# shionhonda/IaGo

Measured on AMD Instinct MI355X. Metric: self-play games/sec, higher is better.
Workload: dtype f16 MFMA operands (float32 split in 2 / 3 pieces), f32 accumulate; u64 bitboards; f32 / f64 tree statistics

## Files before the change

### iago_amd/csrc/conv_policy_body.hpp

```cpp
#pragma once
#include "abi_common.hpp"
#include "search_request.hpp"

#include <hip/hip_fp16.h>

#include <cstdlib>

#include <atomic>

namespace iago_policy {


typedef _Float16 half8 __attribute__((ext_vector_type(8)));
typedef float float16v __attribute__((ext_vector_type(16)));
typedef float float4v __attribute__((ext_vector_type(4)));
#define IAGO_POLICY_MFMA16(acc, a, b) asm volatile("v_mfma_f32_16x16x32_f16 %0, %1, %2, %0" : "+a"(acc) : "v"(a), "v"(b))
typedef unsigned int u32x4 __attribute__((ext_vector_type(4)));
typedef float f2 __attribute__((ext_vector_type(2)));
typedef _Float16 h2 __attribute__((ext_vector_type(2)));

constexpr int RS = 800;
constexpr int ZB = 1280;
constexpr int BS = 64 * RS + ZB;
constexpr int HEAD_FLOATS = 64;
constexpr int W1_LDS = (64 * 18 + 64) * 4;
constexpr int LDS_BYTES = BS + 1024 + HEAD_FLOATS * 4 + W1_LDS;
constexpr float S1 = 1.0f / 2048.0f, S2 = 1.0f / (2048.0f * 2048.0f);

struct PolicyParams {
    const uint64_t *own, *opp;
    const int64_t *index;
    const int32_t *n_dev;
    int64_t n;
    const float *w1, *b1;
    const uint4 *w_hi[7], *w_mid[7], *w_lo[7];
    const float *bias[7];
    const float *w9, *b10;
    float *probs;
    uint32_t *overflow;
    int layer_lo, layer_hi;
    uint4 *scratch;
    int64_t row_lo, row_hi;
};

__device__ __forceinline__ void split3(const f2 v, h2 &hi, h2 &mid, h2 &lo)
{
    hi = __builtin_convertvector(v, h2);
    const f2 r1 = (v - __builtin_convertvector(hi, f2)) * 2048.0f;
    mid = __builtin_convertvector(r1, h2);
    const f2 r2 = (r1 - __builtin_convertvector(mid, f2)) * 2048.0f;
    lo = __builtin_convertvector(r2, h2);
}

extern __shared__ __align__(16) char policy_lds[];

template <bool SRCH = false>
__device__ __forceinline__ void policy_item(const PolicyParams &P, const int64_t row_id, const uint32_t *pos = nullptr,
                                            float *res = nullptr, const float *w1_staged = nullptr,
                                            const float *head_w = nullptr)
{
    char *const T = policy_lds;
    int tid_ = threadIdx.x;
    if constexpr (SRCH)
        asm volatile("" : "+v"(tid_));
    const int tid = tid_, wv = __builtin_amdgcn_readfirstlane(tid >> 6), lane = tid & 63;
    const int64_t b = P.index ? P.index[row_id] : row_id;

    if (tid < ZB / 16)
        *(uint4 *)(T + 64 * RS + tid * 16) = make_uint4(0, 0, 0, 0);
    bool saturated = false;
    if (P.layer_lo > 0) {
        const uint4 *src = P.scratch + (row_id - P.row_lo) * (64 * RS / 16);
        for (int e = tid; e < 64 * RS / 16; e += 256)
            *(uint4 *)(T + e * 16) = src[e];
    } else {
        const int cell = tid & 63, y = cell >> 3, x = cell & 7;
        const uint64_t bits0 = SRCH ? iago_request::opp(pos) : P.opp[b];
        const uint64_t bits1 = SRCH ? iago_request::own(pos) : P.own[b];
        float in[18];
#pragma unroll
        for (int c = 0; c < 2; c++)
#pragma unroll
            for (int ky = 0; ky < 3; ky++)
#pragma unroll
                for (int kx = 0; kx < 3; kx++) {
                    const int yy = y + ky - 1, xx = x + kx - 1;
                    const bool ok = yy >= 0 && yy < 8 && xx >= 0 && xx < 8;
                    const int a = (yy * 8 + xx) & 63;
                    in[c * 9 + ky * 3 + kx] = (ok && (((c ? bits1 : bits0) >> a) & 1ull)) ? 1.0f : 0.0f;
                }
        const float *w1s = w1_staged;
        if constexpr (!SRCH) {
            float *const st = (float *)(T + BS + 1024 + HEAD_FLOATS * 4);
            for (int e = tid; e < 64 * 18 / 4; e += 256)
                ((float4 *)st)[e] = ((const float4 *)P.w1)[e];
            if (tid < 16)
                ((float4 *)(st + 64 * 18))[tid] = ((const float4 *)P.b1)[tid];
            __syncthreads();
            w1s = st;
        }
#pragma unroll 1
        for (int g2 = 0; g2 < 2; g2++) {
            const int grp = __builtin_amdgcn_readfirstlane(g2 * 4 + wv);
            const int co0 = grp * 8;
            _Float16 p0[8], p1[8], p2[8];
#pragma unroll
            for (int k = 0; k < 8; k += 2) {
                const float *wa = w1s + (co0 + k) * 18, *wb = wa + 18;
                f2 acc = (f2){w1s[64 * 18 + co0 + k], w1s[64 * 18 + co0 + k + 1]};
#pragma unroll
                for (int j = 0; j < 18; j++)
                    acc = __builtin_elementwise_fma((f2){wa[j], wb[j]}, (f2){in[j], in[j]}, acc);
                saturated |= !(acc.x <= 65000.0f) || !(acc.y <= 65000.0f);
                f2 v;
                v.x = fminf(fmaxf(acc.x, 0.0f), 65000.0f);
                v.y = fminf(fmaxf(acc.y, 0.0f), 65000.0f);
                h2 a0, a1, a2;
                split3(v, a0, a1, a2);
                p0[k] = a0.x, p0[k + 1] = a0.y;
                p1[k] = a1.x, p1[k + 1] = a1.y;
                p2[k] = a2.x, p2[k + 1] = a2.y;
            }
            char *dst = T + cell * RS + (grp >> 1) * 32 + (grp & 1) * 16;
            *(uint4 *)dst = *(const uint4 *)p0;
            *(uint4 *)(dst + 256) = *(const uint4 *)p1;
            *(uint4 *)(dst + 512) = *(const uint4 *)p2;
        }
    }
    __syncthreads();

    const int c16 = lane & 15, kq = lane >> 4;
    uint32_t addr[4][9];
#pragma unroll
    for (int q = 0; q < 4; q++)
#pragma unroll
        for (int tap = 0; tap < 9; tap++) {
            const int cell = 16 * q + c16;
            const int yy = (cell >> 3) + tap / 3 - 1, xx = (cell & 7) + tap % 3 - 1;
            const bool ok = yy >= 0 && yy < 8 && xx >= 0 && xx < 8;
            const int lin = (cell + (tap / 3 - 1) * 8 + (tap % 3 - 1)) & 7;
            addr[q][tap] = (uint32_t)((ok ? (yy * 8 + xx) * RS : 64 * RS + 32 * lin) + kq * 16);
        }
    uint32_t wrow[4];
#pragma unroll
    for (int q = 0; q < 4; q++)
        wrow[q] = (uint32_t)((16 * q + c16) * RS);

    for (int L = P.layer_lo; L < P.layer_hi; L++) {
        const int n_pairs = L == 0 ? 2 : 4;
        const char *const wh = (const char *)P.w_hi[L], *const wm = (const char *)P.w_mid[L], *const wl = (const char *)P.w_lo[L];
        const uint32_t a_lane = (uint32_t)(((32 * wv + c16) * 2 + (kq & 1) + (kq >> 1) * (9 * 256)) * 16);
        auto a_load = [&](const char *base, uint32_t step_bytes, int m) -> u32x4 {
            return *(const u32x4 *)(base + step_bytes + a_lane + (uint32_t)m * 512u);
        };
        float4v acc0[2][4], acc0b[2][4], acc1[2][4], acc2[2][4];
#pragma unroll
        for (int m = 0; m < 2; m++)
#pragma unroll
            for (int n = 0; n < 4; n++)
#pragma unroll
                for (int v = 0; v < 4; v++) {
                    acc0[m][n][v] = 0.0f;
                    acc0b[m][n][v] = 0.0f;
                    acc1[m][n][v] = 0.0f;
                    acc2[m][n][v] = 0.0f;
                }
        u32x4 a_hi[3][2], a_mid[3][2], a_lo[3][2];
#pragma unroll
        for (int i = 0; i < 2; i++)
#pragma unroll
            for (int m = 0; m < 2; m++) {
                a_hi[i][m] = a_load(wh, (uint32_t)i * 4096u, m);
                a_mid[i][m] = a_load(wm, (uint32_t)i * 4096u, m);
                a_lo[i][m] = a_load(wl, (uint32_t)i * 4096u, m);
            }
        half8 bh[3], bm[3], bl[3];
        auto b_addr = [&](int tile) -> const char * {
            const int over = tile >= 36 ? 64 : 0, tt = tile % 36;
            return T + addr[tt & 3][tt >> 2] + over;
        };
        {
            const char *p0 = b_addr(0), *p1 = b_addr(1);
            bh[0] = *(const half8 *)p0, bm[0] = *(const half8 *)(p0 + 256), bl[0] = *(const half8 *)(p0 + 512);
            bh[1] = *(const half8 *)p1, bm[1] = *(const half8 *)(p1 + 256), bl[1] = *(const half8 *)(p1 + 512);
        }
        for (int cp = 0; cp < n_pairs; cp++) {
#pragma unroll
            for (int tap = 0; tap < 9; tap++) {
                int cp2 = cp, tp2 = tap + 2;
                if (tp2 >= 9) {
                    tp2 -= 9;
                    cp2 += 1;
                }
                if (cp2 >= n_pairs) {
                    cp2 = n_pairs - 1;
                    tp2 = 8;
                }
                const uint32_t w2 = (uint32_t)(18 * cp2 + tp2) * 4096u;
                half8 ah[2], am[2], al[2];
#pragma unroll
                for (int m = 0; m < 2; m++) {
                    ah[m] = __builtin_bit_cast(half8, a_hi[tap % 3][m]);
                    am[m] = __builtin_bit_cast(half8, a_mid[tap % 3][m]);
                    al[m] = __builtin_bit_cast(half8, a_lo[tap % 3][m]);
                }
#pragma unroll
                for (int q = 0; q < 4; q++) {
                    const int tile = tap * 4 + q, cur = tile % 3, nxt = (tile + 2) % 3;
                    const char *p = b_addr(tile + 2);
                    __builtin_amdgcn_sched_barrier(0);
                    IAGO_POLICY_MFMA16(acc2[0][q], ah[0], bl[cur]);
                    bh[nxt] = *(const half8 *)p;
                    __builtin_amdgcn_sched_barrier(0);
                    IAGO_POLICY_MFMA16(acc2[1][q], ah[1], bl[cur]);
                    bm[nxt] = *(const half8 *)(p + 256);
                    __builtin_amdgcn_sched_barrier(0);
                    IAGO_POLICY_MFMA16(acc1[0][q], ah[0], bm[cur]);
                    bl[nxt] = *(const half8 *)(p + 512);
                    __builtin_amdgcn_sched_barrier(0);
                    IAGO_POLICY_MFMA16(acc1[1][q], ah[1], bm[cur]);
                    if (q == 0)
                        a_hi[(tap + 2) % 3][0] = a_load(wh, w2, 0);
                    else if (q == 1)
                        a_mid[(tap + 2) % 3][0] = a_load(wm, w2, 0);
                    else if (q == 2)
                        a_lo[(tap + 2) % 3][0] = a_load(wl, w2, 0);
                    __builtin_amdgcn_sched_barrier(0);
                    if (tap & 1)
                        IAGO_POLICY_MFMA16(acc0b[0][q], ah[0], bh[cur]);
                    else
                        IAGO_POLICY_MFMA16(acc0[0][q], ah[0], bh[cur]);
                    if (q == 0)
                        a_hi[(tap + 2) % 3][1] = a_load(wh, w2, 1);
                    else if (q == 1)
                        a_mid[(tap + 2) % 3][1] = a_load(wm, w2, 1);
                    else if (q == 2)
                        a_lo[(tap + 2) % 3][1] = a_load(wl, w2, 1);
                    __builtin_amdgcn_sched_barrier(0);
                    if (tap & 1)
                        IAGO_POLICY_MFMA16(acc0b[1][q], ah[1], bh[cur]);
                    else
                        IAGO_POLICY_MFMA16(acc0[1][q], ah[1], bh[cur]);
                    IAGO_POLICY_MFMA16(acc2[0][q], al[0], bh[cur]);
                    IAGO_POLICY_MFMA16(acc2[1][q], al[1], bh[cur]);
                    IAGO_POLICY_MFMA16(acc1[0][q], am[0], bh[cur]);
                    IAGO_POLICY_MFMA16(acc1[1][q], am[1], bh[cur]);
                    IAGO_POLICY_MFMA16(acc2[0][q], am[0], bm[cur]);
                    IAGO_POLICY_MFMA16(acc2[1][q], am[1], bm[cur]);
                    __builtin_amdgcn_sched_barrier(0);
                }
            }
#pragma unroll
            for (int q = 0; q < 4; q++)
#pragma unroll
                for (int tap = 0; tap < 9; tap++)
                    addr[q][tap] += 64u;
        }
#pragma unroll
        for (int q = 0; q < 4; q++)
#pragma unroll
            for (int tap = 0; tap < 9; tap++)
                addr[q][tap] -= 64u * (uint32_t)n_pairs;

        f2 bia[2][2];
#pragma unroll
        for (int m = 0; m < 2; m++) {
            const float4 bq = *(const float4 *)(P.bias[L] + 32 * wv + 16 * m + 4 * kq);
            bia[m][0] = (f2){bq.x, bq.y};
            bia[m][1] = (f2){bq.z, bq.w};
        }
        asm volatile("s_nop 15\n\ts_nop 7" ::: "memory");
        __syncthreads();
        float vmax = 0.0f;
        f2 vsum = (f2){0.0f, 0.0f};
#pragma unroll
        for (int q = 0; q < 4; q++) {
            char *row = T + wrow[q] + (32 * wv + 4 * kq) * 2;
#pragma unroll
            for (int m = 0; m < 2; m++) {
                h2 p0[2], p1[2], p2[2];
#pragma unroll
                for (int t2 = 0; t2 < 2; t2++) {
                    const f2 m0 = (f2){acc0[m][q][2 * t2], acc0[m][q][2 * t2 + 1]} + (f2){acc0b[m][q][2 * t2], acc0b[m][q][2 * t2 + 1]};
                    const f2 m1 = (f2){acc1[m][q][2 * t2], acc1[m][q][2 * t2 + 1]};
                    const f2 m2 = (f2){acc2[m][q][2 * t2], acc2[m][q][2 * t2 + 1]};
                    f2 v = (m2 * S2 + m1 * S1) + m0 + bia[m][t2];
                    vmax = fmaxf(fmaxf(vmax, v.x), v.y);
                    vsum += v;
                    v.x = __builtin_amdgcn_fmed3f(v.x, 0.0f, 65000.0f);
                    v.y = __builtin_amdgcn_fmed3f(v.y, 0.0f, 65000.0f);
                    split3(v, p0[t2], p1[t2], p2[t2]);
                }
                *(uint2 *)(row + 32 * m) = (uint2){__builtin_bit_cast(uint32_t, p0[0]), __builtin_bit_cast(uint32_t, p0[1])};
                *(uint2 *)(row + 32 * m + 256) =
                    (uint2){__builtin_bit_cast(uint32_t, p1[0]), __builtin_bit_cast(uint32_t, p1[1])};
                *(uint2 *)(row + 32 * m + 512) =
                    (uint2){__builtin_bit_cast(uint32_t, p2[0]), __builtin_bit_cast(uint32_t, p2[1])};
            }
        }
        saturated |= !(vmax <= 65000.0f) || !(vsum.x + vsum.y == vsum.x + vsum.y);
        __syncthreads();
    }
    if (P.overflow && saturated)
        *P.overflow = 1u;
    if (P.layer_hi < 7) {
        uint4 *dst = P.scratch + (row_id - P.row_lo) * (64 * RS / 16);
        for (int e = tid; e < 64 * RS / 16; e += 256)
            dst[e] = *(const uint4 *)(T + e * 16);
        return;
    }

    if (wv == 0) {
        const char *row = T + lane * RS;
        float acc = 0.0f;
#pragma unroll 4
        for (int c8 = 0; c8 < 16; c8++) {
            const half8 xh = *(const half8 *)(row + c8 * 16), xm = *(const half8 *)(row + 256 + c8 * 16),
                        xl = *(const half8 *)(row + 512 + c8 * 16);
            const float *w9 = SRCH ? head_w : P.w9;
            const float4 wa = *(const float4 *)(w9 + c8 * 8), wb = *(const float4 *)(w9 + c8 * 8 + 4);
            const float w[8] = {wa.x, wa.y, wa.z, wa.w, wb.x, wb.y, wb.z, wb.w};
#pragma unroll
            for (int e = 0; e < 8; e++) {
                const float xv = ((float)xl[e] * S2 + (float)xm[e] * S1) + (float)xh[e];
                acc = fmaf(w[e], xv, acc);
            }
        }
        const float logit = acc + (SRCH ? head_w[128 + lane] : P.b10[lane]);
        float mx = logit;
#pragma unroll
        for (int o = 32; o > 0; o >>= 1)
            mx = fmaxf(mx, __shfl_xor(mx, o));
        const float e = expf(logit - mx);
        float sum = e;
#pragma unroll
        for (int o = 32; o > 0; o >>= 1)
            sum += __shfl_xor(sum, o);
        if constexpr (SRCH)
            res[lane] = e / sum;
        else
            P.probs[row_id * 64 + lane] = e / sum;
    }
}

inline int policy_params_of(const iago_policy_split3_args *a, PolicyParams &P)
{
    if (!a || a->n < 0)
        return iago_fail(IAGO_ERR_INVALID, "iago_policy_forward_split3: null args or n < 0");
    if (!a->own || !a->opp || !a->w1 || !a->b1 || !a->w9 || !a->b10 || !a->probs)
        return iago_fail(IAGO_ERR_INVALID, "iago_policy_forward_split3: null pointer");
    for (int L = 0; L < 7; L++) {
        if (!a->w_hi[L] || !a->w_mid[L] || !a->w_lo[L] || !a->bias[L] || ((uintptr_t)a->w_hi[L] & 15u) ||
            ((uintptr_t)a->w_mid[L] & 15u) || ((uintptr_t)a->w_lo[L] & 15u) || ((uintptr_t)a->bias[L] & 15u))
            return iago_fail(IAGO_ERR_INVALID, "iago_policy_forward_split3: weights and biases of blocks 2..8 must be "
                                               "non-null and 16-byte aligned");
        P.w_hi[L] = (const uint4 *)a->w_hi[L];
        P.w_mid[L] = (const uint4 *)a->w_mid[L];
        P.w_lo[L] = (const uint4 *)a->w_lo[L];
        P.bias[L] = a->bias[L];
    }
    if (((uintptr_t)a->w9 & 15u) || ((uintptr_t)a->w1 & 15u) || ((uintptr_t)a->b1 & 15u))
        return iago_fail(IAGO_ERR_INVALID, "iago_policy_forward_split3: w1, b1, w9 must be 16-byte aligned");
    P.own = a->own;
    P.opp = a->opp;
    P.index = a->index;
    P.n_dev = a->n_dev;
    P.n = a->n;
    P.w1 = a->w1;
    P.b1 = a->b1;
    P.w9 = a->w9;
    P.b10 = a->b10;
    P.probs = a->probs;
    P.overflow = a->overflow;
    P.layer_lo = 0;
    P.layer_hi = 7;
    P.scratch = nullptr;
    P.row_lo = 0;
    P.row_hi = a->n;
    return IAGO_OK;
}

}
```

### iago_amd/csrc/conv_policy_kernel.hip

```cpp
#include "conv_policy_body.hpp"

#include <cstdlib>

namespace {
using namespace iago_policy;

__global__ __launch_bounds__(256) __attribute__((amdgpu_waves_per_eu(1, 1))) void policy_resident_kernel(PolicyParams P)
{
    int64_t n_rows = P.row_hi;
    if (P.n_dev)
        n_rows = min(n_rows, (int64_t)*P.n_dev);
    for (int64_t row = P.row_lo + blockIdx.x; row < n_rows; row += gridDim.x) {
        policy_item(P, row);
        __syncthreads();
    }
}

}

int iago_policy_forward_split3(const iago_policy_split3_args *a, void *stream)
{
    if (a && a->n == 0)
        return IAGO_OK;
    PolicyParams P;
    if (const int rc = policy_params_of(a, P))
        return rc;
    static std::atomic<uint64_t> configured{0};
    if (iago_reserve_lds((const void *)policy_resident_kernel, LDS_BYTES, configured,
                         "iago_policy_forward_split3: cannot reserve 52 KB of LDS"))
        return IAGO_ERR_HIP;
    static const int64_t cap = []() {
        const char *e = getenv("IAGO_POLICY_GRID");
        const long v = e ? atol(e) : 256;
        return (int64_t)(v < 1 ? 1 : v > 1024 ? 1024 : v);
    }();

    const int parts = a->parts < 1 ? 1 : (a->parts > 7 ? 7 : a->parts);
    if (parts > 1 && (!a->scratch || ((uintptr_t)a->scratch & 15u)))
        return iago_fail(IAGO_ERR_INVALID, "iago_policy_forward_split3: parts > 1 needs a 16-byte aligned scratch "
                                           "buffer of n x 51,200 bytes");
    P.scratch = (uint4 *)a->scratch;
    const int64_t chunk = (parts > 1 && a->scratch_rows > 0 && a->scratch_rows < a->n) ? a->scratch_rows : a->n;
    for (int64_t lo = 0; lo < a->n; lo += chunk) {
        P.row_lo = lo;
        P.row_hi = lo + chunk < a->n ? lo + chunk : a->n;
        const int64_t rows = P.row_hi - P.row_lo;
        const unsigned grid = (unsigned)(rows < cap ? rows : cap);
        for (int p = 0; p < parts; p++) {
            P.layer_lo = 7 * p / parts;
            P.layer_hi = 7 * (p + 1) / parts;
            hipLaunchKernelGGL(policy_resident_kernel, dim3(grid), dim3(256), LDS_BYTES, (hipStream_t)stream, P);
        }
    }
    return iago_check_launch("iago_policy_forward_split3");
}
```

### iago_amd/csrc/conv_trunk_body.hpp

```cpp
#pragma once
#include "abi_common.hpp"
#include "rollout_row_body.hpp"
#include "search_request.hpp"

#include <hip/hip_fp16.h>

#include <atomic>
#include <type_traits>

namespace iago_trunk {


typedef _Float16 half8 __attribute__((ext_vector_type(8)));
typedef float float16v __attribute__((ext_vector_type(16)));
typedef float float4v __attribute__((ext_vector_type(4)));
typedef unsigned int u32x4 __attribute__((ext_vector_type(4)));
typedef float f2 __attribute__((ext_vector_type(2)));
typedef _Float16 h2 __attribute__((ext_vector_type(2)));

constexpr int RS = 544;
constexpr int ZB = 1024;
constexpr int BS = 64 * RS + ZB;
constexpr int lds_alloc(int tb) { return tb * BS + 1024; }
constexpr int MAX_LAYERS = 8;

#define IAGO_MFMA16(acc, a, b) asm volatile("v_mfma_f32_16x16x32_f16 %0, %1, %2, %0" : "+a"(acc) : "v"(a), "v"(b))

struct TrunkRParams {
    const uint4 *x_hi, *x_lo;
    uint4 *y_hi, *y_lo;
    const uint4 *w_hi[MAX_LAYERS], *w_lo[MAX_LAYERS];
    const float *bias[MAX_LAYERS];
    int64_t n;
    int32_t cin0, n_layers;
    uint32_t *overflow;
    const float *planes;
    const uint64_t *own, *opp;
    const float *w1, *b1;
    const uint4 *w9_hi, *w9_lo;
    const float *b9, *w10, *w11;
    float *out;
    const int64_t *index;
    const int32_t *n_dev;
    int32_t count_lo, count_hi;
    int32_t layer_lo, layer_hi;
    char *scratch;
};
constexpr int IMG = 64 * RS;

struct Piece {
    const int64_t *index;
    const int32_t *n_dev;
    char *scratch;
    int layer_lo, layer_hi;
    const uint32_t *pos;
    float *res;
    const float *w1s;
    const char *head_w;
};
constexpr int HEAD_W_W9LO = 8192, HEAD_W_W10 = 16384, HEAD_W_W11 = 16384 + 32768, HEAD_W_B9 = HEAD_W_W11 + 512,
              HEAD_W_LDS = HEAD_W_B9 + 16;
__device__ __forceinline__ Piece whole_walk(const TrunkRParams &P)
{
    return Piece{P.index, P.n_dev, P.scratch, P.layer_lo, P.layer_hi, nullptr, nullptr, nullptr, nullptr};
}

constexpr int head_lds(int tb) { return (9 * 64 * tb + 64 * tb + 128 * tb) * 4; }
constexpr int W1_LDS = (64 * 18 + 64) * 4;
constexpr int lds_alloc_fused(int tb) { return lds_alloc(tb) + head_lds(tb) + W1_LDS; }

__device__ __forceinline__ int cell_of_lane(int r)
{
    return r < 4 ? r : r < 12 ? 16 + (r - 4) : r < 16 ? 4 + (r - 12) : r < 20 ? 24 + (r - 16) : r < 28 ? 8 + (r - 20)
                                                                                              : 28 + (r - 28);
}

extern __shared__ __align__(16) char trunk_lds[];

constexpr bool tile_off_board(int tb, int tap, int n)
{
    return tb >= 2 && ((tap < 3 && (n & 7) == 0) || (tap >= 6 && (n & 7) == 7));
}
constexpr int kept_before(int tb, int tap, int n)
{
    int k = 0;
    for (int t = 0; t < 9; t++)
        for (int m = 0; m < 4 * tb; m++) {
            if (t == tap && m == n)
                return k;
            k += !tile_off_board(tb, t, m);
        }
    return k;
}
constexpr int kept_tile(int tb, int k)
{
    for (int t = 0; t < 9; t++)
        for (int m = 0; m < 4 * tb; m++)
            if (!tile_off_board(tb, t, m) && k-- == 0)
                return t * 4 * tb + m;
    return -1;
}
template <int I0, int I1, class F>
__device__ __forceinline__ void static_for(F &&f)
{
    if constexpr (I0 < I1) {
        f(std::integral_constant<int, I0>{});
        static_for<I0 + 1, I1>(f);
    }
}

template <bool FUSED, int TB, bool SRCH = false>
__device__ __forceinline__ void trunk_item(const TrunkRParams &P, const Piece &W, const int64_t b0, const int64_t n_rows)
{
    constexpr int NN = 4 * TB;
    char *const T = trunk_lds;
    int tid_ = threadIdx.x;
    if constexpr (SRCH)
        asm volatile("" : "+v"(tid_));
    const int tid = tid_, wv = __builtin_amdgcn_readfirstlane(tid >> 6), lane = tid & 63, r = lane & 31, h = lane >> 5;

    if (tid < TB * (ZB / 16))
        *(uint4 *)(T + (tid / (ZB / 16)) * BS + 64 * RS + (tid % (ZB / 16)) * 16) = make_uint4(0, 0, 0, 0);
    bool saturated = false;
    constexpr bool PIECES = FUSED && TB <= 2;
    if (PIECES && W.layer_lo > 0) {
        constexpr int PER = (TB * (IMG / 16) + 255) / 256;
        uint4 img[PER];
#pragma unroll
        for (int i = 0; i < PER; i++) {
            const int e = min(tid + i * 256, TB * (IMG / 16) - 1);
            const int board = e / (IMG / 16), off = e - board * (IMG / 16);
            const int64_t row = min(b0 + board, n_rows - 1);
            img[i] = ((const uint4 *)(W.scratch + row * IMG))[off];
        }
#pragma unroll
        for (int i = 0; i < PER; i++) {
            const int e = tid + i * 256;
            const int board = e / (IMG / 16), off = e - board * (IMG / 16);
            if (e < TB * (IMG / 16))
                *(uint4 *)(T + board * BS + off * 16) = img[i];
        }
    } else if constexpr (FUSED) {
        const int cell = tid & 63, y = cell >> 3, x = cell & 7;
        float in[TB][18];
#pragma unroll
        for (int board = 0; board < TB; board++) {
            const int64_t row = min(b0 + board, n_rows - 1);
            const int64_t b = W.index ? W.index[row] : row;
            const float *pl = P.planes + b * 128;
            uint64_t bits0, bits1;
            if constexpr (SRCH) {
                const uint32_t *w = W.pos + iago_request::WORDS * board;
                bits1 = iago_request::own(w);
                bits0 = iago_request::opp(w);
            } else {
                bits0 = P.planes ? 0ull : P.opp[b];
                bits1 = P.planes ? 0ull : P.own[b];
            }
#pragma unroll
            for (int c = 0; c < 2; c++)
#pragma unroll
                for (int ky = 0; ky < 3; ky++)
#pragma unroll
                    for (int kx = 0; kx < 3; kx++) {
                        const int yy = y + ky - 1, xx = x + kx - 1;
                        const bool ok = yy >= 0 && yy < 8 && xx >= 0 && xx < 8;
                        const int a = (yy * 8 + xx) & 63;
                        float v;
                        if (P.planes)
                            v = ok ? pl[c * 64 + a] : 0.0f;
                        else
                            v = (ok && (((c ? bits1 : bits0) >> a) & 1ull)) ? 1.0f : 0.0f;
                        in[board][c * 9 + ky * 3 + kx] = v;
                    }
        }
        const float *w1s = W.w1s;
        if constexpr (!SRCH) {
            float *const st = (float *)(T + lds_alloc(TB) + head_lds(TB));
            for (int e = tid; e < 64 * 18 / 4; e += 256)
                ((float4 *)st)[e] = ((const float4 *)P.w1)[e];
            if (tid < 16)
                ((float4 *)(st + 64 * 18))[tid] = ((const float4 *)P.b1)[tid];
            __syncthreads();
            w1s = st;
        }
#pragma unroll 1
        for (int g2 = 0; g2 < 2; g2++) {
            const int grp = __builtin_amdgcn_readfirstlane(g2 * 4 + wv);
            const int co0 = grp * 8;
            _Float16 h8[TB][8], l8[TB][8];
#pragma unroll
            for (int k = 0; k < 8; k++) {
                const float *wk = w1s + (co0 + k) * 18;
                const float bk = w1s[64 * 18 + co0 + k];
                float wreg[18];
#pragma unroll
                for (int j = 0; j < 18; j++)
                    wreg[j] = wk[j];
                float accs[TB];
                if constexpr (TB % 2 == 0) {
#pragma unroll
                    for (int bp = 0; bp < TB; bp += 2) {
                        f2 acc = (f2){bk, bk};
#pragma unroll
                        for (int j = 0; j < 18; j++)
                            acc = __builtin_elementwise_fma((f2){wreg[j], wreg[j]}, (f2){in[bp][j], in[bp + 1][j]}, acc);
                        accs[bp] = acc.x;
                        accs[bp + 1] = acc.y;
                    }
                } else {
#pragma unroll
                    for (int board = 0; board < TB; board++) {
                        float acc = bk;
#pragma unroll
                        for (int j = 0; j < 18; j++)
                            acc = fmaf(wreg[j], in[board][j], acc);
                        accs[board] = acc;
                    }
                }
#pragma unroll
                for (int board = 0; board < TB; board++) {
                    const float acc = accs[board];
                    saturated |= !(acc <= 65000.0f);
                    const float v = fminf(fmaxf(acc, 0.0f), 65000.0f);
                    const _Float16 vh = (_Float16)v;
                    h8[board][k] = vh;
                    l8[board][k] = (_Float16)((v - (float)vh) * 2048.0f);
                }
            }
#pragma unroll
            for (int board = 0; board < TB; board++) {
                char *dst = T + board * BS + cell * RS + (grp >> 1) * 32 + (grp & 1) * 16;
                *(uint4 *)dst = *(const uint4 *)h8[board];
                *(uint4 *)(dst + 256) = *(const uint4 *)l8[board];
            }
        }
    } else {
        const int chunks0 = P.cin0 >> 4;
        const int pieces = TB * chunks0 * 128;
        for (int e = tid; e < pieces; e += 256) {
            const int board = e / (chunks0 * 128), rem = e - board * chunks0 * 128;
            const int chunk = rem >> 7, cell = (rem >> 1) & 63, hp = rem & 1;
            const int64_t b = min(b0 + board, P.n - 1);
            const int64_t src = (b * chunks0 + chunk) * 128 + (rem & 127);
            char *dst = T + board * BS + cell * RS + chunk * 32 + hp * 16;
            *(uint4 *)dst = P.x_hi[src];
            *(uint4 *)(dst + 256) = P.x_lo[src];
        }
    }
    __syncthreads();

    constexpr bool ROWS = TB >= 2;
    static_assert(TB == 1 || TB == 2 || TB == 4, "boards per workgroup");
    const int c16 = lane & 15, kq = lane >> 4;
    constexpr int NADDR = ROWS ? 9 : 36;
    uint32_t addr[NADDR];
    uint32_t sx[2] = {0u, 0u};
    uint32_t wrow[ROWS ? 1 : 4];
    if constexpr (ROWS) {
        const int x = c16 & 7, odd = c16 >> 3;
#pragma unroll
        for (int tap = 0; tap < 9; tap++) {
            const int row = tap < 3 ? 1 : 0;
            const int yy = row + tap / 3 - 1, xx = x + tap % 3 - 1;
            const bool ok = xx >= 0 && xx < 8;
            addr[tap] = (uint32_t)(odd * BS + (ok ? (yy * 8 + xx) * RS : 64 * RS + 32 * (xx & 7)) + kq * 16);
        }
        sx[0] = x > 0 ? 8u * RS : 0u;
        sx[1] = x < 7 ? 8u * RS : 0u;
        wrow[0] = (uint32_t)(odd * BS + x * RS);
    } else {
#pragma unroll
        for (int q = 0; q < 4; q++)
#pragma unroll
            for (int tap = 0; tap < 9; tap++) {
                const int cell = 16 * q + c16;
                const int yy = (cell >> 3) + tap / 3 - 1, xx = (cell & 7) + tap % 3 - 1;
                const bool ok = yy >= 0 && yy < 8 && xx >= 0 && xx < 8;
                const int lin = (cell + (tap / 3 - 1) * 8 + (tap % 3 - 1)) & 7;
                addr[9 * q + tap] = (uint32_t)((ok ? (yy * 8 + xx) * RS : 64 * RS + 32 * lin) + kq * 16);
            }
#pragma unroll
        for (int q = 0; q < 4; q++)
            wrow[q] = (uint32_t)((16 * q + c16) * RS);
    }
    auto b_off = [&](int tap, int n) -> uint32_t {
        if constexpr (ROWS) {
            const int dx = tap % 3 - 1, r = (n & 7) - (tap < 3 ? 1 : 0);
            return addr[tap] + (uint32_t)r * (dx == 0 ? 8u * RS : sx[dx > 0]) + (uint32_t)(n >> 3) * (2u * BS);
        } else {
            return addr[9 * n + tap];
        }
    };

    const int L_lo = PIECES ? W.layer_lo : 0, L_hi = PIECES ? W.layer_hi : P.n_layers;
    for (int L = L_lo; L < L_hi; L++) {
        const int n_pairs = L == 0 ? (P.cin0 >> 5) : 4;
        const char *const wh = (const char *)P.w_hi[L], *const wl = (const char *)P.w_lo[L];
        const uint32_t a_lane = (uint32_t)(((32 * wv + c16) * 2 + (kq & 1) + (kq >> 1) * (9 * 256)) * 16);
        auto a_load = [&](const char *base, uint32_t step_bytes, int m) -> u32x4 {
            return *(const u32x4 *)(base + step_bytes + a_lane + (uint32_t)m * 512u);
        };
        float4v acc_main[2][NN], acc_cross[2][NN];
#pragma unroll
        for (int m = 0; m < 2; m++)
#pragma unroll
            for (int n = 0; n < NN; n++)
#pragma unroll
                for (int v = 0; v < 4; v++) {
                    acc_main[m][n][v] = 0.0f;
                    acc_cross[m][n][v] = 0.0f;
                }

        u32x4 a_hi[3][2], a_lo[3][2];
#pragma unroll
        for (int i = 0; i < 2; i++)
#pragma unroll
            for (int m = 0; m < 2; m++) {
                a_hi[i][m] = a_load(wh, (uint32_t)i * 4096u, m);
                a_lo[i][m] = a_load(wl, (uint32_t)i * 4096u, m);
            }
        constexpr int KEPT = kept_before(TB, 9, 0), NR = KEPT % 4 == 0 ? 4 : 6;
        static_assert(KEPT % NR == 0, "the B ring must line up at every chunk pair");
        half8 bh[NR], bl[NR];
        static_for<0, 3>([&](auto kc) __attribute__((always_inline)) {
            constexpr int tile = kept_tile(TB, decltype(kc)::value);
            const char *p0 = T + b_off(tile / NN, tile % NN);
            bh[decltype(kc)::value] = *(const half8 *)p0;
            bl[decltype(kc)::value] = *(const half8 *)(p0 + 256);
        });
        for (int cp = 0; cp < n_pairs; cp++) {
            static_for<0, KEPT>([&](auto kc) __attribute__((always_inline)) {
                constexpr int k = decltype(kc)::value, tile = kept_tile(TB, k), tap = tile / NN, n = tile % NN;
                constexpr int j = k - kept_before(TB, tap, 0);
                static_assert(kept_before(TB, tap + 1, 0) - kept_before(TB, tap, 0) >= 4, "four A loads per k-step");
                constexpr int kn = k + 3, tile_n = kept_tile(TB, kn % KEPT), cur = k % NR, nxt = kn % NR;
                constexpr uint32_t over = kn >= KEPT ? 64u : 0u;
                int cp2 = cp, tp2 = tap + 2;
                if (tp2 >= 9) {
                    tp2 -= 9;
                    cp2 += 1;
                }
                if (cp2 >= n_pairs) {
                    cp2 = n_pairs - 1;
                    tp2 = 8;
                }
                const uint32_t w2 = (uint32_t)(18 * cp2 + tp2) * 4096u;
                const half8 ah0 = __builtin_bit_cast(half8, a_hi[tap % 3][0]), ah1 = __builtin_bit_cast(half8, a_hi[tap % 3][1]);
                const half8 al0 = __builtin_bit_cast(half8, a_lo[tap % 3][0]), al1 = __builtin_bit_cast(half8, a_lo[tap % 3][1]);
                const char *p = T + b_off(tile_n / NN, tile_n % NN) + over;
                __builtin_amdgcn_sched_barrier(0);
                IAGO_MFMA16(acc_cross[0][n], ah0, bl[cur]);
                bh[nxt] = *(const half8 *)p;
                __builtin_amdgcn_sched_barrier(0);
                IAGO_MFMA16(acc_cross[1][n], ah1, bl[cur]);
                bl[nxt] = *(const half8 *)(p + 256);
                __builtin_amdgcn_sched_barrier(0);
                IAGO_MFMA16(acc_main[0][n], ah0, bh[cur]);
                if constexpr (j == 0)
                    a_hi[(tap + 2) % 3][0] = a_load(wh, w2, 0);
                else if constexpr (j == 1)
                    a_hi[(tap + 2) % 3][1] = a_load(wh, w2, 1);
                else if constexpr (j == 2)
                    a_lo[(tap + 2) % 3][0] = a_load(wl, w2, 0);
                else if constexpr (j == 3)
                    a_lo[(tap + 2) % 3][1] = a_load(wl, w2, 1);
                __builtin_amdgcn_sched_barrier(0);
                IAGO_MFMA16(acc_main[1][n], ah1, bh[cur]);
                IAGO_MFMA16(acc_cross[0][n], al0, bh[cur]);
                IAGO_MFMA16(acc_cross[1][n], al1, bh[cur]);
                __builtin_amdgcn_sched_barrier(0);
            });
#pragma unroll
            for (int i = 0; i < NADDR; i++)
                addr[i] += 64u;
        }
#pragma unroll
        for (int i = 0; i < NADDR; i++)
            addr[i] -= 64u * (uint32_t)n_pairs;

        f2 bia[2][2];
#pragma unroll
        for (int m = 0; m < 2; m++) {
            const float4 bq = *(const float4 *)(P.bias[L] + 32 * wv + 16 * m + 4 * kq);
            bia[m][0] = (f2){bq.x, bq.y};
            bia[m][1] = (f2){bq.z, bq.w};
        }
        asm volatile("s_nop 15\n\ts_nop 7" ::: "memory");
        __syncthreads();
        float vmax = 0.0f;
        f2 vsum = (f2){0.0f, 0.0f};
#pragma unroll
        for (int n = 0; n < NN; n++) {
            char *row = T + (ROWS ? wrow[0] + (n & 7) * (8 * RS) + (n >> 3) * (2 * BS) : wrow[ROWS ? 0 : n]) + (32 * wv + 4 * kq) * 2;
#pragma unroll
            for (int m = 0; m < 2; m++) {
                h2 hi[2], lo[2];
#pragma unroll
                for (int t2 = 0; t2 < 2; t2++) {
                    const f2 mm = (f2){acc_main[m][n][2 * t2], acc_main[m][n][2 * t2 + 1]};
                    const f2 c = (f2){acc_cross[m][n][2 * t2], acc_cross[m][n][2 * t2 + 1]};
                    f2 v = c * (1.0f / 2048.0f) + mm + bia[m][t2];
                    vmax = fmaxf(fmaxf(vmax, v.x), v.y);
                    vsum += v;
                    v.x = __builtin_amdgcn_fmed3f(v.x, 0.0f, 65000.0f);
                    v.y = __builtin_amdgcn_fmed3f(v.y, 0.0f, 65000.0f);
                    hi[t2] = __builtin_convertvector(v, h2);
                    lo[t2] = __builtin_convertvector((v - __builtin_convertvector(hi[t2], f2)) * 2048.0f, h2);
                }
                *(uint2 *)(row + 32 * m) = (uint2){__builtin_bit_cast(uint32_t, hi[0]), __builtin_bit_cast(uint32_t, hi[1])};
                *(uint2 *)(row + 32 * m + 256) =
                    (uint2){__builtin_bit_cast(uint32_t, lo[0]), __builtin_bit_cast(uint32_t, lo[1])};
            }
        }
        saturated |= !(vmax <= 65000.0f) || !(vsum.x + vsum.y == vsum.x + vsum.y);
        __syncthreads();
    }
    if (P.overflow && saturated)
        *P.overflow = 1u;

    if (PIECES && W.layer_hi < P.n_layers) {
        for (int e = tid; e < TB * (IMG / 16); e += 256) {
            const int board = e / (IMG / 16), off = e - board * (IMG / 16);
            if (b0 + board < n_rows)
                ((uint4 *)(W.scratch + (b0 + board) * IMG))[off] = *(const uint4 *)(T + board * BS + off * 16);
        }
        return;
    }
    if constexpr (FUSED) {
        constexpr int NC = 64 * TB;
        float *const Dm = (float *)(T + lds_alloc(TB));
        float *const h9s = Dm + 9 * NC;
        float *const hid = h9s + NC;
        float4 w10row[16];
        if constexpr (!SRCH) {
#pragma unroll
            for (int c = 0; c < 16; c++)
                w10row[c] = ((const float4 *)(P.w10 + (tid & 127) * 64))[c];
        }
        const float w11j = SRCH ? ((const float *)(W.head_w + HEAD_W_W11))[tid & 127] : P.w11[tid & 127];
        const float b9 = SRCH ? *(const float *)(W.head_w + HEAD_W_B9) : P.b9[0];
        const int lane_cell = cell_of_lane(r);
        if (wv < TB) {
            const u32x4 *w9h = (const u32x4 *)P.w9_hi + r * 2 + h;
            const u32x4 *w9l = (const u32x4 *)P.w9_lo + r * 2 + h;
            float16v hm[2], hc[2];
#pragma unroll
            for (int jt = 0; jt < 2; jt++)
#pragma unroll
                for (int v = 0; v < 16; v++) {
                    hm[jt][v] = 0.0f;
                    hc[jt][v] = 0.0f;
                }
            u32x4 w9a[SRCH ? 1 : 8], w9b[SRCH ? 1 : 8];
            if constexpr (!SRCH) {
#pragma unroll
                for (int c = 0; c < 8; c++) {
                    w9a[c] = w9h[c * 64];
                    w9b[c] = w9l[c * 64];
                }
            }
#pragma unroll
            for (int c = 0; c < 8; c++) {
                const half8 ah = SRCH ? *(const half8 *)(W.head_w + (c * 64 + r * 2 + h) * 16)
                                      : __builtin_bit_cast(half8, w9a[SRCH ? 0 : c]);
                const half8 al = SRCH ? *(const half8 *)(W.head_w + HEAD_W_W9LO + (c * 64 + r * 2 + h) * 16)
                                      : __builtin_bit_cast(half8, w9b[SRCH ? 0 : c]);
#pragma unroll
                for (int jt = 0; jt < 2; jt++) {
                    const int jj = 2 * wv + jt;
                    const char *p = T + (jj >> 1) * BS + (32 * (jj & 1) + lane_cell) * RS + h * 16 + c * 32;
                    const half8 bh9 = *(const half8 *)p, bl9 = *(const half8 *)(p + 256);
                    hm[jt] = __builtin_amdgcn_mfma_f32_32x32x16_f16(ah, bh9, hm[jt], 0, 0, 0);
                    hc[jt] = __builtin_amdgcn_mfma_f32_32x32x16_f16(ah, bl9, hc[jt], 0, 0, 0);
                    hc[jt] = __builtin_amdgcn_mfma_f32_32x32x16_f16(al, bh9, hc[jt], 0, 0, 0);
                }
            }
#pragma unroll
            for (int jt = 0; jt < 2; jt++) {
                const int jj = 2 * wv + jt;
                const int base = (jj >> 1) * 64 + 32 * (jj & 1) + lane_cell;
#pragma unroll
                for (int t = 0; t < 4; t++)
                    Dm[(4 * h + t) * NC + base] = hm[jt][t] + hc[jt][t] * (1.0f / 2048.0f);
                if (h == 0)
                    Dm[8 * NC + base] = hm[jt][4] + hc[jt][4] * (1.0f / 2048.0f);
            }
        }
        __syncthreads();
        if constexpr (SRCH) {
#pragma unroll
            for (int c = 0; c < 16; c++)
                w10row[c] = ((const float4 *)(W.head_w + HEAD_W_W10))[c * 128 + (tid & 127)];
        }
        if (tid < NC) {
            const int cell = tid & 63, y = cell >> 3, x = cell & 7;
            float s9 = 0.0f;
#pragma unroll
            for (int tap = 0; tap < 9; tap++) {
                const int yy = y + tap / 3 - 1, xx = x + tap % 3 - 1;
                if (yy >= 0 && yy < 8 && xx >= 0 && xx < 8)
                    s9 += Dm[tap * NC + (tid & ~63) + yy * 8 + xx];
            }
            h9s[tid] = fmaxf(s9 + b9, 0.0f);
        }
        __syncthreads();
        if ((tid >> 7) * 2 < TB) {
            const int j = tid & 127, pb = (tid >> 7) * 2;
            float s0 = 0.0f, s1 = 0.0f;
#pragma unroll
            for (int c = 0; c < 16; c++) {
                const float4 wq = w10row[c];
                const float4 x0 = *(const float4 *)(h9s + pb * 64 + 4 * c);
                const float4 x1 = *(const float4 *)(h9s + (pb + 1 < TB ? pb + 1 : pb) * 64 + 4 * c);
                s0 = fmaf(wq.x, x0.x, s0);
                s0 = fmaf(wq.y, x0.y, s0);
                s0 = fmaf(wq.z, x0.z, s0);
                s0 = fmaf(wq.w, x0.w, s0);
                s1 = fmaf(wq.x, x1.x, s1);
                s1 = fmaf(wq.y, x1.y, s1);
                s1 = fmaf(wq.z, x1.z, s1);
                s1 = fmaf(wq.w, x1.w, s1);
            }
            hid[pb * 128 + j] = s0 * w11j;
            if (pb + 1 < TB)
                hid[(pb + 1) * 128 + j] = s1 * w11j;
        }
        __syncthreads();
        if (tid < TB && b0 + tid < n_rows) {
            float4 hv[32];
#pragma unroll
            for (int j4 = 0; j4 < 32; j4++)
                hv[j4] = *(const float4 *)(hid + tid * 128 + 4 * j4);
            float v = 0.0f;
#pragma unroll
            for (int j4 = 0; j4 < 32; j4++) {
#pragma clang fp reassociate(off)
                v += hv[j4].x;
                v += hv[j4].y;
                v += hv[j4].z;
                v += hv[j4].w;
            }
            const int64_t row = b0 + tid;
            if constexpr (SRCH)
                W.res[tid] = v;
            else
                P.out[W.index ? W.index[row] : row] = v;
        }
        return;
    }
    for (int e = tid; e < TB * 1024; e += 256) {
        const int board = e >> 10, cb = (e >> 7) & 7, cell = (e >> 1) & 63, hp = e & 1;
        const int64_t b = b0 + board;
        if (b < P.n) {
            const char *src = T + board * BS + cell * RS + cb * 32 + hp * 16;
            P.y_hi[b * 1024 + (e & 1023)] = *(const uint4 *)src;
            P.y_lo[b * 1024 + (e & 1023)] = *(const uint4 *)(src + 256);
        }
    }
}

template <bool FUSED, int TB>
__device__ __forceinline__ void trunk_walk(const TrunkRParams &P, const Piece &W, const int64_t bid, const int64_t nb)
{
    int64_t n_rows = P.n;
    if constexpr (FUSED) {
        if (W.n_dev)
            n_rows = min(P.n, (int64_t)*W.n_dev);
        if (n_rows <= P.count_lo || n_rows > P.count_hi)
            return;
    }
    for (int64_t b0 = bid * TB; b0 < n_rows; b0 += nb * TB) {
        trunk_item<FUSED, TB>(P, W, b0, n_rows);
        __syncthreads();
    }
}

inline int value_params_of(const iago_value_split_args *a, TrunkRParams &P)
{
    if (!a || a->n < 0)
        return iago_fail(IAGO_ERR_INVALID, "iago_value_forward_split: null args or n < 0");
    if ((!a->planes && (!a->own || !a->opp)) || !a->w1 || !a->b1 || !a->w9_hi || !a->w9_lo || !a->b9 || !a->w10 ||
        !a->w11 || !a->out)
        return iago_fail(IAGO_ERR_INVALID, "iago_value_forward_split: null pointer");
    for (int L = 0; L < 7; L++) {
        if (!a->w_hi[L] || !a->w_lo[L] || !a->bias[L] || ((uintptr_t)a->w_hi[L] & 15u) || ((uintptr_t)a->w_lo[L] & 15u) ||
            ((uintptr_t)a->bias[L] & 15u))
            return iago_fail(IAGO_ERR_INVALID, "iago_value_forward_split: weights and biases of blocks 2..8 must be "
                                               "non-null and 16-byte aligned");
        P.w_hi[L] = (const uint4 *)a->w_hi[L];
        P.w_lo[L] = (const uint4 *)a->w_lo[L];
        P.bias[L] = a->bias[L];
    }
    P.w_hi[7] = P.w_hi[6];
    P.w_lo[7] = P.w_lo[6];
    P.bias[7] = P.bias[6];
    if (((uintptr_t)a->w9_hi & 15u) || ((uintptr_t)a->w9_lo & 15u) || ((uintptr_t)a->w10 & 15u) || ((uintptr_t)a->w1 & 15u) ||
        ((uintptr_t)a->b1 & 15u))
        return iago_fail(IAGO_ERR_INVALID, "iago_value_forward_split: w1, b1, w9_hi, w9_lo, w10 must be 16-byte aligned");
    P.x_hi = P.x_lo = nullptr;
    P.y_hi = P.y_lo = nullptr;
    P.n = a->n;
    P.cin0 = 64;
    P.n_layers = 7;
    P.overflow = a->overflow;
    P.planes = a->planes;
    P.own = a->own;
    P.opp = a->opp;
    P.w1 = a->w1;
    P.b1 = a->b1;
    P.w9_hi = (const uint4 *)a->w9_hi;
    P.w9_lo = (const uint4 *)a->w9_lo;
    P.b9 = a->b9;
    P.w10 = a->w10;
    P.w11 = a->w11;
    P.out = a->out;
    if (a->index && a->planes)
        return iago_fail(IAGO_ERR_INVALID, "iago_value_forward_split: a gather list needs the boards, not planes");
    P.index = a->index;
    P.n_dev = a->n_dev;
    P.layer_lo = 0;
    P.layer_hi = 7;
    P.scratch = nullptr;
    return IAGO_OK;
}

}
```

### iago_amd/csrc/search_kernel.hip

```cpp
#include "mcts_dev.hpp"
#include "conv_trunk_body.hpp"
#include "conv_policy_body.hpp"
#include "sample_dev.hpp"
#include "search_request.hpp"
#include "../../include/iago_hip_serving.h"

#include <algorithm>
#include <cstdlib>
#include <mutex>
#include <string>
#include <vector>

namespace {
using namespace iago;
using namespace iago_mcts;

typedef unsigned long long u64;
#define RLX_AGENT __ATOMIC_RELAXED, __HIP_MEMORY_SCOPE_AGENT

constexpr uint32_t QCAP = IAGO_SEARCH_QUEUE_ENTRIES;
constexpr int CTL_FINISHED = 2, CTL_ABORT = 3;
__host__ __device__ constexpr int ctl_head(uint32_t q) { return 8 + 2 * (int)q; }
__host__ __device__ constexpr int ctl_tail(uint32_t q) { return 9 + 2 * (int)q; }
enum { ST_READY = 0, ST_WAIT_PRIOR, ST_PRIOR_READY, ST_ROLL, ST_ROLL_FRESH, ST_WAIT_VALUE, ST_HAVE_VALUE, ST_DONE, ST_TURN, ST_MOVE,
       ST_WAIT_DRAW, ST_DRAW,
       ST_IDLE };
constexpr int CTL_NO_CHILDREN = 4;
constexpr uint32_t MATCH_KEY = 0x4D415443u;
constexpr int CTL_BAD_DRAW = 13;
constexpr int CTL_PROGRESS = 5, CTL_PLAYING = 6;
constexpr int CTL_NET_WGS = 7;
constexpr int CTL_IDLE = 14;
constexpr int CTL_NEXT_GAME = 12;
namespace rq = iago_request;
using rq::KIND_POLICY;
using rq::KIND_VALUE;
using rq::NOBODY;
constexpr int GAMES_PER_WG = IAGO_SEARCH_GAMES_PER_WORKGROUP;

constexpr int SEARCH_IMG_V = iago_trunk::lds_alloc(2) + iago_trunk::head_lds(2);
constexpr int SEARCH_IMG_P = iago_policy::BS + 1024 + iago_policy::HEAD_FLOATS * 4;
constexpr int SEARCH_IMG_TOP = SEARCH_IMG_V > SEARCH_IMG_P ? SEARCH_IMG_V : SEARCH_IMG_P;

struct SearchParams {
    Tree T;
    const uint64_t *root_own, *root_opp;
    const uint8_t *active;
    float c_puct, lmbda;
    int32_t n_thr, n_sims, n_game_wgs, games_per_wg;
    int32_t *cur_node;
    uint64_t *cur_own, *cur_opp;
    int32_t *path;
    int32_t path_stride;
    int32_t *done;
    uint8_t *roll;
    int8_t *z;
    float *leaf_value;
    int8_t *z_log;
    int32_t *z_log_n;
    int32_t z_log_rows;
    u64 *q_slots;
    uint32_t *ctl;
    u64 *rep_v, *rep_p;
    int64_t *totals;
    int32_t *stats;
    uint64_t *wg_own, *wg_opp;
    long long clock_limit;
    int32_t max_turns;
    uint64_t *game_own, *game_opp;
    int32_t *n_turns;
    uint64_t *rec_own, *rec_opp;
    uint8_t *rec_valid;
    int8_t *rec_move;
    int32_t *rec_pi;
    int32_t games_total, stream;
    u64 *vtable;
    uint32_t vtable_mask;
    int64_t *trace;
    int32_t trace_rows;
    int32_t policy_xcds;
    int32_t pair_backlog;
    int32_t pace_margin, pace_backlog;
    int32_t ahead_idle;
    int32_t roll_defer;
    int32_t path_lds_cap;
    int32_t wave;
    float vloss;
    int64_t n_slots;
    int64_t *wave_timing;
    int32_t park_empties;
    uint8_t *parked;
    int32_t *park_stones;
    uint8_t *park_pass;
    int32_t explore_turns;
    int32_t cap_fast, cap_full_256;
    int32_t chain_skip;
    uint16_t *noise_counts;
    int32_t noise_eps, noise_lg;
    int32_t forced_k_256;
    int32_t negamax;
    float prior_off;
    double visit_off;
    const int32_t *gumbel_g, *gumbel_ln;
    const int16_t *gumbel_sched;
    int32_t gumbel_m, gumbel_c_visit, gumbel_c_scale;
};

constexpr int ROOT_PLAIN = 0, ROOT_NOISE = 1, ROOT_GUMBEL = 2;

__device__ __forceinline__ u64 ld(const u64 *p) { return __hip_atomic_load(p, RLX_AGENT); }
__device__ __forceinline__ void st(u64 *p, u64 x) { __hip_atomic_store(p, x, RLX_AGENT); }

__device__ __forceinline__ u64 *ring_entry(const SearchParams &S, uint32_t q, uint32_t t)
{
    return S.q_slots + ((u64)q * QCAP + t % QCAP) * (u64)rq::SLOT_STRIDE;
}

__device__ __forceinline__ void send_request(const SearchParams &S, uint32_t kind, int64_t g, uint32_t reply_tag,
                                             uint64_t own, uint64_t opp)
{
    const uint32_t t = __hip_atomic_fetch_add(&S.ctl[ctl_tail(kind)], 1u, RLX_AGENT);
    u64 *e = S.q_slots + ((u64)kind * QCAP + t % QCAP) * (u64)rq::SLOT_STRIDE;
    st(e + rq::W_TAG, rq::entry_word(t, reply_tag));
    st(e + rq::W_OWN_LO, rq::entry_word(t, (uint32_t)own));
    st(e + rq::W_OWN_HI, rq::entry_word(t, (uint32_t)(own >> 32)));
    st(e + rq::W_OPP_LO, rq::entry_word(t, (uint32_t)opp));
    st(e + rq::W_OPP_HI, rq::entry_word(t, (uint32_t)(opp >> 32)));
    st(e + rq::W_WHO, rq::entry_word(t, rq::who_word(kind, (uint32_t)g)));
    atomicAdd((unsigned long long *)&S.totals[(uint32_t)g == NOBODY ? 11 : kind], 1ull);
}

__device__ __forceinline__ bool search_over(const SearchParams &S, const long long t0)
{
    bool out = false;
    if (threadIdx.x == 0)
        out = __hip_atomic_load(&S.ctl[CTL_FINISHED], RLX_AGENT) >= (uint32_t)S.n_game_wgs ||
              __hip_atomic_load(&S.ctl[CTL_ABORT], RLX_AGENT) != 0u || wall_clock64() - t0 > S.clock_limit;
    return __builtin_amdgcn_ballot_w64(out) != 0ull;
}

__device__ __forceinline__ int ring_backlog(const SearchParams &S, uint32_t q)
{
    int d = 0;
    if (threadIdx.x == 0)
        d = (int32_t)(__hip_atomic_load(&S.ctl[ctl_tail(q)], RLX_AGENT) - __hip_atomic_load(&S.ctl[ctl_head(q)], RLX_AGENT));
    return __builtin_amdgcn_readfirstlane(d);
}
__device__ __forceinline__ uint32_t ring_take(const SearchParams &S, uint32_t q)
{
    uint32_t t = 0;
    if (threadIdx.x == 0)
        t = __hip_atomic_fetch_add(&S.ctl[ctl_head(q)], 1u, RLX_AGENT);
    return __builtin_amdgcn_readfirstlane(t);
}
__device__ __forceinline__ int ring_fetch(const SearchParams &S, uint32_t q, uint32_t t, uint32_t max_spins, uint32_t *dst,
                                          const long long t0)
{
    const int tid = threadIdx.x;
    const u64 *e = ring_entry(S, q, t);
    u64 x = 0;
    int status = 0;
    for (uint32_t spins = 0;; spins++) {
        x = (tid < rq::WORDS) ? ld(e + tid) : 0ull;
        const bool ok = tid >= rq::WORDS || rq::entry_is(x, t);
        if (__builtin_amdgcn_ballot_w64(ok) == ~0ull)
            break;
        if (max_spins && spins + 1u >= max_spins) {
            status = 1;
            break;
        }
        if ((spins & 15u) == 15u && search_over(S, t0)) {
            status = 2;
            break;
        }
        __builtin_amdgcn_s_sleep(8);
    }
    if (status == 0 && tid < rq::WORDS)
        dst[tid] = (uint32_t)x;
    return status;
}

__device__ __forceinline__ void reply_value(const SearchParams &S, const uint32_t *r, uint32_t bits)
{
    if (rq::game(r) != NOBODY)
        st(&S.rep_v[(int64_t)rq::game(r)], rq::reply_word(rq::tag(r), bits));
}
__device__ __forceinline__ void reply_prior(const SearchParams &S, const uint32_t *r, int i, uint32_t bits)
{
    st(&S.rep_p[(int64_t)rq::game(r) * 64 + i], rq::reply_word(rq::tag(r), bits));
}

__device__ __forceinline__ uint32_t vtable_slot(const SearchParams &S, uint64_t own, uint64_t opp)
{
    uint64_t h = own * 0x9E3779B97F4A7C15ull ^ (opp + 0xD1B54A32D192ED03ull) * 0xBF58476D1CE4E5B9ull;
    h ^= h >> 29;
    h *= 0x94D049BB133111EBull;
    h ^= h >> 32;
    return (uint32_t)h & S.vtable_mask;
}

__device__ __forceinline__ bool vtable_get(const SearchParams &S, uint64_t own, uint64_t opp, uint32_t &bits, uint32_t &writer)
{
    const u64 *e = S.vtable + (u64)vtable_slot(S, own, opp) * 4u;
    const u64 s1 = ld(e), o = ld(e + 1), p = ld(e + 2), v = ld(e + 3);
    __builtin_amdgcn_fence(__ATOMIC_ACQUIRE, "wavefront");
    const u64 s2 = ld(e);
    bits = (uint32_t)v;
    writer = (uint32_t)(s1 >> 32);
    return s1 != 0ull && (s1 & 1ull) == 0ull && s1 == s2 && o == own && p == opp && (v >> 32) == (s1 & 0xFFFFFFFFull);
}

__device__ __forceinline__ u64 *vtable_put_begin(const SearchParams &S, uint64_t own, uint64_t opp, uint32_t bits, uint32_t writer,
                                                 u64 &publish)
{
    u64 *e = S.vtable + (u64)vtable_slot(S, own, opp) * 4u;
    const u64 s = __hip_atomic_fetch_or(e, 1ull, RLX_AGENT);
    if (s & 1ull)
        return nullptr;
    uint32_t seq = (uint32_t)s + 2u;
    seq = seq ? seq : 2u;
    st(e + 1, own);
    st(e + 2, opp);
    st(e + 3, ((u64)seq << 32) | bits);
    publish = ((u64)writer << 32) | seq;
    return e;
}
__device__ __forceinline__ void vtable_put_end(u64 *e, u64 publish)
{
    asm volatile("s_waitcnt vmcnt(0)" ::: "memory");
    st(e, publish);
}

template <int CTRL>
__device__ __forceinline__ void most_visited_step(int &n, int &a)
{
    const int on = (int)dpp_u32<CTRL>((uint32_t)n), oa = (int)dpp_u32<CTRL>((uint32_t)a);
    const bool take = on > n || (on == n && oa < a);
    n = take ? on : n;
    a = take ? oa : a;
}

__device__ __forceinline__ bool group8_all(bool x)
{
    return group8_add(x ? 0u : 1u) == 0u;
}

__device__ __forceinline__ int policy_draw(const u64 *rep, uint64_t lg, double u)
{
    double s = 0.0;
#pragma unroll 1
    for (int j = 0; j < 64; j++)
        s += ((lg >> j) & 1ull) ? (double)__uint_as_float(rq::reply_bits(ld(rep + j))) : 0.0;
    double last = 0.0;
#pragma unroll 1
    for (int j = 0; j < 64; j++)
        last += (((lg >> j) & 1ull) ? (double)__uint_as_float(rq::reply_bits(ld(rep + j))) : 0.0) / s;
    if (!(s > 0.0) || !(s <= 1.7976931348623157e308) || !(last > 0.0))
        return 64;
    double acc = 0.0;
    int n = 0;
#pragma unroll 1
    for (int j = 0; j < 64; j++) {
        acc += (((lg >> j) & 1ull) ? (double)__uint_as_float(rq::reply_bits(ld(rep + j))) : 0.0) / s;
        n += acc / last <= u ? 1 : 0;
    }
    return n;
}

__device__ __forceinline__ int path_entry(int path_at, const int32_t *gpath, int d)
{
    return path_at >= 0 ? ((const int32_t *)iago_trunk::trunk_lds)[path_at + d] : gpath[d];
}

template <bool WAVE>
__device__ __forceinline__ void backup_game(const SearchParams &S, int64_t g, uint32_t r, int leaf, bool fresh, float vg,
                                            int path_n, const int8_t zl, const int negamax, const int path_at,
                                            const int64_t gt)
{
    const int64_t base = gt * (int64_t)S.T.capacity;
    const float lmbda = S.lmbda;
    if (fresh && lmbda < 1.0f && r == 0u)
        S.T.nodes[base + leaf].v = vg;
    const int8_t zg = lmbda > 0.0f ? zl : (int8_t)0;
    const float lv = leaf_mix(lmbda, vg, zg);
    if (r == 0u) {
        S.leaf_value[g] = lv;
        if (S.z_log && lmbda > 0.0f)
            log_z(S.z_log, S.z_log_n, S.z_log_rows, gt, S.T.n_games, zg);
    }
    const int len = path_n < S.path_stride ? path_n : S.path_stride;
    const int32_t *const gpath = S.path + g * (int64_t)S.path_stride;
    const float lvd = backup_value(negamax, lv, path_n, (int)r);
    for (int d = (int)r; d < len; d += 8) {
        const int node = path_entry(path_at, gpath, d);
        visit(S.T, base + node, lvd);
        if constexpr (WAVE)
            S.T.nodes[base + node].reserved1 -= 1;
    }
}

__device__ __forceinline__ bool wg_handoff_or(bool x)
{
    __builtin_amdgcn_fence(__ATOMIC_RELEASE, "workgroup");
    const bool any = __syncthreads_or(x) != 0;
    __builtin_amdgcn_fence(__ATOMIC_ACQUIRE, "workgroup");
    return any;
}


struct Slot {
    int tid, gl;
    int wg;
    uint32_t r;
    Lane8 L;
    bool mine, exists;
    int64_t g, gt, base;
    int64_t n_slots;
    int W, s_in, tl;
    int path_at;
    int32_t *gpath;
    bool whole, need_v, need_z;
    int search_end;
};

struct Game {
    int state;
    uint32_t epoch;
    int n_done, turn, stones;
    bool pass_flg, g_over;
    uint64_t g_own, g_opp;
};

struct Cursor {
    int node, fc, k, nv, nvv;
    uint32_t vbits;
    uint64_t own, opp;
    int path_n, leaf;
    bool may_expand, leaf_fresh;
    float v_reply;
};

struct GameLds {
    uint64_t h_own[GAMES_PER_WG], h_opp[GAMES_PER_WG];
    int32_t h_stream[GAMES_PER_WG];
    int32_t h_game[GAMES_PER_WG];
    int32_t h_budget[GAMES_PER_WG];
    uint8_t h_fast[GAMES_PER_WG];
    uint32_t wg_count[7];
    int32_t ch_from[GAMES_PER_WG], ch_len[GAMES_PER_WG], ch_run[GAMES_PER_WG];
    int32_t roll_list[GAMES_PER_WG];
    uint32_t roll_wave[BLOCK / 64], roll_wave_old[BLOCK / 64];
    int32_t pace[4];
    uint32_t claimed;
    int32_t negamax;
    int8_t h_z[GAMES_PER_WG];
};
template <bool WAVE> struct GameShared : GameLds {};
template <> struct GameShared<true> : GameLds {
    int32_t wv_next[GAMES_PER_WG], wv_size[GAMES_PER_WG], wv_block[GAMES_PER_WG];
    long long wv_time[4];
};

template <bool WAVE>
__device__ __forceinline__ Slot make_slot(const SearchParams &S, const int wg)
{
    Slot I;
    I.wg = wg;
    I.tid = threadIdx.x;
    I.gl = I.tid >> 3;
    I.L = make_lane8(threadIdx.x);
    I.r = I.L.l8;
    I.mine = I.tid < 8 * S.games_per_wg;
    I.g = (int64_t)wg * S.games_per_wg + I.gl;
    I.W = WAVE ? S.wave : 1;
    I.n_slots = WAVE ? S.n_slots : S.T.n_games;
    I.exists = I.mine && I.g < I.n_slots;
    I.gt = WAVE ? I.g / I.W : I.g;
    I.s_in = WAVE ? (int)(I.g % I.W) : 0;
    I.tl = WAVE ? I.gl / I.W : 0;
    I.base = I.exists ? I.gt * (int64_t)S.T.capacity : 0;
    I.need_v = S.lmbda < 1.0f;
    I.need_z = S.lmbda > 0.0f;
    const bool path_lds = (size_t)S.games_per_wg * (size_t)S.path_stride * 4u <= (size_t)S.path_lds_cap;
    I.path_at = path_lds ? I.gl * S.path_stride : -1;
    I.gpath = S.path + (I.exists ? I.g : 0) * (int64_t)S.path_stride;
    I.whole = S.max_turns > 0;
    I.search_end = I.whole ? ST_MOVE : ST_DONE;
    return I;
}

__device__ __forceinline__ void start_game(Game &G, uint64_t own, uint64_t opp)
{
    G.g_own = own;
    G.g_opp = opp;
    G.turn = 0;
    G.stones = 4;
    G.pass_flg = false;
    G.g_over = false;
    G.n_done = 0;
}

template <bool WAVE>
__device__ __forceinline__ void cursor_to(Cursor &C, int node, uint32_t fc, uint32_t nv, uint32_t an, uint32_t vv, uint32_t vbits)
{
    C.node = node;
    C.fc = (int)fc;
    C.k = (int)((an >> 8) & 0xFFu);
    C.nv = (int)nv;
    if (WAVE)
        C.nvv = (int)vv;
    C.vbits = vbits;
}

__device__ __forceinline__ void finish_playout(const SearchParams &S, const Slot &I, const GameLds &sh, Game &G,
                                               const Cursor &C, bool fresh, float v)
{
    backup_game<false>(S, I.g, I.r, C.leaf, fresh, v, C.path_n, sh.h_z[I.gl], sh.negamax, I.path_at, I.g);
    G.n_done++;
    if (S.trace && I.r == 0u)
        atomicAdd((unsigned long long *)&S.totals[9], 1ull);
    if (I.r == 0u)
        S.done[I.g] = G.turn * S.n_sims + G.n_done;
    G.state = G.n_done >= sh.h_budget[I.gl] ? I.search_end : ST_READY;
}

__device__ __forceinline__ void take_replies(const SearchParams &S, const iago_row::HwParams &R, const Slot &I,
                                             const GameLds &sh, Game &G, Cursor &C)
{
    if (G.state == ST_WAIT_PRIOR || G.state == ST_WAIT_DRAW) {
        bool ok = true;
#pragma unroll
        for (int i = 0; i < 8; i++)
            ok = ok && rq::reply_tag(ld(&S.rep_p[I.g * 64 + (int)I.r * 8 + i])) == G.epoch;
        if (group8_all(ok)) {
            if (G.state == ST_WAIT_DRAW) {
                const uint64_t lg = group8_legal(to_lane(G.g_own, I.L), to_lane(G.g_opp, I.L), I.L);
                const double u = sample_uniform(R.key0, R.key1 ^ MATCH_KEY, R.id_base + (uint32_t)sh.h_game[I.gl],
                                                (uint32_t)G.turn, 0u);
                C.leaf = policy_draw(S.rep_p + I.g * 64, lg, u);
                if (C.leaf == 64) {
                    if (I.r == 0u)
                        __hip_atomic_store(&S.ctl[CTL_BAD_DRAW], 1u, RLX_AGENT);
                    C.leaf = (int)__builtin_ctzll(lg);
                }
            }
            G.state = G.state == ST_WAIT_PRIOR ? ST_PRIOR_READY : ST_DRAW;
        }
    } else if (G.state == ST_WAIT_VALUE) {
        const u64 x = ld(&S.rep_v[I.g]);
        if (rq::reply_tag(x) == G.epoch) {
            C.v_reply = __uint_as_float(rq::reply_bits(x));
            G.state = ST_HAVE_VALUE;
        }
    }
}

__device__ __forceinline__ int most_visited(const Tree &T, const Slot &I, uint64_t lg, int rfc, bool at_move, int (&row_n)[8])
{
    int best_n = -1, best_a = 0x7fffffff;
#pragma unroll
    for (int i = 0; i < 8; i++) {
        const int a = (int)(8u * I.r) + i;
        int n = 0;
        if (at_move && rfc >= 0 && ((lg >> a) & 1ull)) {
            n = T.nodes[I.base + rfc + __popcll(lg & ((1ull << a) - 1ull))].n_visits;
            if (n > best_n) {
                best_n = n;
                best_a = a;
            }
        }
        row_n[i] = n;
    }
    most_visited_step<DPP_XOR1>(best_n, best_a);
    most_visited_step<DPP_XOR2>(best_n, best_a);
    most_visited_step<DPP_HALF_MIRROR>(best_n, best_a);
    return best_n >= 0 ? best_a : -2;
}

__device__ __forceinline__ void record_turn(const SearchParams &S, const Slot &I, const GameLds &sh, const Game &G, int valid,
                                            int mv, const int (&row_n)[8])
{
    const int64_t row = (int64_t)G.turn * S.games_total + sh.h_game[I.gl];
    if (I.r == 0u) {
        S.rec_own[row] = G.g_own;
        S.rec_opp[row] = G.g_opp;
        S.rec_valid[row] = (uint8_t)valid;
        S.rec_move[row] = (int8_t)(valid ? mv : -1);
    }
#pragma unroll
    for (int i = 0; i < 8; i++)
        S.rec_pi[row * 64 + (int)(8u * I.r) + i] = row_n[i];
}

__device__ __forceinline__ void advance_root(const Tree &T, const Slot &I, uint64_t lg, int rfc, int mv)
{
    int child = -1;
    if (rfc >= 0) {
        if (mv >= 0 && ((lg >> mv) & 1ull))
            child = rfc + __popcll(lg & ((1ull << mv) - 1ull));
        else if (mv == -1 && (int)T.nodes[I.base + rfc].action == -1)
            child = rfc;
    }
    if (child >= 0) {
        T.root[I.g] = child;
        T.nodes[I.base + child].parent = -1;
    } else {
        fresh_root(T, I.g, I.base);
    }
}

__device__ __forceinline__ void play_move(const SearchParams &S, const Slot &I, const GameLds &sh, Game &G, bool played, int mv,
                                          const long long t0)
{
    place_stone(G.g_own, G.g_opp, mv, I.L);
    const bool was_over = G.g_over;
    G.stones += played ? 1 : 0;
    const bool passing = !played && !was_over;
    if (passing && G.pass_flg)
        G.stones = 64;
    if (!was_over)
        G.pass_flg = passing;
    if (G.turn % 2 == 1)
        G.g_over = was_over || G.stones >= 64;
    G.turn++;
    if (G.turn >= S.max_turns || (G.turn % 2 == 0 && G.g_over)) {
        if (I.r == 0u) {
            const int64_t id = sh.h_game[I.gl];
            S.n_turns[id] = G.turn;
            S.game_own[id] = G.g_own;
            S.game_opp[id] = G.g_opp;
        }
        G.state = ST_DONE;
        if (S.trace && I.r == 0u && I.g < S.trace_rows) {
            int64_t *row = S.trace + 4 * ((int64_t)S.trace_rows - 1 - I.g);
            row[0] = wall_clock64() - t0;
            row[1] = G.epoch;
            row[2] = G.turn;
        }
    } else {
        G.state = ST_TURN;
    }
}

template <bool PARK>
__device__ __forceinline__ void turn_boundary(const SearchParams &S, const iago_row::HwParams &R, const Slot &I, GameLds &sh,
                                              Game &G, const Cursor &C, bool &busy, const long long t0)
{
    const Tree &T = S.T;
    for (int rep = 0; rep < 6; rep++) {
        const bool at_move = G.state == ST_MOVE, at_turn = G.state == ST_TURN, at_draw = G.state == ST_DRAW;
        if (__builtin_amdgcn_ballot_w64(at_move || at_turn || at_draw) == 0ull)
            break;
        busy = busy || at_move || at_turn || at_draw;
        if (at_move || at_turn || at_draw)
            sh.ch_from[I.gl] = -1;
        const bool explores = S.explore_turns > 0 && at_move && G.turn < S.explore_turns;
        const bool caps = S.cap_fast > 0 && at_turn;
        uint32_t w = 0u;
        if (__builtin_amdgcn_ballot_w64(explores || caps) != 0ull)
            w = turn_word(R.key0, R.key1 ^ (caps ? CAP_KEY : EXPLORE_KEY), R.id_base + (uint32_t)sh.h_game[I.gl], (uint32_t)G.turn);
        if (caps) {
            const bool fast = cap_fast_turn(w, (uint32_t)S.cap_full_256);
            sh.h_budget[I.gl] = fast ? S.cap_fast : S.n_sims;
            sh.h_fast[I.gl] = fast ? 1 : 0;
        }
        const uint64_t lg = group8_legal(to_lane(G.g_own, I.L), to_lane(G.g_opp, I.L), I.L);
        const bool can_move = lg != 0ull && !G.g_over;
        const int code = (at_turn && can_move && !S.stream) ? (int)S.active[I.g] : 0;
        const bool match = code == 2 || code == 3;
        const bool forced = match && G.stones > 62 && __popcll(lg) == 1;
        const bool policy_turn = match && !forced && (G.turn & 1) == (code == 2 ? 1 : 0);
        if (policy_turn) {
            G.epoch++;
            if (I.r == 0u)
                send_request(S, KIND_POLICY, I.g, G.epoch, G.g_own, G.g_opp);
            G.state = ST_WAIT_DRAW;
        }
        bool park = false;
        if constexpr (PARK)
            park = at_turn && can_move && 64 - __popcll(G.g_own | G.g_opp) <= S.park_empties;
        if (park) {
            if (I.r == 0u) {
                const int64_t id = sh.h_game[I.gl];
                S.n_turns[id] = G.turn;
                S.game_own[id] = G.g_own;
                S.game_opp[id] = G.g_opp;
                S.park_stones[id] = G.stones;
                S.park_pass[id] = G.pass_flg ? 1 : 0;
                S.parked[id] = 1;
            }
            G.state = ST_DONE;
        }
        if (at_turn && can_move && !forced && !policy_turn && !park) {
            G.n_done = 0;
            if (I.r == 0u)
                S.done[I.g] = G.turn * S.n_sims;
            G.state = ST_READY;
        }
        const bool drawn = at_draw || forced;
        const bool moving = at_move || drawn || (at_turn && !can_move);
        const int root = moving ? T.root[I.g] : 0;
        const int rfc = moving ? T.nodes[I.base + root].first_child : -1;
        int row_n[8];
        int best = most_visited(T, I, lg, rfc, at_move, row_n);
        if (__builtin_amdgcn_ballot_w64(explores) != 0ull) {
            const int drawn_a = explore_draw8(row_n, I.r, w);
            best = (explores && drawn_a < 64) ? drawn_a : best;
        }
        if (moving) {
            int mv = -1;
            if (at_move) {
                mv = best;
                if (mv == -2 && I.r == 0u)
                    __hip_atomic_store(&S.ctl[CTL_NO_CHILDREN], 1u, RLX_AGENT);
            }
            if (at_draw)
                mv = C.leaf;
            if (forced)
                mv = (int)__builtin_ctzll(lg);
            if (S.rec_move)
                record_turn(S, I, sh, G, at_move ? ((S.cap_fast > 0 && sh.h_fast[I.gl]) ? 4 : 1) : (drawn ? 2 : 0), mv, row_n);
            if (!G.g_over && !forced && I.r == 0u)
                advance_root(T, I, lg, rfc, mv);
            play_move(S, I, sh, G, at_move || drawn, mv, t0);
        }
    }
}

__device__ __forceinline__ void ask_priors(const SearchParams &S, const Slot &I, GameLds &sh, Game &G, const Cursor &C)
{
    G.epoch++;
    if (I.r == 0u)
        send_request(S, KIND_POLICY, I.g, G.epoch, C.own, C.opp);
    G.state = ST_WAIT_PRIOR;
    if (sh.pace[3] > 0 && I.need_v) {
        uint64_t rest = group8_legal(to_lane(C.own, I.L), to_lane(C.opp, I.L), I.L);
        while (rest) {
            const int a2 = (int)__builtin_ctzll(rest);
            rest &= rest - 1ull;
            uint64_t c_own = C.own, c_opp = C.opp;
            place_stone(c_own, c_opp, a2, I.L);
            uint32_t known = 0u, by = 0u;
            if (I.r == 0u && !vtable_get(S, c_own, c_opp, known, by) && atomicSub(&sh.pace[3], 1) > 0)
                send_request(S, KIND_VALUE, (int64_t)NOBODY, (uint32_t)I.g, c_own, c_opp);
        }
    }
}

template <bool WAVE>
__device__ __forceinline__ void reach_leaf(const SearchParams &S, const Slot &I, GameShared<WAVE> &sh, Game &G, Cursor &C,
                                           bool descending)
{
    if (descending && C.fc >= 0 && I.r == 0u)
        S.T.overflow[I.gt] = 1;
    C.leaf = C.node;
    if constexpr (!WAVE) {
        if (S.chain_skip && I.r == 0u) {
            const int run = sh.ch_run[I.gl];
            sh.ch_from[I.gl] = (!descending && C.path_n <= S.path_stride && run < C.path_n - 1) ? run : -1;
            sh.ch_len[I.gl] = C.path_n;
        }
    }
    const float c = __uint_as_float(C.vbits);
    C.leaf_fresh = I.need_v && c != c;
    bool ask = C.leaf_fresh;
    if (S.vtable) {
        uint32_t hit = 0u, bits = 0u, by = 0u;
        if (C.leaf_fresh && I.r == 0u && vtable_get(S, C.own, C.opp, bits, by)) {
            hit = 1u;
            atomicAdd((unsigned long long *)&S.totals[8], 1ull);
            if (by == (uint32_t)I.g)
                atomicAdd((unsigned long long *)&S.totals[12], 1ull);
        }
        hit = group8_add(hit);
        bits = group8_add(I.r == 0u ? bits : 0u);
        if (hit) {
            C.vbits = bits;
            ask = false;
        }
    }
    if (ask)
        G.epoch++;
    if (I.r == 0u) {
        S.cur_node[I.g] = C.node;
        S.cur_own[I.g] = C.own;
        S.cur_opp[I.g] = C.opp;
        sh.h_own[I.gl] = C.own;
        sh.h_opp[I.gl] = C.opp;
        sh.h_stream[I.gl] = G.turn * S.n_sims + G.n_done + I.s_in;
        if (ask)
            send_request(S, KIND_VALUE, I.g, G.epoch, C.own, C.opp);
    }
    G.state = ask ? ST_ROLL_FRESH : ST_ROLL;
    if constexpr (WAVE) {
        __threadfence_block();
        const int len = C.path_n < S.path_stride ? C.path_n : S.path_stride;
        for (int d = (int)I.r; d < len; d += 8)
            S.T.nodes[I.base + path_entry(I.path_at, I.gpath, d)].reserved1 += 1;
        if (I.r == 0u)
            sh.wv_next[I.tl] = I.s_in + 1;
    }
}

template <int NOISE>
__device__ __forceinline__ void expand(const SearchParams &S, const Slot &I, Cursor &C, bool &descending, bool have_priors,
                                       bool &need_prior)
{
    const Tree &T = S.T;
    const bool grow = descending && C.may_expand && C.fc < 0 && C.nv >= S.n_thr;
    if (__builtin_amdgcn_ballot_w64(grow) == 0ull)
        return;
    const uint64_t lg = group8_legal(to_lane(C.own, I.L), to_lane(C.opp, I.L), I.L);
    if (grow) {
        const int kn = lg ? __popcll(lg) : 1;
        if (lg != 0ull && kn > 1 && !have_priors) {
            need_prior = true;
            descending = false;
        } else {
            C.may_expand = false;
            const uint32_t fc1 = alloc_children(T, I.gt, kn, I.r == 0u);
            if (fc1 != 0u) {
                const int nf = (int)fc1 - 1;
                make_children(T, I.base, nf, C.node, lg, I.r, S.prior_off,
                              [&](int a) { return __uint_as_float(rq::reply_bits(ld(&S.rep_p[I.g * 64 + a]))); });
                if constexpr (NOISE == ROOT_NOISE) {
                    if (C.path_n == 1 && kn > 1) {
                        uint32_t c[8];
#pragma unroll
                        for (int i = 0; i < 8; i++)
                            c[i] = S.noise_counts[I.g * 64 + (int)(8u * I.r) + i];
                        noise_remix_children(T, I.base, nf, lg, I.r, c, (uint32_t)S.noise_eps, (uint32_t)S.noise_lg);
                    }
                }
                if (I.r == 0u)
                    link_children(T, I.base + C.node, nf, kn);
                C.fc = nf;
                C.k = kn;
            }
        }
    }
    __threadfence_block();
}

__device__ __forceinline__ void gumbel_child(const SearchParams &S, const Slot &I, uint4 s, uint4 l, int j, int want, int max_n,
                                             double &best_v, int &best_i, uint32_t (&pl)[4])
{
    const int n = (int)s.x;
    if (n != want)
        return;
    const int a = (int)(int8_t)(l.z & 0xFFu);
    const double v = gumbel_score(S.gumbel_g[I.gt * 64 + (a & 63)], gumbel_logit_q16(__uint_as_float(s.z), S.gumbel_ln),
                                  gumbel_q16(__uint_as_float(s.y), n), max_n, S.gumbel_c_visit, S.gumbel_c_scale);
    if (v > best_v) {
        best_v = v;
        best_i = j;
        pl[0] = l.x, pl[1] = (uint32_t)n, pl[2] = l.z & 0xFFFFu, pl[3] = s.w;
    }
}

template <bool WAVE, int NOISE>
__device__ __forceinline__ int select_child(const SearchParams &S, const Slot &I, Cursor &C, bool descending)
{
    const int kk = descending ? C.k : 0;
    const double sq = sqrt((double)(WAVE ? C.nv + C.nvv : C.nv));
    const double force_k = (NOISE == ROOT_NOISE && C.path_n == 1 && kk >= 2) ? (double)S.forced_k_256 : 0.0, force_n = (double)C.nv;
    double best_v = -INFINITY;
    int best_i = 0x7fffffff;
    uint32_t pl[4] = {0u, 0u, 0u, 0u};
    [[maybe_unused]] bool groot = false;
    [[maybe_unused]] int want = 0, max_n = 0;
    if constexpr (NOISE == ROOT_GUMBEL) {
        groot = C.path_n == 1 && kk >= 2;
        const int kg = groot ? kk : 0;
        uint32_t t = 0u, mx = 0u;
        for (int j = (int)I.r; j < kg; j += 8) {
            const uint32_t n = (uint32_t)S.T.nodes[I.base + C.fc + j].n_visits;
            t += n;
            mx = max(mx, n);
        }
        t = group8_add(t);
        mx = max(mx, dpp_u32<DPP_XOR1>(mx));
        mx = max(mx, dpp_u32<DPP_XOR2>(mx));
        mx = max(mx, dpp_u32<DPP_HALF_MIRROR>(mx));
        max_n = (int)mx;
        const int row = kk < S.gumbel_m ? kk : S.gumbel_m, col = (int)t < S.n_sims - 1 ? (int)t : S.n_sims - 1;
        want = groot ? (int)S.gumbel_sched[(int64_t)row * S.n_sims + col] : 0;
        uint32_t hit = 0u;
        for (int j = (int)I.r; j < kg; j += 8)
            hit |= S.T.nodes[I.base + C.fc + j].n_visits == want ? 1u : 0u;
        want = group8_add(hit) != 0u ? want : max_n;
    }
    for (int j0 = (int)I.r; j0 < kk; j0 += 16) {
        const int j1 = j0 + 8;
        const bool two = j1 < kk;
        const int64_t c0 = I.base + C.fc + j0, c1 = two ? I.base + C.fc + j1 : c0;
        uint4 s0, l0, s1, l1;
        node_record(S.T, c0, s0, l0);
        node_record(S.T, c1, s1, l1);
        if constexpr (NOISE == ROOT_GUMBEL) {
            if (groot) {
                gumbel_child(S, I, s0, l0, j0, want, max_n, best_v, best_i, pl);
                if (two)
                    gumbel_child(S, I, s1, l1, j1, want, max_n, best_v, best_i, pl);
                continue;
            }
        }
        score_child<WAVE, NOISE == ROOT_NOISE>(S.c_puct, (double)S.vloss, S.visit_off, s0, l0, j0, sq, best_v, best_i, pl, force_k,
                                               force_n);
        if (two)
            score_child<WAVE, NOISE == ROOT_NOISE>(S.c_puct, (double)S.vloss, S.visit_off, s1, l1, j1, sq, best_v, best_i, pl,
                                                   force_k, force_n);
    }
    argmax_step_payload<DPP_XOR1>(best_v, best_i, pl);
    argmax_step_payload<DPP_XOR2>(best_v, best_i, pl);
    argmax_step_payload<DPP_HALF_MIRROR>(best_v, best_i, pl);
    uint64_t own = C.own, opp = C.opp;
    const int action = descending ? (int)(int8_t)(pl[2] & 0xFFu) : -1;
    place_stone(own, opp, action, I.L);
    if (descending) {
        C.own = own;
        C.opp = opp;
        cursor_to<WAVE>(C, C.fc + best_i, pl[0], pl[1], pl[2], pl[2] >> 16, pl[3]);
    }
    return action;
}

template <bool WAVE, int NOISE>
__device__ __forceinline__ bool descend(const SearchParams &S, const Slot &I, GameShared<WAVE> &sh, Game &G, Cursor &C,
                                        int pace_limit, int &st_levels, int &st_children)
{
    bool my_turn = true;
    if constexpr (WAVE)
        my_turn = I.s_in == sh.wv_next[I.tl];
    const bool fresh_start = G.state == ST_READY && (WAVE ? my_turn : G.turn * S.n_sims + G.n_done <= pace_limit);
    bool descending = fresh_start || (G.state == ST_PRIOR_READY && my_turn);
    bool have_priors = G.state == ST_PRIOR_READY;
    bool skip_record = G.state == ST_PRIOR_READY;
    bool need_prior = false;
    if (fresh_start) {
        const int root = S.T.root[I.gt];
        C.own = I.whole ? G.g_own : S.root_own[I.gt];
        C.opp = I.whole ? G.g_opp : S.root_opp[I.gt];
        uint4 s0, l0;
        node_record(S.T, I.base + root, s0, l0);
        cursor_to<WAVE>(C, root, l0.x, s0.x, l0.z, l0.w, s0.w);
        C.path_n = 0;
        C.may_expand = true;
    }
    int jump_at = -1, jumped = 0;
    if constexpr (!WAVE) {
        if (S.chain_skip) {
            jump_at = descending ? sh.ch_from[I.gl] : -1;
            if (fresh_start && I.r == 0u)
                sh.ch_run[I.gl] = 0;
        }
    }
    const bool went = descending;
    for (int depth = 0; depth < MAX_DEPTH; depth++) {
        if constexpr (!WAVE) {
            if (descending && depth + jumped >= MAX_DEPTH) {
                descending = false;
                jumped = -1;
            }
            if (descending && !skip_record && C.path_n == jump_at) {
                const int len = sh.ch_len[I.gl], n_skip = len - 1 - jump_at;
                const int last = path_entry(I.path_at, I.gpath, len - 1);
                if (path_entry(I.path_at, I.gpath, jump_at) == C.node && depth + n_skip < MAX_DEPTH) {
                    uint4 s0, l0;
                    node_record(S.T, I.base + last, s0, l0);
                    if (n_skip & 1) {
                        const uint64_t t = C.own;
                        C.own = C.opp;
                        C.opp = t;
                    }
                    cursor_to<WAVE>(C, last, l0.x, s0.x, l0.z, l0.w, s0.w);
                    C.path_n = len;
                    skip_record = true;
                    jumped = n_skip;
                    st_levels += n_skip;
                    st_children += n_skip;
                    if (I.r == 0u)
                        atomicAdd(&sh.wg_count[6], (uint32_t)n_skip);
                }
                jump_at = -1;
            }
        }
        if (descending && !skip_record) {
            if (I.r == 0u) {
                if (C.path_n < S.path_stride) {
                    if (I.path_at >= 0)
                        ((int32_t *)iago_trunk::trunk_lds)[I.path_at + C.path_n] = C.node;
                    else
                        I.gpath[C.path_n] = C.node;
                }
                else
                    S.T.overflow[I.gt] = 1;
            }
            C.path_n++;
        }
        skip_record = false;
        expand<NOISE>(S, I, C, descending, have_priors, need_prior);
        have_priors = false;
        descending = descending && C.fc >= 0;
        if (__builtin_amdgcn_ballot_w64(descending) == 0ull)
            break;
        st_levels += descending ? 1 : 0;
        st_children += descending ? C.k : 0;
        if (__builtin_amdgcn_ballot_w64(descending && C.k != 1) == 0ull) {
            uint4 s0, l0;
            node_record(S.T, descending ? I.base + C.fc : I.base, s0, l0);
            const bool pass_child = (int)(int8_t)(l0.z & 0xFFu) < 0;
            if (__builtin_amdgcn_ballot_w64(descending && !pass_child) == 0ull) {
                if (descending) {
                    const uint64_t t = C.own;
                    C.own = C.opp;
                    C.opp = t;
                    cursor_to<WAVE>(C, C.fc, l0.x, s0.x, l0.z, l0.w, s0.w);
                }
                continue;
            }
        }
        const bool one = C.k == 1;
        const int action = select_child<WAVE, NOISE>(S, I, C, descending);
        if constexpr (!WAVE) {
            if (S.chain_skip && descending && I.r == 0u && !(one && action < 0))
                sh.ch_run[I.gl] = C.path_n;
        }
    }
    if constexpr (!WAVE)
        descending = descending || jumped < 0;
    if (went) {
        if (need_prior)
            ask_priors(S, I, sh, G, C);
        else
            reach_leaf<WAVE>(S, I, sh, G, C, descending);
    }
    if (I.exists && I.r == 0u)
        S.roll[I.g] = (I.need_z && (G.state == ST_ROLL || G.state == ST_ROLL_FRESH)) ? 1 : 0;
    return went;
}

struct CtlWords {
    uint32_t abort, idle, t0, h0, t1, h1, play, prog, next;
};
__device__ __forceinline__ CtlWords read_ctl(const SearchParams &S, int tid)
{
    CtlWords c = {0u, 0u, 0u, 0u, 0u, 0u, 0u, 0u, 0u};
    if (tid == 0) {
        if (S.stream)
            c.next = __hip_atomic_load(&S.ctl[CTL_NEXT_GAME], RLX_AGENT);
        c.abort = __hip_atomic_load(&S.ctl[CTL_ABORT], RLX_AGENT);
        c.idle = __hip_atomic_load(&S.ctl[CTL_IDLE], RLX_AGENT);
        c.t0 = __hip_atomic_load(&S.ctl[ctl_tail(0)], RLX_AGENT);
        c.h0 = __hip_atomic_load(&S.ctl[ctl_head(0)], RLX_AGENT);
        c.t1 = __hip_atomic_load(&S.ctl[ctl_tail(1)], RLX_AGENT);
        c.h1 = __hip_atomic_load(&S.ctl[ctl_head(1)], RLX_AGENT);
        c.play = __hip_atomic_load(&S.ctl[CTL_PLAYING], RLX_AGENT);
        c.prog = __hip_atomic_load(&S.ctl[CTL_PROGRESS], RLX_AGENT);
    }
    return c;
}

__device__ __forceinline__ bool rollout_passes(const SearchParams &S, const iago_row::HwParams &R, const Slot &I, GameLds &sh,
                                               bool rolls, bool &deferred, bool &table_ready)
{
    const uint64_t bal = __builtin_amdgcn_ballot_w64(rolls && I.r == 0u);
    const uint64_t balo = __builtin_amdgcn_ballot_w64(rolls && deferred && I.r == 0u);
    if ((I.tid & 63) == 0) {
        sh.roll_wave[I.tid >> 6] = (uint32_t)(((bal & 0x0101010101010101ull) * 0x0102040810204080ull) >> 56);
        sh.roll_wave_old[I.tid >> 6] = (uint32_t)(((balo & 0x0101010101010101ull) * 0x0102040810204080ull) >> 56);
    }
    if (I.tid < GAMES_PER_WG)
        sh.roll_list[I.tid] = -1;
    __syncthreads();
    uint32_t gm = 0u, go = 0u;
#pragma unroll
    for (int w = 0; w < BLOCK / 64; w++) {
        gm |= sh.roll_wave[w] << (8 * w);
        go |= sh.roll_wave_old[w] << (8 * w);
    }
    const int n_roll = __popc(gm), rem = n_roll & 15;
    const int n_now = (n_roll < 16 || rem > S.roll_defer) ? n_roll : n_roll - rem;
    const uint32_t below = (1u << I.gl) - 1u;
    const int rank = deferred ? __popc(go & below) : __popc(go) + __popc(gm & ~go & below);
    const bool now = rolls && rank < n_now;
    if (now && I.r == 0u)
        sh.roll_list[rank] = (int32_t)I.g;
    deferred = rolls && !now;
    __syncthreads();
    if (I.tid == 0)
        sh.wg_count[2 + (n_roll == 0 ? 0 : n_roll <= 16 ? 1 : n_roll <= 20 ? 2 : 3)]++;
    const iago_row::RowHandoff hand = {sh.h_own, sh.h_opp, sh.h_stream, sh.h_game, sh.h_z,
                                       (int32_t)((int64_t)I.wg * S.games_per_wg)};
#pragma unroll 1
    for (int at = 0; at < n_now; at += 16) {
        iago_row::rollout_row_body<false, true, true>(R, 0u, sh.roll_list + at, table_ready, &hand);
        table_ready = true;
        __syncthreads();
    }
    return !rolls || now;
}

__device__ __forceinline__ void wave_backups(const SearchParams &S, const Slot &I, GameShared<true> &sh, Game &G,
                                             const Cursor &C, const long long c_roll, bool &busy)
{
    const long long c_back = wall_clock64();
    if (I.tid == 0)
        sh.wv_time[1] += c_back - c_roll;
    if (I.mine && I.r == 0u && G.state != ST_HAVE_VALUE && G.state != ST_DONE && I.s_in < sh.wv_size[I.tl])
        sh.wv_block[I.tl] = 1;
    __syncthreads();
    const bool ready = I.mine && G.state != ST_DONE && sh.wv_block[I.tl] == 0;
    if (wg_handoff_or(ready)) {
        for (int j = 0; j < I.W; j++) {
            if (ready && I.s_in == j && G.state == ST_HAVE_VALUE) {
                backup_game<true>(S, I.g, I.r, C.leaf, C.leaf_fresh, C.v_reply, C.path_n, sh.h_z[I.gl], sh.negamax, I.path_at, I.gt);
                if (S.trace && I.r == 0u)
                    atomicAdd((unsigned long long *)&S.totals[9], 1ull);
            }
            wg_handoff_or(false);
        }
        if (ready) {
            G.n_done += sh.wv_size[I.tl];
            const int m = S.n_sims - G.n_done < I.W ? S.n_sims - G.n_done : I.W;
            G.state = G.n_done >= S.n_sims ? ST_DONE : (I.s_in < m ? ST_READY : ST_IDLE);
            if (I.r == 0u)
                S.done[I.g] = G.n_done;
            busy = true;
        }
        __syncthreads();
        if (ready && I.s_in == 0 && I.r == 0u) {
            const int m = S.n_sims - G.n_done < I.W ? S.n_sims - G.n_done : I.W;
            sh.wv_size[I.tl] = m;
            sh.wv_next[I.tl] = 0;
        }
    }
    if (I.mine && I.r == 0u && I.s_in == 0)
        sh.wv_block[I.tl] = 0;
    if (I.tid == 0)
        sh.wv_time[2] += wall_clock64() - c_back;
}

__device__ __forceinline__ bool iteration_end(const SearchParams &S, const Slot &I, GameLds &sh, const Game &G,
                                              const CtlWords &c, const long long t0, int &contrib, bool &in_play)
{
    const Tree &T = S.T;
    if (S.trace && I.wg == 0 && I.tid == 0 && (int64_t)sh.wg_count[0] < S.trace_rows - T.n_games) {
        const int64_t iters = (int64_t)sh.wg_count[0];
        S.trace[4 * iters + 0] = wall_clock64() - t0;
        S.trace[4 * iters + 1] = __hip_atomic_load(&S.ctl[ctl_tail(0)], RLX_AGENT) + __hip_atomic_load(&S.ctl[ctl_tail(1)], RLX_AGENT);
        S.trace[4 * iters + 2] = __hip_atomic_load(&S.ctl[ctl_head(0)], RLX_AGENT) + __hip_atomic_load(&S.ctl[ctl_head(1)], RLX_AGENT);
        S.trace[4 * iters + 3] = (int64_t)__hip_atomic_load(&S.ctl[CTL_FINISHED], RLX_AGENT) |
                                 (__hip_atomic_load(&S.totals[9], RLX_AGENT) << 8);
    }
    if (I.tid == 0)
        sh.wg_count[0]++;
    const int prog = G.state == ST_DONE ? 0 : G.turn * S.n_sims + G.n_done;
    if (I.mine && I.r == 0u) {
        if (prog != contrib)
            atomicAdd(&sh.pace[0], prog - contrib);
        if (in_play && G.state == ST_DONE)
            atomicAdd(&sh.pace[1], -1);
    }
    contrib = prog;
    in_play = in_play && G.state != ST_DONE;
    const bool over = wall_clock64() - t0 > S.clock_limit;
    if (over && I.tid == 0)
        __hip_atomic_store(&S.ctl[CTL_ABORT], 1u, RLX_AGENT);
    const int stop = __syncthreads_or(over || (I.tid == 0 && c.abort != 0u));
    if (I.tid == 0) {
        if (sh.pace[0])
            __hip_atomic_fetch_add(&S.ctl[CTL_PROGRESS], (uint32_t)sh.pace[0], RLX_AGENT);
        if (sh.pace[1])
            __hip_atomic_fetch_add(&S.ctl[CTL_PLAYING], (uint32_t)sh.pace[1], RLX_AGENT);
        sh.pace[0] = 0;
        sh.pace[1] = 0;
        int limit = 0x7fffffff;
        sh.pace[3] = 0;
        const int32_t wait0 = (int32_t)(c.t0 - c.h0), wait1 = (int32_t)(c.t1 - c.h1);
        if (S.ahead_idle >= 0 && S.vtable && I.n_slots <= (int64_t)(QCAP / 2u) && c.idle >= (uint32_t)S.ahead_idle &&
            wait0 <= 0 && wait1 <= 0)
            sh.pace[3] = (int32_t)((QCAP - (uint32_t)I.n_slots) / 2u) / S.n_game_wgs;
        if (S.pace_margin >= 0 && (!S.stream || (int64_t)c.next + T.n_games >= (int64_t)S.games_total)) {
            if (wait0 + wait1 > S.pace_backlog && c.play != 0u && c.play <= (uint32_t)T.n_games)
                limit = (int)(c.prog / c.play) + S.pace_margin;
        }
        sh.pace[2] = limit;
    }
    return stop != 0;
}

__device__ __forceinline__ bool stream_claim(const SearchParams &S, const Slot &I, GameLds &sh, Game &G, bool &in_play)
{
    const Tree &T = S.T;
    const int n_here = (int)min((int64_t)S.games_per_wg, I.n_slots - (int64_t)I.wg * S.games_per_wg);
    if (I.tid == 0)
        sh.claimed = __hip_atomic_fetch_add(&S.ctl[CTL_NEXT_GAME], (uint32_t)n_here, RLX_AGENT);
    __syncthreads();
    const int64_t next = T.n_games + (int64_t)sh.claimed + I.gl;
    if (I.exists && next < S.games_total) {
        start_game(G, S.game_own[next], S.game_opp[next]);
        if (I.r == 0u) {
            S.done[I.g] = 0;
            fresh_root(T, I.g, I.base);
            atomicAdd(&sh.pace[1], 1);
        }
        sh.h_game[I.gl] = (int32_t)next;
        sh.ch_from[I.gl] = -1;
        G.state = ST_TURN;
        in_play = true;
    }
    return __syncthreads_and(!I.mine || G.state == ST_DONE) != 0;
}

template <bool WAVE>
__device__ __forceinline__ void epilogue(const SearchParams &S, const Slot &I, GameShared<WAVE> &sh, const Game &G,
                                         int st_levels, int st_children, const long long t0)
{
    if (I.exists && I.r == 0u && S.stats) {
        if (WAVE) {
            atomicAdd(&S.stats[2 * I.gt], st_levels);
            atomicAdd(&S.stats[2 * I.gt + 1], st_children);
        } else {
            S.stats[2 * I.g] += st_levels;
            S.stats[2 * I.g + 1] += st_children;
        }
    }
    if constexpr (WAVE) {
        if (I.tid < 4 && S.wave_timing)
            atomicAdd((unsigned long long *)&S.wave_timing[I.tid], (unsigned long long)sh.wv_time[I.tid]);
    }
    if (I.exists && I.r == 0u && G.state != ST_DONE && __hip_atomic_load(&S.ctl[CTL_ABORT], RLX_AGENT) != 0u) {
        S.cur_node[I.g] = (int32_t)G.epoch;
        S.leaf_value[I.g] = (float)G.state;
    }
    if (I.tid == 0) {
        atomicAdd((unsigned long long *)&S.totals[2], (unsigned long long)sh.wg_count[0]);
        atomicAdd((unsigned long long *)&S.totals[6], (unsigned long long)sh.wg_count[1]);
        atomicAdd((unsigned long long *)&S.totals[10], (unsigned long long)sh.wg_count[2]);
        atomicAdd((unsigned long long *)&S.totals[13], (unsigned long long)sh.wg_count[3]);
        atomicAdd((unsigned long long *)&S.totals[14], (unsigned long long)sh.wg_count[4]);
        atomicAdd((unsigned long long *)&S.totals[15], (unsigned long long)sh.wg_count[5]);
        if (S.chain_skip)
            atomicAdd((unsigned long long *)&S.totals[16], (unsigned long long)sh.wg_count[6]);
        atomicAdd((unsigned long long *)&S.totals[7], (unsigned long long)(wall_clock64() - t0));
        __hip_atomic_fetch_add(&S.ctl[CTL_FINISHED], 1u, RLX_AGENT);
    }
}

template <bool WAVE, bool PARK = false, int NOISE = ROOT_PLAIN>
__device__ __forceinline__ void game_workgroup(const SearchParams &S, const iago_row::HwParams &R, const long long t0, const int wg)
{
    __shared__ GameShared<WAVE> sh;
    const Slot I = make_slot<WAVE>(S, wg);
    const bool first = I.exists && I.gt < S.games_total && (S.stream || S.active[I.gt] != 0);
    Game G;
    G.state = (first && S.n_sims > 0) ? (I.whole ? ST_TURN : ST_READY) : ST_DONE;
    G.epoch = 0u;
    if constexpr (WAVE) {
        const int m = S.n_sims < I.W ? S.n_sims : I.W;
        if (G.state == ST_READY && I.s_in >= m)
            G.state = ST_IDLE;
        if (I.tid < GAMES_PER_WG) {
            sh.wv_next[I.tid] = 0;
            sh.wv_size[I.tid] = m;
            sh.wv_block[I.tid] = 0;
        }
        if (I.tid < 4)
            sh.wv_time[I.tid] = 0;
    }
    if (I.exists && I.r == 0u) {
        S.done[I.g] = 0;
        S.roll[I.g] = 0;
    }
    if (I.mine) {
        sh.h_game[I.gl] = (int32_t)I.gt;
        sh.h_budget[I.gl] = S.n_sims;
        sh.h_fast[I.gl] = 0;
        sh.ch_from[I.gl] = -1;
    }
    const bool whole_game = I.whole && I.exists && I.g < S.games_total;
    start_game(G, whole_game ? S.game_own[I.g] : 0ull, whole_game ? S.game_opp[I.g] : 0ull);
    if (whole_game && G.state == ST_DONE && I.r == 0u)
        S.n_turns[I.g] = 0;
    Cursor C = {};
    C.fc = -1;
    int st_levels = 0, st_children = 0;
    if (I.tid < 7)
        sh.wg_count[I.tid] = 0u;
    if (I.tid == 7)
        sh.negamax = S.negamax;
    bool deferred = false;
    bool table_ready = false;
    int contrib = 0;
    bool in_play = G.state != ST_DONE;
    if (I.tid < 4)
        sh.pace[I.tid] = I.tid == 2 ? 0x7fffffff : 0;
    __syncthreads();
    if (I.mine && in_play && I.r == 0u)
        atomicAdd(&sh.pace[1], 1);
    int pace_limit = 0x7fffffff;

    for (;;) {
        const long long c_it = WAVE ? wall_clock64() : 0;
        bool busy = false;
        if (I.mine) {
            take_replies(S, R, I, sh, G, C);
            if (!WAVE && G.state == ST_HAVE_VALUE) {
                finish_playout(S, I, sh, G, C, true, C.v_reply);
                busy = true;
            }
            if (!WAVE && I.whole)
                turn_boundary<PARK>(S, R, I, sh, G, C, busy, t0);
        }
        const long long c_desc = WAVE ? wall_clock64() : 0;
        for (int sub = 0; sub < (WAVE ? I.W : 1); sub++) {
            bool went = false;
            if (I.mine) {
                went = descend<WAVE, NOISE>(S, I, sh, G, C, pace_limit, st_levels, st_children);
                busy = busy || went;
            }
            if constexpr (WAVE) {
                if (!wg_handoff_or(went))
                    break;
            }
        }
        if constexpr (WAVE) {
            if (I.tid == 0)
                sh.wv_time[0] += wall_clock64() - c_desc;
        }
        const CtlWords c = read_ctl(S, I.tid);
        const bool rolls = I.mine && I.need_z && (G.state == ST_ROLL || G.state == ST_ROLL_FRESH);
        const long long c_roll = WAVE ? wall_clock64() : 0;
        const bool rolled = rollout_passes(S, R, I, sh, rolls, deferred, table_ready);
        if (I.mine && rolled) {
            if (G.state == ST_ROLL) {
                if constexpr (WAVE) {
                    C.v_reply = __uint_as_float(C.vbits);
                    G.state = ST_HAVE_VALUE;
                } else {
                    finish_playout(S, I, sh, G, C, C.leaf_fresh, __uint_as_float(C.vbits));
                }
            } else if (G.state == ST_ROLL_FRESH) {
                G.state = ST_WAIT_VALUE;
            }
        }
        if constexpr (WAVE)
            wave_backups(S, I, sh, G, C, c_roll, busy);
        const bool stop = iteration_end(S, I, sh, G, c, t0, contrib, in_play);
        bool all_done = __syncthreads_and(!I.mine || G.state == ST_DONE) != 0;
        pace_limit = sh.pace[2];
        if (all_done && !stop && S.stream)
            all_done = stream_claim(S, I, sh, G, in_play);
        if (all_done || stop)
            break;
        if (!__syncthreads_or(busy)) {
            if (I.tid == 0)
                sh.wg_count[1]++;
            __builtin_amdgcn_s_sleep(32);
            if constexpr (WAVE) {
                if (I.tid == 0)
                    sh.wv_time[3] += wall_clock64() - c_it;
            }
        }
    }
    epilogue<WAVE>(S, I, sh, G, st_levels, st_children, t0);
}


struct NetLds {
    uint32_t req[2][rq::WORDS];
    uint32_t status, count;
    float res_v[2], res_p[64];
};
struct NetWeights {
    float *w1_val, *w1_pol;
    char *head_v;
    float *head_p;
};
struct NetState {
    uint32_t carry;
    int n_carry;
    u64 *put_e;
    u64 put_word;
    long long t_wait, t_walk, n_pairs;
};

__device__ __forceinline__ NetWeights stage_net_weights(const iago_trunk::TrunkRParams &VP, const iago_policy::PolicyParams &PP)
{
    const int tid = threadIdx.x;
    float *const w1_val = (float *)(iago_trunk::trunk_lds + SEARCH_IMG_TOP), *const w1_pol = w1_val + (64 * 18 + 64);
    for (int e = tid; e < 64 * 18 / 4; e += 256) {
        ((float4 *)w1_val)[e] = ((const float4 *)VP.w1)[e];
        ((float4 *)w1_pol)[e] = ((const float4 *)PP.w1)[e];
    }
    if (tid < 16) {
        ((float4 *)(w1_val + 64 * 18))[tid] = ((const float4 *)VP.b1)[tid];
        ((float4 *)(w1_pol + 64 * 18))[tid] = ((const float4 *)PP.b1)[tid];
    }
    char *const head_v = (char *)(w1_pol + (64 * 18 + 64));
    float *const head_p = (float *)(head_v + iago_trunk::HEAD_W_LDS);
    for (int e = tid; e < 512; e += 256) {
        ((uint4 *)head_v)[e] = VP.w9_hi[e];
        ((uint4 *)(head_v + iago_trunk::HEAD_W_W9LO))[e] = VP.w9_lo[e];
    }
    for (int e = tid; e < 128 * 16; e += 256)
        ((float4 *)(head_v + iago_trunk::HEAD_W_W10))[(e & 15) * 128 + (e >> 4)] = ((const float4 *)VP.w10)[e];
    if (tid < 128)
        ((float *)(head_v + iago_trunk::HEAD_W_W11))[tid] = VP.w11[tid];
    if (tid == 0)
        *(float *)(head_v + iago_trunk::HEAD_W_B9) = VP.b9[0];
    if (tid < 128)
        head_p[tid] = PP.w9[tid];
    if (tid < 64)
        head_p[128 + tid] = PP.b10[tid];
    __syncthreads();
    return NetWeights{w1_val, w1_pol, head_v, head_p};
}

__device__ __forceinline__ void claim(const SearchParams &S, const uint32_t home, NetState &N, NetLds &L, const long long t0)
{
    const int tid = threadIdx.x;
    int status = 2, count = 0;
    bool polling = false;
    for (;;) {
        uint32_t q = home;
        bool have = N.n_carry > 0;
        uint32_t t1 = N.carry;
        if (have) {
            q = KIND_VALUE;
            N.n_carry = 0;
        } else if (ring_backlog(S, home) > 0) {
            t1 = ring_take(S, home);
            have = true;
        } else if (ring_backlog(S, home ^ 1u) > 0) {
            q = home ^ 1u;
            t1 = ring_take(S, q);
            have = true;
        }
        if (have) {
            status = ring_fetch(S, q, t1, 0u, L.req[0], t0);
            count = status == 0 ? 1 : 0;
            if (status == 0 && q == KIND_VALUE && ring_backlog(S, KIND_VALUE) >= S.pair_backlog) {
                const uint32_t t2 = ring_take(S, KIND_VALUE);
                if (ring_fetch(S, KIND_VALUE, t2, 8u, L.req[1], t0) == 0) {
                    count = 2;
                } else {
                    N.carry = t2;
                    N.n_carry = 1;
                }
            }
            break;
        }
        if (search_over(S, t0))
            break;
        if (!polling) {
            polling = true;
            if (tid == 0)
                __hip_atomic_fetch_add(&S.ctl[CTL_IDLE], 1u, RLX_AGENT);
        }
        __builtin_amdgcn_s_sleep(16);
    }
    if (polling && tid == 0)
        __hip_atomic_fetch_add(&S.ctl[CTL_IDLE], 0xFFFFFFFFu, RLX_AGENT);
    if (tid == 0) {
        L.status = (uint32_t)status;
        L.count = (uint32_t)count;
    }
}

__device__ __forceinline__ void answer_value(const SearchParams &S, const iago_trunk::TrunkRParams &VP, NetState &N, NetLds &L,
                                             const NetWeights &Wt, const int64_t row0, const int count)
{
    const int tid = threadIdx.x;
    iago_trunk::Piece W = iago_trunk::whole_walk(VP);
    W.pos = L.req[0];
    W.res = L.res_v;
    W.w1s = Wt.w1_val;
    W.head_w = Wt.head_v;
    if (count == 2)
        iago_trunk::trunk_item<true, 2, true>(VP, W, row0, row0 + count);
    else
        iago_trunk::trunk_item<true, 1, true>(VP, W, row0, row0 + count);
    __syncthreads();
    if (tid < count) {
        const uint32_t *r = L.req[tid];
        const uint32_t bits = __float_as_uint(L.res_v[tid]);
        reply_value(S, r, bits);
        if (S.vtable)
            N.put_e = vtable_put_begin(S, rq::own(r), rq::opp(r), bits, rq::game(r) != NOBODY ? rq::game(r) : rq::tag(r),
                                       N.put_word);
    }
}

__device__ __forceinline__ void answer_policy(const SearchParams &S, const iago_policy::PolicyParams &PP, NetLds &L,
                                              const NetWeights &Wt, const int64_t row0)
{
    const int tid = threadIdx.x;
    iago_policy::policy_item<true>(PP, row0, L.req[0], L.res_p, Wt.w1_pol, Wt.head_p);
    __syncthreads();
    if (tid < 64)
        reply_prior(S, L.req[0], tid, __float_as_uint(L.res_p[tid]));
}

__device__ __forceinline__ void leave(const SearchParams &S, const NetState &N)
{
    if (threadIdx.x == 0) {
        atomicAdd((unsigned long long *)&S.totals[3], (unsigned long long)N.n_pairs);
        atomicAdd((unsigned long long *)&S.totals[4], (unsigned long long)N.t_wait);
        atomicAdd((unsigned long long *)&S.totals[5], (unsigned long long)N.t_walk);
    }
}

__device__ __forceinline__ void net_workgroup(const SearchParams &S, const iago_trunk::TrunkRParams &VP,
                                              const iago_policy::PolicyParams &PP, const long long t0, const int wg)
{
    __shared__ __align__(16) NetLds L;
    const int tid = threadIdx.x;
    const int64_t row0 = 4 * (int64_t)wg;
    const uint32_t home = ((int)((uint32_t)wg & 7u) >= 8 - S.policy_xcds) ? KIND_POLICY : KIND_VALUE;
    NetState N = {0u, 0, nullptr, 0, 0, 0, 0};
    const NetWeights Wt = stage_net_weights(VP, PP);
    for (;;) {
        const long long c0 = wall_clock64();
        if (N.put_e) {
            vtable_put_end(N.put_e, N.put_word);
            N.put_e = nullptr;
        }
        if (tid < 64)
            claim(S, home, N, L, t0);
        __syncthreads();
        const long long c1 = wall_clock64();
        N.t_wait += c1 - c0;
        if (L.status != 0u) {
            leave(S, N);
            return;
        }
        const uint32_t kind = rq::kind(L.req[0]);
        const int count = (int)L.count;
        N.n_pairs += count - 1;
        if (kind == KIND_VALUE)
            answer_value(S, VP, N, L, Wt, row0, count);
        else
            answer_policy(S, PP, L, Wt, row0);
        __syncthreads();
        N.t_walk += wall_clock64() - c1;
    }
}

template <bool WAVE, bool PARK = false, int NOISE = ROOT_PLAIN>
__device__ __forceinline__ void search_body(const SearchParams &S, const iago_row::HwParams &R, const iago_trunk::TrunkRParams &VP,
                                            const iago_policy::PolicyParams &PP)
{
    const long long t0 = wall_clock64();
    const int wg = (int)blockIdx.x;
    if (wg == 0 && threadIdx.x == 0)
        __hip_atomic_store(&S.ctl[CTL_NET_WGS], (uint32_t)gridDim.x - (uint32_t)S.n_game_wgs, RLX_AGENT);
    if (wg < S.n_game_wgs)
        game_workgroup<WAVE, PARK, NOISE>(S, R, t0, wg);
    net_workgroup(S, VP, PP, t0, wg);
}

__global__ __launch_bounds__(256) __attribute__((amdgpu_waves_per_eu(1, 1))) void search_kernel(
    SearchParams S, iago_row::HwParams R, iago_trunk::TrunkRParams VP, iago_policy::PolicyParams PP)
{
    search_body<false>(S, R, VP, PP);
}

__global__ __launch_bounds__(256) __attribute__((amdgpu_waves_per_eu(1, 1))) void search_wave_kernel(
    SearchParams S, iago_row::HwParams R, iago_trunk::TrunkRParams VP, iago_policy::PolicyParams PP)
{
    search_body<true>(S, R, VP, PP);
}

__global__ __launch_bounds__(256) __attribute__((amdgpu_waves_per_eu(2, 2))) void search_game_kernel(SearchParams S,
                                                                                                   iago_row::HwParams R)
{
    game_workgroup<false>(S, R, wall_clock64(), (int)blockIdx.x);
}

__global__ __launch_bounds__(256) __attribute__((amdgpu_waves_per_eu(1, 1))) void search_park_kernel(
    SearchParams S, iago_row::HwParams R, iago_trunk::TrunkRParams VP, iago_policy::PolicyParams PP)
{
    search_body<false, true>(S, R, VP, PP);
}

__global__ __launch_bounds__(256) __attribute__((amdgpu_waves_per_eu(2, 2))) void search_game_park_kernel(SearchParams S,
                                                                                                        iago_row::HwParams R)
{
    game_workgroup<false, true>(S, R, wall_clock64(), (int)blockIdx.x);
}

__global__ __launch_bounds__(256) __attribute__((amdgpu_waves_per_eu(1, 1))) void search_noise_kernel(
    SearchParams S, iago_row::HwParams R, iago_trunk::TrunkRParams VP, iago_policy::PolicyParams PP)
{
    search_body<false, false, ROOT_NOISE>(S, R, VP, PP);
}

__global__ __launch_bounds__(256) __attribute__((amdgpu_waves_per_eu(2, 2))) void search_game_noise_kernel(SearchParams S,
                                                                                                         iago_row::HwParams R)
{
    game_workgroup<false, false, ROOT_NOISE>(S, R, wall_clock64(), (int)blockIdx.x);
}

__global__ __launch_bounds__(256) __attribute__((amdgpu_waves_per_eu(1, 1))) void search_gumbel_kernel(
    SearchParams S, iago_row::HwParams R, iago_trunk::TrunkRParams VP, iago_policy::PolicyParams PP)
{
    search_body<false, false, ROOT_GUMBEL>(S, R, VP, PP);
}

__global__ __launch_bounds__(256) __attribute__((amdgpu_waves_per_eu(2, 2))) void search_game_gumbel_kernel(SearchParams S,
                                                                                                          iago_row::HwParams R)
{
    game_workgroup<false, false, ROOT_GUMBEL>(S, R, wall_clock64(), (int)blockIdx.x);
}

__global__ __launch_bounds__(256) __attribute__((amdgpu_waves_per_eu(1, 1))) void search_net_kernel(
    SearchParams S, iago_trunk::TrunkRParams VP, iago_policy::PolicyParams PP)
{
    const long long t0 = wall_clock64();
    if (blockIdx.x == 0 && threadIdx.x == 0)
        __hip_atomic_store(&S.ctl[CTL_NET_WGS], (uint32_t)gridDim.x, RLX_AGENT);
    net_workgroup(S, VP, PP, t0, (int)blockIdx.x);
}

struct ArenaSet {
    SearchParams S;
    iago_row::HwParams R;
    iago_trunk::TrunkRParams VP;
    iago_policy::PolicyParams PP;
};
struct ArenaArgs {
    ArenaSet set[2];
};
static_assert(sizeof(ArenaArgs) <= 4096, "the arena's two parameter sets must fit the kernel argument segment");

__global__ __launch_bounds__(256) __attribute__((amdgpu_waves_per_eu(1, 1))) void search_arena_kernel(ArenaArgs P)
{
    const long long t0 = wall_clock64();
    const int b = (int)blockIdx.x;
    const int ga = P.set[0].S.n_game_wgs, games = ga + P.set[1].S.n_game_wgs;
    if (b == 0 && threadIdx.x == 0) {
        __hip_atomic_store(&P.set[0].S.ctl[CTL_NET_WGS], (uint32_t)gridDim.x - (uint32_t)games, RLX_AGENT);
        __hip_atomic_store(&P.set[1].S.ctl[CTL_NET_WGS], (uint32_t)gridDim.x - (uint32_t)games, RLX_AGENT);
    }
    const int home = b < games ? (b >= ga ? 1 : 0) : (b & 1);
    if (b < games) {
        const ArenaSet &X = P.set[home];
        game_workgroup<false>(X.S, X.R, t0, home ? b - ga : b);
    }
#pragma unroll 1
    for (int pass = 0; pass < 2; pass++) {
        const ArenaSet &X = P.set[home ^ pass];
        net_workgroup(X.S, X.VP, X.PP, t0, b);
    }
}

constexpr int search_lds() { return SEARCH_IMG_TOP + iago_trunk::W1_LDS + iago_policy::W1_LDS + iago_trunk::HEAD_W_LDS + 192 * 4; }

__global__ void search_scratch_warm_kernel(uint32_t *out, int n)
{
    volatile uint32_t a[64];
    for (int i = 0; i < 64; i++)
        a[i] = (uint32_t)(i * n) + threadIdx.x;
    uint32_t sum = 0;
    for (int i = 0; i < 64; i++)
        sum += a[(i * 7 + n) & 63];
    if (n == 0x7fffffff && out)
        out[0] = sum;
}

struct FormCache {
    const void *kernel;
    std::atomic<uint64_t> reserved{0};
    int static_lds = -1;
    struct {
        int lds = -1, per_cu = 0, cus = 0;
    } on[64];
};

using SearchKernel = void (*)(SearchParams, iago_row::HwParams, iago_trunk::TrunkRParams, iago_policy::PolicyParams);
using GameKernel = void (*)(SearchParams, iago_row::HwParams);
struct Variant {
    const char *who, *no_lds;
    SearchKernel single;
    GameKernel game;
    FormCache single_form{(const void *)single}, game_form{(const void *)game};
};
struct {
    Variant plain, wave, park, noise, gumbel;
} variants = {
    {"iago_mcts_search_persistent", nullptr, search_kernel, search_game_kernel},
    {"iago_mcts_search_wave", "iago_mcts_search_wave: cannot reserve the nets' LDS image", search_wave_kernel, nullptr},
    {"iago_mcts_search_park", "iago_mcts_search_park: cannot reserve the nets' LDS image", search_park_kernel, search_game_park_kernel},
    {"iago_mcts_search_noise", "iago_mcts_search_noise: cannot reserve the nets' LDS image", search_noise_kernel, search_game_noise_kernel},
    {"iago_mcts_search_gumbel", "iago_mcts_search_gumbel: cannot reserve the nets' LDS image", search_gumbel_kernel, search_game_gumbel_kernel}};
FormCache net_form{(const void *)search_net_kernel}, arena_form{(const void *)search_arena_kernel};
std::mutex form_cache_mutex;

int reserve_lds(FormCache &f, int bytes, const char *who) { return iago_reserve_lds(f.kernel, bytes, f.reserved, who); }

bool static_lds_of(FormCache &f, int &bytes)
{
    std::lock_guard<std::mutex> lock(form_cache_mutex);
    hipFuncAttributes fa;
    if (f.static_lds < 0 && hipFuncGetAttributes(&fa, f.kernel) == hipSuccess)
        f.static_lds = (int)fa.sharedSizeBytes;
    bytes = f.static_lds;
    return bytes >= 0;
}

bool residency_of(FormCache &f, int dev, int lds, int &per_cu, int *cus)
{
    std::lock_guard<std::mutex> lock(form_cache_mutex);
    auto &r = f.on[dev & 63];
    if (cus && r.cus < 1 && hipDeviceGetAttribute(&r.cus, hipDeviceAttributeMultiprocessorCount, dev) != hipSuccess) {
        r.cus = 0;
        return false;
    }
    if (r.lds != lds) {
        r.lds = -1;
        if (hipOccupancyMaxActiveBlocksPerMultiprocessor(&r.per_cu, f.kernel, 256, (size_t)lds) != hipSuccess)
            return false;
        r.lds = lds;
    }
    per_cu = r.per_cu;
    if (cus)
        *cus = r.cus;
    return true;
}

}

extern "C" int iago_mcts_search_capacity(int32_t *cus, int32_t *workgroups_per_cu)
{
    if (!cus || !workgroups_per_cu)
        return iago_fail(IAGO_ERR_INVALID, "iago_mcts_search_capacity: null pointer");
    if (reserve_lds(variants.plain.single_form, search_lds(), "iago_mcts_search_capacity: cannot reserve the nets' LDS image"))
        return IAGO_ERR_HIP;
    int dev = 0, n_cu = 0, per = 0;
    if (hipGetDevice(&dev) != hipSuccess)
        return iago_fail(IAGO_ERR_HIP, "iago_mcts_search_capacity: hipGetDevice failed");
    if (!residency_of(variants.plain.single_form, dev, search_lds(), per, &n_cu))
        return iago_fail(IAGO_ERR_HIP, "iago_mcts_search_capacity: the device does not answer");
    if (n_cu < 1 || per < 1 || per > 255)
        return iago_fail(IAGO_ERR_CAPACITY, "iago_mcts_search_capacity: the search kernel does not fit a CU of this device");
    *cus = n_cu;
    *workgroups_per_cu = per;
    return IAGO_OK;
}

struct iago_search_streams {
    int device;
    int32_t cus, game_cus;
    hipStream_t game, net;
    hipEvent_t ready, game_done, net_done;
};

namespace {
struct LaunchRequest {
    iago_search_streams *streams = nullptr;
    const iago_search_wave_args *wave = nullptr;
    const iago_search_park_args *park = nullptr;
    int explore_turns = 0;
    int cap_fast = 0, cap_full_256 = 256;
    const iago_root_noise *noise = nullptr;
    int forced_k_256 = 0;
    const iago_gumbel_root *gumbel = nullptr;
    Variant &variant() const
    {
        return wave ? variants.wave : gumbel ? variants.gumbel : noise ? variants.noise : park ? variants.park : variants.plain;
    }
};

constexpr int SEARCH_FLAGS = IAGO_SEARCH_CHAIN_SKIP | IAGO_SEARCH_NEGAMAX | IAGO_SEARCH_PUCT_AZ;
int games_per_wg_of(const iago_mcts_search_args *a)
{
    return a->games_per_workgroup > 0 ? (a->games_per_workgroup & ~SEARCH_FLAGS) : a->games_per_workgroup;
}

int check_args(const iago_mcts_search_args *a, const iago_search_wave_args *wv)
{
    if (!a || !a->tree || !a->value || !a->policy || !a->rollout)
        return iago_fail(IAGO_ERR_INVALID, "iago_mcts_search_persistent: null args");
    const iago_mcts_tree *tree = a->tree;
    if (tree->n_games < 1 || tree->capacity < 1 || !tree->nodes || ((uintptr_t)tree->nodes & 31u) || !tree->n_nodes ||
        !tree->root || !tree->overflow || !tree->has_v)
        return iago_fail(IAGO_ERR_INVALID, "iago_mcts_search_persistent: bad tree (the value cache `v` is required)");
    if (tree->n_games > 0x7FFFFFF0ll)
        return iago_fail(IAGO_ERR_INVALID, "iago_mcts_search_persistent: too many games");
    if (!a->active || !a->cur_node || !a->cur_own || !a->cur_opp || !a->path ||
        a->path_stride < 8 || !a->done || !a->roll || !a->leaf_value || !a->q_slots || !a->ctl || !a->rep_v || !a->rep_p ||
        !a->totals || !a->wg_own || !a->wg_opp || ((uintptr_t)a->q_slots & 63u) || ((uintptr_t)a->rep_p & 7u) ||
        ((uintptr_t)a->rep_v & 7u) || ((uintptr_t)a->ctl & 15u))
        return iago_fail(IAGO_ERR_INVALID, "iago_mcts_search_persistent: null or misaligned state array");
    if (a->n_thr < 1 || a->n_sims < 0 || !(a->lmbda >= 0.0f && a->lmbda <= 1.0f) || a->net_workgroups < 1)
        return iago_fail(IAGO_ERR_INVALID, "iago_mcts_search_persistent: n_thr >= 1, n_sims >= 0, 0 <= lmbda <= 1, "
                                           "net_workgroups >= 1 expected");
    if (a->max_turns < 0 || (a->max_turns > 0 && (!a->game_own || !a->game_opp || !a->n_turns)) ||
        (a->max_turns > 0 && a->rec_move && (!a->rec_own || !a->rec_opp || !a->rec_valid || !a->rec_pi)))
        return iago_fail(IAGO_ERR_INVALID, "iago_mcts_search_persistent: whole games (max_turns > 0) need game_own, game_opp, "
                                           "n_turns, and all of rec_own / rec_opp / rec_valid / rec_move / rec_pi or none");
    if (a->games_total < 0 || (a->games_total > 0 && (a->max_turns == 0 || a->n_sims < 1 || a->z_log || a->z_log_rows > 0 ||
                                                      a->trace || a->trace_rows > 0)))
        return iago_fail(IAGO_ERR_INVALID, "iago_mcts_search_persistent: games_total >= 0; a stream (games_total > 0) plays "
                                           "whole games (max_turns > 0, n_sims >= 1), without z_log or trace");
    if (a->max_turns == 0 && (!a->root_own || !a->root_opp))
        return iago_fail(IAGO_ERR_INVALID, "iago_mcts_search_persistent: root_own / root_opp expected");
    if (a->z_log_rows > 0 && (!a->z_log || !a->z_log_n))
        return iago_fail(IAGO_ERR_INVALID, "iago_mcts_search_persistent: z_log needs z_log_n");
    const iago_rollout_args *ro = a->rollout;
    const int64_t n_slots = tree->n_games * (wv ? wv->width : 1);
    if (wv && n_slots > (int64_t)QCAP)
        return iago_fail(IAGO_ERR_CAPACITY, "iago_mcts_search_wave: more slots (n_games x width) than a request ring holds");
    if (ro->n != n_slots || !ro->z || !ro->table || ((uintptr_t)ro->table & 15u) || ro->log_form || ro->trace ||
        ro->uniforms || ro->throughput_hint != 0)
        return iago_fail(IAGO_ERR_INVALID, "iago_mcts_search_persistent: product-form rollout of the n games without "
                                           "trace / uniforms expected");
    const int gpw = games_per_wg_of(a);
    if (!wv && gpw > 0 && gpw != 8 && gpw != 16 && gpw != 24 && gpw != 32)
        return iago_fail(IAGO_ERR_INVALID, "iago_mcts_search_persistent: games_per_workgroup is 0 (= 32), 8, 16 or 32");
    if (a->max_cus < 0)
        return iago_fail(IAGO_ERR_INVALID, "iago_mcts_search_persistent: max_cus < 0");
    if (a->vtable_slots > 0 && (!a->vtable || ((uintptr_t)a->vtable & 31u) || (a->vtable_slots & (a->vtable_slots - 1)) != 0))
        return iago_fail(IAGO_ERR_INVALID, "iago_mcts_search_persistent: vtable must be 32-byte aligned, vtable_slots a "
                                           "power of two");
    return IAGO_OK;
}

struct SearchGrid {
    int gpw;
    int chain_skip;
    int negamax;
    int puct_az;
    int64_t n_slots, n_game_wgs, net_wgs, grid;
    int path_lds_cap, game_lds;
};

void size_games(const iago_mcts_search_args *a, const iago_search_wave_args *wv, SearchGrid &G)
{
    G.gpw = wv || games_per_wg_of(a) <= 0 ? GAMES_PER_WG : games_per_wg_of(a);
    G.chain_skip = (!wv && a->games_per_workgroup > 0 && (a->games_per_workgroup & IAGO_SEARCH_CHAIN_SKIP)) ? 1 : 0;
    G.negamax = (a->games_per_workgroup > 0 && (a->games_per_workgroup & IAGO_SEARCH_NEGAMAX)) ? 1 : 0;
    G.puct_az = (a->games_per_workgroup > 0 && (a->games_per_workgroup & IAGO_SEARCH_PUCT_AZ)) ? 1 : 0;
    G.n_slots = a->tree->n_games * (wv ? wv->width : 1);
    G.n_game_wgs = (G.n_slots + G.gpw - 1) / G.gpw;
    G.path_lds_cap = SEARCH_IMG_TOP;
    G.game_lds = 0;
}

int cus_to_count_on(int max_cus, int cus) { return max_cus > 0 && max_cus < cus ? max_cus : cus; }

int check_net_rows(const iago_mcts_search_args *a, int64_t grid, const char *msg)
{
    if (a->value->n < 4 * grid || a->policy->n < 4 * grid || a->value->planes || a->value->index || a->value->n_dev ||
        a->policy->index || a->policy->n_dev || !a->value->own || a->value->own != a->wg_own ||
        a->value->opp != a->wg_opp || a->policy->own != a->wg_own || a->policy->opp != a->wg_opp)
        return iago_fail(IAGO_ERR_INVALID, msg);
    return IAGO_OK;
}

int size_grid(const iago_mcts_search_args *a, const LaunchRequest &q, SearchGrid &G)
{
    size_games(a, q.wave, G);
    int32_t cus = 0, per_cu = 0;
    if (const int rc = iago_mcts_search_capacity(&cus, &per_cu))
        return rc;
    int64_t resident = (int64_t)cus_to_count_on(a->max_cus, cus) * per_cu;
    if (const iago_search_streams *sp = q.streams) {
        int dev = 0;
        if (hipGetDevice(&dev) != hipSuccess || dev != sp->device || sp->cus != cus)
            return iago_fail(IAGO_ERR_INVALID, "iago_mcts_search_split: the streams belong to another device");
        if (a->max_cus != 0)
            return iago_fail(IAGO_ERR_INVALID, "iago_mcts_search_split: max_cus must be 0 (the split owns the device's CUs)");
        if (!q.variant().game)
            return iago_fail(IAGO_ERR_INVALID, "iago_mcts_search_split: this search has no game launch (the wave search is not split)");
        FormCache &game = q.variant().game_form;
        const size_t want = (size_t)G.gpw * (size_t)a->path_stride * 4u;
        int fixed = 0, per_game = 0;
        if (!static_lds_of(game, fixed))
            return iago_fail(IAGO_ERR_HIP, "iago_mcts_search_split: hipFuncGetAttributes failed");
        G.game_lds = (want + (size_t)fixed + 256u) * 2u <= (size_t)160 * 1024u ? (int)want : 0;
        G.path_lds_cap = G.game_lds;
        if (G.game_lds && reserve_lds(game, 96 * 1024, "iago_mcts_search_split: cannot reserve the game workgroups' LDS"))
            return IAGO_ERR_HIP;
        if (!residency_of(game, dev, G.game_lds, per_game, nullptr))
            return iago_fail(IAGO_ERR_HIP, "iago_mcts_search_split: the device does not answer");
        if (G.n_game_wgs > (int64_t)sp->game_cus * per_game)
            return iago_fail(IAGO_ERR_CAPACITY, "iago_mcts_search_split: the game workgroups do not fit the game launch's CUs "
                                                "(more game CUs, fewer games per launch, or the single launch)");
        const int64_t net_cus = cus - (sp->game_cus > cus / 8 ? sp->game_cus : cus / 8);
        resident = G.n_game_wgs + net_cus * per_cu;
    }
    if (G.n_game_wgs + 1 > resident)
        return iago_fail(IAGO_ERR_CAPACITY, "iago_mcts_search_persistent: the game workgroups and one net workgroup do not "
                                            "fit the device together (fewer games per launch, or the per-playout launches)");
    G.net_wgs = std::min<int64_t>(a->net_workgroups, resident - G.n_game_wgs);
    G.grid = G.n_game_wgs + G.net_wgs;
    return check_net_rows(a, G.grid, "iago_mcts_search_persistent: the nets read their rows from wg_own / wg_opp "
                                     "(four rows per workgroup of the grid: n >= 4 x (game + net workgroups)), no gather list, no "
                                     "device count");
}

SearchParams search_params(const iago_mcts_search_args *a, const SearchGrid &G, const LaunchRequest &q)
{
    const iago_search_wave_args *wv = q.wave;
    SearchParams S;
    S.T = *a->tree;
    S.root_own = a->root_own;
    S.root_opp = a->root_opp;
    S.active = a->active;
    S.c_puct = a->c_puct;
    S.lmbda = a->lmbda;
    S.n_thr = a->n_thr;
    S.n_sims = a->n_sims;
    S.n_game_wgs = (int32_t)G.n_game_wgs;
    S.games_per_wg = G.gpw;
    S.cur_node = a->cur_node;
    S.cur_own = a->cur_own;
    S.cur_opp = a->cur_opp;
    S.path = a->path;
    S.path_stride = a->path_stride;
    S.done = a->done;
    S.roll = a->roll;
    S.z = a->rollout->z;
    S.leaf_value = a->leaf_value;
    S.z_log = a->z_log_rows > 0 ? a->z_log : nullptr;
    S.z_log_n = a->z_log_n;
    S.z_log_rows = a->z_log_rows;
    S.q_slots = (u64 *)a->q_slots;
    S.ctl = a->ctl;
    S.rep_v = (u64 *)a->rep_v;
    S.rep_p = (u64 *)a->rep_p;
    S.totals = a->totals;
    S.stats = a->stats;
    S.wg_own = a->wg_own;
    S.wg_opp = a->wg_opp;
    S.clock_limit = (long long)(a->time_limit_ms > 0 ? a->time_limit_ms : 2000) * 100000ll;
    static const int pair_backlog = [] {
        const char *e = getenv("IAGO_PERSISTENT_PAIR");
        const int v = e ? atoi(e) : 1;
        return v < 1 ? 0x7fffffff : v;
    }();
    S.pair_backlog = pair_backlog;
    static const int policy_xcds = [] {
        const char *e = getenv("IAGO_PERSISTENT_POLICY_XCDS");
        const int v = e ? atoi(e) : 2;
        return v < 0 ? 0 : (v > 7 ? 7 : v);
    }();
    S.policy_xcds = policy_xcds;
    const char *pace_env = getenv("IAGO_PERSISTENT_PACE_BACKLOG");
    S.pace_backlog = pace_env ? atoi(pace_env) : 128;
    S.pace_margin = wv ? -1 : a->pace_margin == 0 ? 16 : (a->pace_margin < 0 ? -1 : a->pace_margin);
    const char *ahead_env = getenv("IAGO_PERSISTENT_AHEAD");
    S.ahead_idle = ahead_env ? atoi(ahead_env) : 4;
    const char *defer_env = getenv("IAGO_PERSISTENT_ROLL_DEFER");
    S.roll_defer = defer_env ? atoi(defer_env) : 10;
    if (S.roll_defer < 0 || S.roll_defer > 15)
        S.roll_defer = S.roll_defer < 0 ? 0 : 15;
    S.path_lds_cap = G.path_lds_cap;
    S.wave = wv ? wv->width : 1;
    S.vloss = wv ? wv->vloss : 0.0f;
    S.n_slots = G.n_slots;
    S.wave_timing = wv ? wv->timing : nullptr;
    S.max_turns = a->max_turns;
    S.game_own = a->game_own;
    S.game_opp = a->game_opp;
    S.n_turns = a->n_turns;
    S.rec_own = a->rec_own;
    S.rec_opp = a->rec_opp;
    S.rec_valid = a->rec_valid;
    S.rec_move = a->rec_move;
    S.rec_pi = a->rec_pi;
    S.stream = a->games_total > 0 ? 1 : 0;
    S.games_total = a->games_total > 0 ? a->games_total : (int32_t)a->tree->n_games;
    S.vtable = a->vtable_slots > 0 ? (u64 *)a->vtable : nullptr;
    S.vtable_mask = a->vtable_slots > 0 ? (uint32_t)(a->vtable_slots - 1) : 0u;
    S.trace = a->trace_rows > 0 ? a->trace : nullptr;
    S.trace_rows = a->trace_rows;
    S.park_empties = q.park ? q.park->park_empties : -1;
    S.parked = q.park ? q.park->parked : nullptr;
    S.park_stones = q.park ? q.park->stones : nullptr;
    S.park_pass = q.park ? q.park->pass_flg : nullptr;
    S.explore_turns = q.explore_turns;
    S.cap_fast = q.cap_fast;
    S.cap_full_256 = q.cap_full_256;
    S.chain_skip = G.chain_skip;
    S.negamax = G.negamax;
    S.prior_off = G.puct_az ? PRIOR_OFF_ALPHAZERO : PRIOR_OFF_REFERENCE;
    S.visit_off = G.puct_az ? VISIT_OFF_ALPHAZERO : VISIT_OFF_REFERENCE;
    S.noise_counts = q.noise ? q.noise->counts : nullptr;
    S.noise_eps = q.noise ? q.noise->eps_256 : 0;
    S.noise_lg = q.noise ? __builtin_ctz((unsigned)q.noise->draws) : 0;
    S.forced_k_256 = q.noise ? q.forced_k_256 : 0;
    S.gumbel_g = q.gumbel ? q.gumbel->g : nullptr;
    S.gumbel_ln = q.gumbel ? q.gumbel->ln_q16 : nullptr;
    S.gumbel_sched = q.gumbel ? q.gumbel->sched : nullptr;
    S.gumbel_m = q.gumbel ? q.gumbel->m : 0;
    S.gumbel_c_visit = q.gumbel ? q.gumbel->c_visit : 0;
    S.gumbel_c_scale = q.gumbel ? q.gumbel->c_scale_256 : 0;
    return S;
}

int net_params(const iago_mcts_search_args *a, iago_trunk::TrunkRParams &VP, iago_policy::PolicyParams &PP, iago_row::HwParams &R)
{
    if (const int rc = iago_trunk::value_params_of(a->value, VP))
        return rc;
    VP.count_lo = 0;
    VP.count_hi = 0x7fffffff;
    if (const int rc = iago_policy::policy_params_of(a->policy, PP))
        return rc;
    R = iago_row::hw_params_of(a->rollout);
    R.own = a->cur_own;
    R.opp = a->cur_opp;
    R.mask = a->roll;
    R.stream_ids = a->done;
    return IAGO_OK;
}

int zero_polled(const iago_mcts_search_args *a, int64_t n_slots, void *stream)
{
    if (hipMemsetAsync(a->ctl, 0, 64, (hipStream_t)stream) != hipSuccess ||
        hipMemsetAsync(a->q_slots, 0, (size_t)2 * QCAP * 64, (hipStream_t)stream) != hipSuccess ||
        hipMemsetAsync(a->rep_v, 0, (size_t)n_slots * 8, (hipStream_t)stream) != hipSuccess ||
        hipMemsetAsync(a->rep_p, 0, (size_t)n_slots * 512, (hipStream_t)stream) != hipSuccess)
        return iago_fail(IAGO_ERR_HIP, "iago_mcts_search_persistent: hipMemsetAsync failed");
    return IAGO_OK;
}

int launch_search(const iago_mcts_search_args *a, void *stream, const LaunchRequest &q, const SearchGrid &G, const SearchParams &S)
{
    iago_trunk::TrunkRParams VP;
    iago_policy::PolicyParams PP;
    iago_row::HwParams R;
    if (const int rc = net_params(a, VP, PP, R))
        return rc;
    constexpr int lds = search_lds();
    if (const int rc = zero_polled(a, G.n_slots, stream))
        return rc;
    const dim3 grid((unsigned)G.grid), block(256);
    iago_search_streams *const sp = q.streams;
    Variant &v = q.variant();
    if (!sp) {
        if (v.no_lds && reserve_lds(v.single_form, lds, v.no_lds))
            return IAGO_ERR_HIP;
        hipLaunchKernelGGL(v.single, grid, block, lds, (hipStream_t)stream, S, R, VP, PP);
        return iago_check_launch(v.who);
    }
    if (reserve_lds(net_form, lds, "iago_mcts_search_split: cannot reserve the nets' LDS image"))
        return IAGO_ERR_HIP;
    if (hipEventRecord(sp->ready, (hipStream_t)stream) != hipSuccess || hipStreamWaitEvent(sp->game, sp->ready, 0) != hipSuccess ||
        hipStreamWaitEvent(sp->net, sp->ready, 0) != hipSuccess)
        return iago_fail(IAGO_ERR_HIP, "iago_mcts_search_split: cannot order the launches after the stream");
    hipLaunchKernelGGL(v.game, dim3((unsigned)G.n_game_wgs), block, G.game_lds, sp->game, S, R);
    int rc = iago_check_launch("iago_mcts_search_split (game launch)");
    if (rc == IAGO_OK) {
        hipLaunchKernelGGL(search_net_kernel, dim3((unsigned)G.net_wgs), block, lds, sp->net, S, VP, PP);
        rc = iago_check_launch("iago_mcts_search_split (net launch)");
    }
    if (hipEventRecord(sp->game_done, sp->game) != hipSuccess || hipEventRecord(sp->net_done, sp->net) != hipSuccess ||
        hipStreamWaitEvent((hipStream_t)stream, sp->game_done, 0) != hipSuccess ||
        hipStreamWaitEvent((hipStream_t)stream, sp->net_done, 0) != hipSuccess)
        return iago_fail(IAGO_ERR_HIP, "iago_mcts_search_split: cannot order the stream after the launches");
    return rc;
}

int search_launch(const iago_mcts_search_args *a, void *stream, const LaunchRequest &q)
{
    SearchGrid G;
    if (const int rc = check_args(a, q.wave))
        return rc;
    if (const int rc = size_grid(a, q, G))
        return rc;
    const SearchParams S = search_params(a, G, q);
    if (q.park && hipMemsetAsync(q.park->parked, 0, (size_t)S.games_total, (hipStream_t)stream) != hipSuccess) {
        (void)hipGetLastError();
        return iago_fail(IAGO_ERR_HIP, "iago_mcts_search_park: clearing parked");
    }
    return launch_search(a, stream, q, G, S);
}

int has_match_codes(const uint8_t *active, int64_t n, hipStream_t stream)
{
    hipPointerAttribute_t at;
    const bool on_device = hipPointerGetAttributes(&at, active) == hipSuccess &&
                           (at.type == hipMemoryTypeDevice || at.type == hipMemoryTypeManaged);
    (void)hipGetLastError();
    std::vector<uint8_t> copy;
    if (on_device) {
        copy.resize((size_t)n);
        if (hipMemcpyAsync(copy.data(), active, (size_t)n, hipMemcpyDeviceToHost, stream) != hipSuccess ||
            hipStreamSynchronize(stream) != hipSuccess) {
            (void)hipGetLastError();
            return -1;
        }
        active = copy.data();
    }
    for (int64_t i = 0; i < n; i++)
        if (active[i] > 1)
            return 1;
    return 0;
}

int self_play_only(const iago_mcts_search_args *a, void *stream, const char *who, const char *why)
{
    if (a->max_turns == 0)
        return iago_fail(IAGO_ERR_INVALID, (std::string(who) + ": whole games only (max_turns > 0)").c_str());
    if (a->games_total == 0 && a->active && a->tree && a->tree->n_games >= 1) {
        const int m = has_match_codes(a->active, a->tree->n_games, (hipStream_t)stream);
        if (m < 0)
            return iago_fail(IAGO_ERR_HIP, (std::string(who) + ": cannot read `active`").c_str());
        if (m)
            return iago_fail(IAGO_ERR_INVALID,
                             (std::string(who) + ": match codes in `active` (self-play games only: " + why + ")").c_str());
    }
    return IAGO_OK;
}

int check_reserved(const int64_t (&reserved)[4], int32_t reserved0, const char *who)
{
    for (int i = 0; i < 4; i++)
        if (reserved[i] != 0 || reserved0 != 0)
            return iago_fail(IAGO_ERR_INVALID, (std::string(who) + ": reserved fields must be 0").c_str());
    return IAGO_OK;
}

int check_park(const iago_search_park_args *pk, const char *who)
{
    const std::string w(who);
    if (!pk->parked || !pk->stones || !pk->pass_flg)
        return iago_fail(IAGO_ERR_INVALID, (w + ": parked, stones and pass_flg expected").c_str());
    if (const int rc = check_reserved(pk->reserved, pk->reserved0, who))
        return rc;
    if (pk->park_empties < 0 || pk->park_empties > IAGO_ENDGAME_MAX_EMPTIES)
        return iago_fail(IAGO_ERR_INVALID, (w + ": park_empties must be in [0, 20]").c_str());
    return IAGO_OK;
}

int explore_launch(const iago_mcts_search_args *a, void *stream, const LaunchRequest &q, const char *who, const char *why)
{
    const std::string w(who);
    if (q.explore_turns < 0 || q.explore_turns > IAGO_MAX_TURNS)
        return iago_fail(IAGO_ERR_INVALID, (w + ": explore_turns must be in [0, 128]").c_str());
    if (q.park) {
        if (const int rc = check_park(q.park, (w + " (park)").c_str()))
            return rc;
        if (q.park->streams && q.park->streams != q.streams)
            return iago_fail(IAGO_ERR_INVALID, (w + " (park): park->streams must be NULL or `streams`").c_str());
    }
    if (const int rc = self_play_only(a, stream, who, why))
        return rc;
    return search_launch(a, stream, q);
}

bool arena_shared(const iago_mcts_search_args *a, const iago_mcts_search_args *b)
{
    const void *pa[] = {a->ctl, a->q_slots, a->rep_v, a->rep_p, a->tree, a->tree->nodes, a->tree->n_nodes, a->tree->root,
                        a->tree->overflow, a->cur_node, a->cur_own, a->cur_opp, a->path, a->done, a->roll, a->leaf_value,
                        a->rollout->z, a->wg_own, a->wg_opp};
    const void *pb[] = {b->ctl, b->q_slots, b->rep_v, b->rep_p, b->tree, b->tree->nodes, b->tree->n_nodes, b->tree->root,
                        b->tree->overflow, b->cur_node, b->cur_own, b->cur_opp, b->path, b->done, b->roll, b->leaf_value,
                        b->rollout->z, b->wg_own, b->wg_opp};
    for (size_t i = 0; i < sizeof(pa) / sizeof(pa[0]); i++)
        if (pa[i] == pb[i])
            return true;
    return a->vtable_slots > 0 && b->vtable_slots > 0 && a->vtable == b->vtable;
}
}

extern "C" int iago_mcts_search_persistent(const iago_mcts_search_args *a, void *stream)
{
    return search_launch(a, stream, LaunchRequest());
}

extern "C" int iago_mcts_search_split(const iago_mcts_search_args *a, iago_search_streams *streams, void *stream)
{
    if (!streams)
        return iago_fail(IAGO_ERR_INVALID, "iago_mcts_search_split: null streams");
    LaunchRequest q;
    q.streams = streams;
    return search_launch(a, stream, q);
}

extern "C" int iago_mcts_search_wave(const iago_mcts_search_args *a, const iago_search_wave_args *w, void *stream)
{
    if (!a || !w)
        return iago_fail(IAGO_ERR_INVALID, "iago_mcts_search_wave: null args");
    if (w->width != 1 && w->width != 8 && w->width != 16 && w->width != 32)
        return iago_fail(IAGO_ERR_INVALID, "iago_mcts_search_wave: width is 1, 8, 16 or 32");
    if (!(w->vloss >= 0.0f && w->vloss <= 3.4028235e38f))
        return iago_fail(IAGO_ERR_INVALID, "iago_mcts_search_wave: vloss >= 0 (finite) expected");
    if (a->max_turns != 0 || a->games_total != 0)
        return iago_fail(IAGO_ERR_INVALID, "iago_mcts_search_wave: one search per launch (max_turns 0, games_total 0): "
                                           "whole games take iago_mcts_search_persistent");
    LaunchRequest q;
    q.wave = w;
    return search_launch(a, stream, q);
}

extern "C" int iago_mcts_search_park(const iago_mcts_search_args *a, const iago_search_park_args *pk, void *stream)
{
    if (!a || !pk)
        return iago_fail(IAGO_ERR_INVALID, "iago_mcts_search_park: null args");
    if (const int rc = check_park(pk, "iago_mcts_search_park"))
        return rc;
    if (const int rc = self_play_only(a, stream, "iago_mcts_search_park",
                                      "a match's policy side needs the net workgroups to its last move"))
        return rc;
    LaunchRequest q;
    q.streams = pk->streams;
    q.park = pk;
    return search_launch(a, stream, q);
}

extern "C" int iago_mcts_search_explore(const iago_mcts_search_args *a, const iago_search_explore_args *ex, void *stream)
{
    if (!a || !ex)
        return iago_fail(IAGO_ERR_INVALID, "iago_mcts_search_explore: null args");
    if (const int rc = check_reserved(ex->reserved, ex->reserved0, "iago_mcts_search_explore"))
        return rc;
    LaunchRequest q;
    q.streams = ex->streams;
    q.park = ex->park;
    q.explore_turns = ex->explore_turns;
    return explore_launch(a, stream, q, "iago_mcts_search_explore", "a match's moves are not drawn from the visit counts");
}

extern "C" int iago_mcts_search_cap(const iago_mcts_search_args *a, const iago_search_cap_args *cap, void *stream)
{
    if (!a || !cap)
        return iago_fail(IAGO_ERR_INVALID, "iago_mcts_search_cap: null args");
    if (const int rc = check_reserved(cap->reserved, cap->reserved0, "iago_mcts_search_cap"))
        return rc;
    if (cap->n_fast < 1 || cap->n_fast > a->n_sims)
        return iago_fail(IAGO_ERR_INVALID, "iago_mcts_search_cap: n_fast must be in [1, n_sims]");
    if (cap->full_per_256 < 1 || cap->full_per_256 > 256)
        return iago_fail(IAGO_ERR_INVALID, "iago_mcts_search_cap: full_per_256 must be in [1, 256]");
    LaunchRequest q;
    q.streams = cap->streams;
    q.park = cap->park;
    q.explore_turns = cap->explore_turns;
    q.cap_fast = cap->n_fast;
    q.cap_full_256 = cap->full_per_256;
    return explore_launch(a, stream, q, "iago_mcts_search_cap", "a match's searches are not capped");
}

extern "C" int iago_mcts_search_noise(const iago_mcts_search_args *a, const iago_search_noise_args *nz, void *stream)
{
    if (!a || !nz)
        return iago_fail(IAGO_ERR_INVALID, "iago_mcts_search_noise: null args");
    if (const int rc = check_reserved(nz->reserved, 0, "iago_mcts_search_noise"))
        return rc;
    if (const int rc = check_root_noise(&nz->noise, "iago_mcts_search_noise"))
        return rc;
    if (a->max_turns != 0 || a->games_total != 0)
        return iago_fail(IAGO_ERR_INVALID, "iago_mcts_search_noise: one search per launch (max_turns 0, games_total 0): whole "
                                           "games with root noise run turn by turn");
    LaunchRequest q;
    q.streams = nz->streams;
    q.noise = &nz->noise;
    return search_launch(a, stream, q);
}

extern "C" int iago_mcts_search_forced(const iago_mcts_search_args *a, const iago_search_forced_args *fz, void *stream)
{
    if (!a || !fz)
        return iago_fail(IAGO_ERR_INVALID, "iago_mcts_search_forced: null args");
    if (const int rc = check_reserved(fz->reserved, fz->reserved0, "iago_mcts_search_forced"))
        return rc;
    if (const int rc = check_root_noise(&fz->noise, "iago_mcts_search_forced"))
        return rc;
    if (fz->k_256 < 1 || fz->k_256 > 4096)
        return iago_fail(IAGO_ERR_INVALID, "iago_mcts_search_forced: k_256 must be in [1, 4096]");
    if (a->max_turns != 0 || a->games_total != 0)
        return iago_fail(IAGO_ERR_INVALID, "iago_mcts_search_forced: one search per launch (max_turns 0, games_total 0): whole "
                                           "games with forced playouts run turn by turn");
    LaunchRequest q;
    q.streams = fz->streams;
    q.noise = &fz->noise;
    q.forced_k_256 = fz->k_256;
    return search_launch(a, stream, q);
}

extern "C" int iago_mcts_search_gumbel(const iago_mcts_search_args *a, const iago_search_gumbel_args *gz, void *stream)
{
    if (!a || !gz)
        return iago_fail(IAGO_ERR_INVALID, "iago_mcts_search_gumbel: null args");
    if (const int rc = check_reserved(gz->reserved, 0, "iago_mcts_search_gumbel"))
        return rc;
    if (const int rc = iago_check_gumbel_root(&gz->gumbel, "iago_mcts_search_gumbel"))
        return rc;
    if (!gz->gumbel.sched)
        return iago_fail(IAGO_ERR_INVALID, "iago_mcts_search_gumbel: null schedule");
    if (a->max_turns != 0 || a->games_total != 0)
        return iago_fail(IAGO_ERR_INVALID, "iago_mcts_search_gumbel: one search per launch (max_turns 0, games_total 0): whole "
                                           "games under the Gumbel rule run turn by turn");
    if (a->n_sims < 1 || a->n_sims > 32767)
        return iago_fail(IAGO_ERR_INVALID, "iago_mcts_search_gumbel: n_sims must be in [1, 32767] (the schedule's columns)");
    if (a->games_per_workgroup <= 0 || !(a->games_per_workgroup & IAGO_SEARCH_NEGAMAX))
        return iago_fail(IAGO_ERR_INVALID, "iago_mcts_search_gumbel: the negamax backup is required (IAGO_SEARCH_NEGAMAX: a root "
                                           "child's Q must be the root mover's value)");
    if (!(a->games_per_workgroup & IAGO_SEARCH_PUCT_AZ))
        return iago_fail(IAGO_ERR_INVALID, "iago_mcts_search_gumbel: the AlphaZero selection is required (IAGO_SEARCH_PUCT_AZ: a "
                                           "child's stored prior must be the policy's p)");
    LaunchRequest q;
    q.streams = gz->streams;
    q.gumbel = &gz->gumbel;
    return search_launch(a, stream, q);
}

extern "C" int iago_mcts_search_arena(const iago_mcts_search_args *a, const iago_mcts_search_args *b, void *stream)
{
    if (!a || !b)
        return iago_fail(IAGO_ERR_INVALID, "iago_mcts_search_arena: null args");
    const iago_mcts_search_args *const set[2] = {a, b};
    for (int i = 0; i < 2; i++) {
        if (set[i]->max_turns != 0 || set[i]->games_total != 0)
            return iago_fail(IAGO_ERR_INVALID, "iago_mcts_search_arena: one search per agent and launch (max_turns 0, "
                                               "games_total 0): a game's two trees live in different workgroups");
        if (const int rc = check_args(set[i], nullptr))
            return rc;
        const int m = has_match_codes(set[i]->active, set[i]->tree->n_games, (hipStream_t)stream);
        if (m < 0)
            return iago_fail(IAGO_ERR_HIP, "iago_mcts_search_arena: cannot read `active`");
        if (m)
            return iago_fail(IAGO_ERR_INVALID, "iago_mcts_search_arena: match codes in `active` (0 / 1 expected)");
    }
    if (arena_shared(a, b))
        return iago_fail(IAGO_ERR_INVALID, "iago_mcts_search_arena: the two argument sets share a tree, ctl, q_slots, reply "
                                           "or state arrays, or a position table (each agent needs its own)");
    const int want = a->net_workgroups > b->net_workgroups ? a->net_workgroups : b->net_workgroups;
    if (want < 2)
        return iago_fail(IAGO_ERR_INVALID, "iago_mcts_search_arena: net_workgroups >= 2 expected (a server per agent)");
    int32_t cus = 0, per_cu = 0;
    if (const int rc = iago_mcts_search_capacity(&cus, &per_cu))
        return rc;
    constexpr int lds = search_lds();
    if (reserve_lds(arena_form, lds, "iago_mcts_search_arena: cannot reserve the nets' LDS image"))
        return IAGO_ERR_HIP;
    int dev = 0, per = 0;
    if (hipGetDevice(&dev) != hipSuccess)
        return iago_fail(IAGO_ERR_HIP, "iago_mcts_search_arena: hipGetDevice failed");
    if (!residency_of(arena_form, dev, lds, per, nullptr))
        return iago_fail(IAGO_ERR_HIP, "iago_mcts_search_arena: the device does not answer");
    if (per < 1)
        return iago_fail(IAGO_ERR_CAPACITY, "iago_mcts_search_arena: the arena kernel does not fit a CU of this device");
    const int64_t resident = (int64_t)cus_to_count_on(b->max_cus, cus_to_count_on(a->max_cus, cus)) * per;
    SearchGrid G[2];
    int64_t games = 0;
    for (int i = 0; i < 2; i++) {
        size_games(set[i], nullptr, G[i]);
        games += G[i].n_game_wgs;
    }
    if (games + 2 > resident)
        return iago_fail(IAGO_ERR_CAPACITY, "iago_mcts_search_arena: both agents' game workgroups and two net workgroups do "
                                            "not fit the device together (fewer games per launch, or one search after the other)");
    const int64_t net_wgs = std::min<int64_t>(want, resident - games);
    const int64_t grid = games + net_wgs;
    ArenaArgs args;
    ArenaSet *const P = args.set;
    for (int i = 0; i < 2; i++) {
        G[i].net_wgs = net_wgs;
        G[i].grid = grid;
        if (const int rc = check_net_rows(set[i], grid,
                                          "iago_mcts_search_arena: each agent's nets read their rows from its wg_own / "
                                          "wg_opp (four rows per workgroup of the WHOLE grid: n >= 4 x (both agents' game "
                                          "workgroups + net workgroups)), no gather list, no device count"))
            return rc;
        P[i].S = search_params(set[i], G[i], LaunchRequest());
        if (const int rc = net_params(set[i], P[i].VP, P[i].PP, P[i].R))
            return rc;
    }
    const long long limit = P[0].S.clock_limit > P[1].S.clock_limit ? P[0].S.clock_limit : P[1].S.clock_limit;
    P[0].S.clock_limit = limit;
    P[1].S.clock_limit = limit;
    for (int i = 0; i < 2; i++)
        if (const int rc = zero_polled(set[i], G[i].n_slots, stream))
            return rc;
    hipLaunchKernelGGL(search_arena_kernel, dim3((unsigned)grid), dim3(256), lds, (hipStream_t)stream, args);
    return iago_check_launch("iago_mcts_search_arena");
}

extern "C" int iago_mcts_search_streams_create(int32_t game_cus, iago_search_streams **out)
{
    if (!out)
        return iago_fail(IAGO_ERR_INVALID, "iago_mcts_search_streams_create: null pointer");
    *out = nullptr;
    int dev = 0, cus = 0;
    if (hipGetDevice(&dev) != hipSuccess || hipDeviceGetAttribute(&cus, hipDeviceAttributeMultiprocessorCount, dev) != hipSuccess)
        return iago_fail(IAGO_ERR_HIP, "iago_mcts_search_streams_create: the device does not answer");
    if (game_cus < 8 || game_cus % 8 != 0 || cus % 8 != 0 || game_cus > cus / 2)
        return iago_fail(IAGO_ERR_INVALID, "iago_mcts_search_streams_create: game_cus is a multiple of 8, at most half the "
                                           "device's CUs");
    uint32_t gm[32] = {0}, nm[32] = {0};
    if (cus > 1024)
        return iago_fail(IAGO_ERR_CAPACITY, "iago_mcts_search_streams_create: more CUs than the mask holds");
    for (int i = 0; i < cus; i++)
        (i < game_cus ? gm : nm)[i / 32] |= 1u << (i % 32);
    iago_search_streams *sp = new iago_search_streams();
    sp->device = dev;
    sp->cus = cus;
    sp->game_cus = game_cus;
    const uint32_t words = (uint32_t)((cus + 31) / 32);
    bool ok = hipExtStreamCreateWithCUMask(&sp->game, words, gm) == hipSuccess;
    ok = ok && hipExtStreamCreateWithCUMask(&sp->net, words, nm) == hipSuccess;
    ok = ok && hipEventCreateWithFlags(&sp->ready, hipEventDisableTiming) == hipSuccess;
    ok = ok && hipEventCreateWithFlags(&sp->game_done, hipEventDisableTiming) == hipSuccess;
    ok = ok && hipEventCreateWithFlags(&sp->net_done, hipEventDisableTiming) == hipSuccess;
    if (ok) {
        hipLaunchKernelGGL(search_scratch_warm_kernel, dim3(1), dim3(64), 0, sp->game, (uint32_t *)nullptr, 1);
        hipLaunchKernelGGL(search_scratch_warm_kernel, dim3(1), dim3(64), 0, sp->net, (uint32_t *)nullptr, 1);
        ok = hipGetLastError() == hipSuccess && hipStreamSynchronize(sp->game) == hipSuccess &&
             hipStreamSynchronize(sp->net) == hipSuccess;
    }
    if (!ok) {
        (void)hipGetLastError();
        iago_mcts_search_streams_destroy(sp);
        return iago_fail(IAGO_ERR_HIP, "iago_mcts_search_streams_create: no CU-masked streams on this device (use the single "
                                       "launch, iago_mcts_search_persistent)");
    }
    *out = sp;
    return IAGO_OK;
}

extern "C" int iago_mcts_search_streams_destroy(iago_search_streams *sp)
{
    if (!sp)
        return IAGO_OK;
    if (sp->game)
        (void)hipStreamDestroy(sp->game);
    if (sp->net)
        (void)hipStreamDestroy(sp->net);
    if (sp->ready)
        (void)hipEventDestroy(sp->ready);
    if (sp->game_done)
        (void)hipEventDestroy(sp->game_done);
    if (sp->net_done)
        (void)hipEventDestroy(sp->net_done);
    delete sp;
    return IAGO_OK;
}
```

Before: 3043.

## Batch two policy boards per workgroup with a row-wise tile walk

Policy net workgroups can now take two queued policy requests at once (TB=2). They stage both boards in LDS and walk a new row-wise tiling that skips tiles lying off the board, so each MFMA A-fragment load is reused across twice as many B tiles. To make room in LDS, the value-head weights are overwritten when a pair is processed and restaged lazily before the next value request. The change adds policy pairing in the claim logic, a per-pair counter, and more LDS and register pressure, plus a restaging cost whenever the workgroup switches back to value work.

```diff
diff --git a/iago_amd/csrc/conv_policy_body.hpp b/iago_amd/csrc/conv_policy_body.hpp
--- a/iago_amd/csrc/conv_policy_body.hpp
+++ b/iago_amd/csrc/conv_policy_body.hpp
@@ -1,6 +1,7 @@
 #pragma once
 #include "abi_common.hpp"
 #include "search_request.hpp"
+#include "walk_tiles.hpp"
 
 #include <hip/hip_fp16.h>
 
@@ -24,7 +25,8 @@
 constexpr int BS = 64 * RS + ZB;
 constexpr int HEAD_FLOATS = 64;
 constexpr int W1_LDS = (64 * 18 + 64) * 4;
-constexpr int LDS_BYTES = BS + 1024 + HEAD_FLOATS * 4 + W1_LDS;
+constexpr int lds_bytes(int tb) { return tb * BS + 1024 + HEAD_FLOATS * 4 + W1_LDS; }
+constexpr int LDS_BYTES = lds_bytes(1);
 constexpr float S1 = 1.0f / 2048.0f, S2 = 1.0f / (2048.0f * 2048.0f);
 
 struct PolicyParams {
@@ -54,44 +56,60 @@
 
 extern __shared__ __align__(16) char policy_lds[];
 
-template <bool SRCH = false>
+template <bool SRCH = false, int TB = 1, bool OWN = SRCH>
 __device__ __forceinline__ void policy_item(const PolicyParams &P, const int64_t row_id, const uint32_t *pos = nullptr,
                                             float *res = nullptr, const float *w1_staged = nullptr,
                                             const float *head_w = nullptr)
 {
+    static_assert(TB == 1 || TB == 2, "boards per workgroup");
+    constexpr bool ROWS = TB == 2;
+    constexpr int NN = 4 * TB;
     char *const T = policy_lds;
     int tid_ = threadIdx.x;
-    if constexpr (SRCH)
+    if constexpr (OWN)
         asm volatile("" : "+v"(tid_));
     const int tid = tid_, wv = __builtin_amdgcn_readfirstlane(tid >> 6), lane = tid & 63;
     const int64_t b = P.index ? P.index[row_id] : row_id;
 
-    if (tid < ZB / 16)
-        *(uint4 *)(T + 64 * RS + tid * 16) = make_uint4(0, 0, 0, 0);
+    if constexpr (ROWS) {
+        if (tid < 2 * (ZB / 16))
+            *(uint4 *)(T + (tid >= ZB / 16 ? BS - ZB : 0) + 64 * RS + tid * 16) = make_uint4(0, 0, 0, 0);
+    } else {
+        if (tid < ZB / 16)
+            *(uint4 *)(T + 64 * RS + tid * 16) = make_uint4(0, 0, 0, 0);
+    }
     bool saturated = false;
     if (P.layer_lo > 0) {
-        const uint4 *src = P.scratch + (row_id - P.row_lo) * (64 * RS / 16);
-        for (int e = tid; e < 64 * RS / 16; e += 256)
-            *(uint4 *)(T + e * 16) = src[e];
+#pragma unroll
+        for (int board = 0; board < TB; board++) {
+            const uint4 *src = P.scratch + (row_id + board - P.row_lo) * (64 * RS / 16);
+            for (int e = tid; e < 64 * RS / 16; e += 256)
+                *(uint4 *)(T + board * BS + e * 16) = src[e];
+        }
     } else {
         const int cell = tid & 63, y = cell >> 3, x = cell & 7;
-        const uint64_t bits0 = SRCH ? iago_request::opp(pos) : P.opp[b];
-        const uint64_t bits1 = SRCH ? iago_request::own(pos) : P.own[b];
-        float in[18];
-#pragma unroll
-        for (int c = 0; c < 2; c++)
-#pragma unroll
-            for (int ky = 0; ky < 3; ky++)
-#pragma unroll
-                for (int kx = 0; kx < 3; kx++) {
-                    const int yy = y + ky - 1, xx = x + kx - 1;
-                    const bool ok = yy >= 0 && yy < 8 && xx >= 0 && xx < 8;
-                    const int a = (yy * 8 + xx) & 63;
-                    in[c * 9 + ky * 3 + kx] = (ok && (((c ? bits1 : bits0) >> a) & 1ull)) ? 1.0f : 0.0f;
-                }
+        float in[TB][18];
+#pragma unroll
+        for (int board = 0; board < TB; board++) {
+            const int64_t bb = board == 0 ? b : (P.index ? P.index[row_id + board] : row_id + board);
+            const uint32_t *const pw = pos + iago_request::WORDS * board;
+            const uint64_t bits0 = SRCH ? iago_request::opp(pw) : P.opp[bb];
+            const uint64_t bits1 = SRCH ? iago_request::own(pw) : P.own[bb];
+#pragma unroll
+            for (int c = 0; c < 2; c++)
+#pragma unroll
+                for (int ky = 0; ky < 3; ky++)
+#pragma unroll
+                    for (int kx = 0; kx < 3; kx++) {
+                        const int yy = y + ky - 1, xx = x + kx - 1;
+                        const bool ok = yy >= 0 && yy < 8 && xx >= 0 && xx < 8;
+                        const int a = (yy * 8 + xx) & 63;
+                        in[board][c * 9 + ky * 3 + kx] = (ok && (((c ? bits1 : bits0) >> a) & 1ull)) ? 1.0f : 0.0f;
+                    }
+        }
         const float *w1s = w1_staged;
         if constexpr (!SRCH) {
-            float *const st = (float *)(T + BS + 1024 + HEAD_FLOATS * 4);
+            float *const st = (float *)(T + TB * BS + 1024 + HEAD_FLOATS * 4);
             for (int e = tid; e < 64 * 18 / 4; e += 256)
                 ((float4 *)st)[e] = ((const float4 *)P.w1)[e];
             if (tid < 16)
@@ -103,48 +121,88 @@
         for (int g2 = 0; g2 < 2; g2++) {
             const int grp = __builtin_amdgcn_readfirstlane(g2 * 4 + wv);
             const int co0 = grp * 8;
-            _Float16 p0[8], p1[8], p2[8];
-#pragma unroll
-            for (int k = 0; k < 8; k += 2) {
-                const float *wa = w1s + (co0 + k) * 18, *wb = wa + 18;
-                f2 acc = (f2){w1s[64 * 18 + co0 + k], w1s[64 * 18 + co0 + k + 1]};
-#pragma unroll
-                for (int j = 0; j < 18; j++)
-                    acc = __builtin_elementwise_fma((f2){wa[j], wb[j]}, (f2){in[j], in[j]}, acc);
-                saturated |= !(acc.x <= 65000.0f) || !(acc.y <= 65000.0f);
-                f2 v;
-                v.x = fminf(fmaxf(acc.x, 0.0f), 65000.0f);
-                v.y = fminf(fmaxf(acc.y, 0.0f), 65000.0f);
-                h2 a0, a1, a2;
-                split3(v, a0, a1, a2);
-                p0[k] = a0.x, p0[k + 1] = a0.y;
-                p1[k] = a1.x, p1[k + 1] = a1.y;
-                p2[k] = a2.x, p2[k + 1] = a2.y;
-            }
-            char *dst = T + cell * RS + (grp >> 1) * 32 + (grp & 1) * 16;
-            *(uint4 *)dst = *(const uint4 *)p0;
-            *(uint4 *)(dst + 256) = *(const uint4 *)p1;
-            *(uint4 *)(dst + 512) = *(const uint4 *)p2;
+            _Float16 p0[TB][8], p1[TB][8], p2[TB][8];
+            if constexpr (ROWS) {
+#pragma unroll
+                for (int k = 0; k < 8; k++) {
+                    const float *wk = w1s + (co0 + k) * 18;
+                    const float bk = w1s[64 * 18 + co0 + k];
+                    f2 acc = (f2){bk, bk};
+#pragma unroll
+                    for (int j = 0; j < 18; j++)
+                        acc = __builtin_elementwise_fma((f2){wk[j], wk[j]}, (f2){in[0][j], in[TB - 1][j]}, acc);
+                    saturated |= !(acc.x <= 65000.0f) || !(acc.y <= 65000.0f);
+                    f2 v;
+                    v.x = fminf(fmaxf(acc.x, 0.0f), 65000.0f);
+                    v.y = fminf(fmaxf(acc.y, 0.0f), 65000.0f);
+                    h2 a0, a1, a2;
+                    split3(v, a0, a1, a2);
+                    p0[0][k] = a0.x, p0[TB - 1][k] = a0.y;
+                    p1[0][k] = a1.x, p1[TB - 1][k] = a1.y;
+                    p2[0][k] = a2.x, p2[TB - 1][k] = a2.y;
+                }
+            } else {
+#pragma unroll
+                for (int k = 0; k < 8; k += 2) {
+                    const float *wa = w1s + (co0 + k) * 18, *wb = wa + 18;
+                    f2 acc = (f2){w1s[64 * 18 + co0 + k], w1s[64 * 18 + co0 + k + 1]};
+#pragma unroll
+                    for (int j = 0; j < 18; j++)
+                        acc = __builtin_elementwise_fma((f2){wa[j], wb[j]}, (f2){in[0][j], in[0][j]}, acc);
+                    saturated |= !(acc.x <= 65000.0f) || !(acc.y <= 65000.0f);
+                    f2 v;
+                    v.x = fminf(fmaxf(acc.x, 0.0f), 65000.0f);
+                    v.y = fminf(fmaxf(acc.y, 0.0f), 65000.0f);
+                    h2 a0, a1, a2;
+                    split3(v, a0, a1, a2);
+                    p0[0][k] = a0.x, p0[0][k + 1] = a0.y;
+                    p1[0][k] = a1.x, p1[0][k + 1] = a1.y;
+                    p2[0][k] = a2.x, p2[0][k + 1] = a2.y;
+                }
+            }
+#pragma unroll
+            for (int board = 0; board < TB; board++) {
+                char *dst = T + board * BS + cell * RS + (grp >> 1) * 32 + (grp & 1) * 16;
+                *(uint4 *)dst = *(const uint4 *)p0[board];
+                *(uint4 *)(dst + 256) = *(const uint4 *)p1[board];
+                *(uint4 *)(dst + 512) = *(const uint4 *)p2[board];
+            }
         }
     }
     __syncthreads();
 
+    static_assert(BS % 256 == 0, "the pair's bank pattern");
     const int c16 = lane & 15, kq = lane >> 4;
-    uint32_t addr[4][9];
-#pragma unroll
-    for (int q = 0; q < 4; q++)
+    uint32_t addr[ROWS ? 1 : 4][9];
+    uint32_t sx[2] = {0u, 0u};
+    uint32_t wrow[ROWS ? 1 : 4];
+    if constexpr (ROWS) {
+        const int x = c16 & 7, odd = c16 >> 3;
 #pragma unroll
         for (int tap = 0; tap < 9; tap++) {
-            const int cell = 16 * q + c16;
-            const int yy = (cell >> 3) + tap / 3 - 1, xx = (cell & 7) + tap % 3 - 1;
-            const bool ok = yy >= 0 && yy < 8 && xx >= 0 && xx < 8;
-            const int lin = (cell + (tap / 3 - 1) * 8 + (tap % 3 - 1)) & 7;
-            addr[q][tap] = (uint32_t)((ok ? (yy * 8 + xx) * RS : 64 * RS + 32 * lin) + kq * 16);
-        }
-    uint32_t wrow[4];
-#pragma unroll
-    for (int q = 0; q < 4; q++)
-        wrow[q] = (uint32_t)((16 * q + c16) * RS);
+            const int row = tap < 3 ? 1 : 0;
+            const int yy = row + tap / 3 - 1, xx = x + tap % 3 - 1;
+            const bool ok = xx >= 0 && xx < 8;
+            addr[0][tap] = (uint32_t)(odd * BS + (ok ? (yy * 8 + xx) * RS : 64 * RS + 32 * (xx & 7)) + kq * 16);
+        }
+        sx[0] = x > 0 ? 8u * RS : 0u;
+        sx[1] = x < 7 ? 8u * RS : 0u;
+        wrow[0] = (uint32_t)(odd * BS + x * RS);
+    } else {
+#pragma unroll
+        for (int q = 0; q < 4; q++)
+#pragma unroll
+            for (int tap = 0; tap < 9; tap++) {
+                const int cell = 16 * q + c16;
+                const int yy = (cell >> 3) + tap / 3 - 1, xx = (cell & 7) + tap % 3 - 1;
+                const bool ok = yy >= 0 && yy < 8 && xx >= 0 && xx < 8;
+                const int lin = (cell + (tap / 3 - 1) * 8 + (tap % 3 - 1)) & 7;
+                addr[q][tap] = (uint32_t)((ok ? (yy * 8 + xx) * RS : 64 * RS + 32 * lin) + kq * 16);
+            }
+#pragma unroll
+        for (int q = 0; q < 4; q++)
+            wrow[q] = (uint32_t)((16 * q + c16) * RS);
+    }
 
     for (int L = P.layer_lo; L < P.layer_hi; L++) {
         const int n_pairs = L == 0 ? 2 : 4;
@@ -153,11 +211,11 @@
         auto a_load = [&](const char *base, uint32_t step_bytes, int m) -> u32x4 {
             return *(const u32x4 *)(base + step_bytes + a_lane + (uint32_t)m * 512u);
         };
-        float4v acc0[2][4], acc0b[2][4], acc1[2][4], acc2[2][4];
+        float4v acc0[2][NN], acc0b[2][NN], acc1[2][NN], acc2[2][NN];
 #pragma unroll
         for (int m = 0; m < 2; m++)
 #pragma unroll
-            for (int n = 0; n < 4; n++)
+            for (int n = 0; n < NN; n++)
 #pragma unroll
                 for (int v = 0; v < 4; v++) {
                     acc0[m][n][v] = 0.0f;
@@ -175,92 +233,176 @@
                 a_lo[i][m] = a_load(wl, (uint32_t)i * 4096u, m);
             }
         half8 bh[3], bm[3], bl[3];
-        auto b_addr = [&](int tile) -> const char * {
-            const int over = tile >= 36 ? 64 : 0, tt = tile % 36;
-            return T + addr[tt & 3][tt >> 2] + over;
-        };
-        {
-            const char *p0 = b_addr(0), *p1 = b_addr(1);
-            bh[0] = *(const half8 *)p0, bm[0] = *(const half8 *)(p0 + 256), bl[0] = *(const half8 *)(p0 + 512);
-            bh[1] = *(const half8 *)p1, bm[1] = *(const half8 *)(p1 + 256), bl[1] = *(const half8 *)(p1 + 512);
-        }
-        for (int cp = 0; cp < n_pairs; cp++) {
-#pragma unroll
-            for (int tap = 0; tap < 9; tap++) {
-                int cp2 = cp, tp2 = tap + 2;
-                if (tp2 >= 9) {
-                    tp2 -= 9;
-                    cp2 += 1;
+        if constexpr (ROWS) {
+            constexpr int KEPT = iago_walk::kept_before(2, 9, 0);
+            static_assert(KEPT == 66 && KEPT % 3 == 0, "the B ring must line up at every chunk pair");
+            auto b_off = [&](int tap, int n) -> uint32_t {
+                const int dx = tap % 3 - 1, r = n - (tap < 3 ? 1 : 0);
+                return addr[0][tap] + (uint32_t)r * (dx == 0 ? 8u * RS : sx[dx > 0]);
+            };
+            iago_walk::static_for<0, 2>([&](auto kc) __attribute__((always_inline)) {
+                constexpr int i = decltype(kc)::value, tile = iago_walk::kept_tile(2, i);
+                const char *p0 = T + b_off(tile / NN, tile % NN);
+                bh[i] = *(const half8 *)p0, bm[i] = *(const half8 *)(p0 + 256), bl[i] = *(const half8 *)(p0 + 512);
+            });
+            for (int cp = 0; cp < n_pairs; cp++) {
+                iago_walk::static_for<0, KEPT>([&](auto kc) __attribute__((always_inline)) {
+                    constexpr int k = decltype(kc)::value, tile = iago_walk::kept_tile(2, k), tap = tile / NN, n = tile % NN;
+                    constexpr int j = k - iago_walk::kept_before(2, tap, 0);
+                    static_assert(iago_walk::kept_before(2, tap + 1, 0) - iago_walk::kept_before(2, tap, 0) >= 3,
+                                  "six A loads per k-step, two per tile");
+                    constexpr int kn = k + 2, tile_n = iago_walk::kept_tile(2, kn % KEPT), cur = k % 3, nxt = kn % 3;
+                    constexpr uint32_t over = kn >= KEPT ? 64u : 0u;
+                    int cp2 = cp, tp2 = tap + 2;
+                    if (tp2 >= 9) {
+                        tp2 -= 9;
+                        cp2 += 1;
+                    }
+                    if (cp2 >= n_pairs) {
+                        cp2 = n_pairs - 1;
+                        tp2 = 8;
+                    }
+                    const uint32_t w2 = (uint32_t)(18 * cp2 + tp2) * 4096u;
+                    const half8 ah0 = __builtin_bit_cast(half8, a_hi[tap % 3][0]), ah1 = __builtin_bit_cast(half8, a_hi[tap % 3][1]);
+                    const half8 am0 = __builtin_bit_cast(half8, a_mid[tap % 3][0]), am1 = __builtin_bit_cast(half8, a_mid[tap % 3][1]);
+                    const half8 al0 = __builtin_bit_cast(half8, a_lo[tap % 3][0]), al1 = __builtin_bit_cast(half8, a_lo[tap % 3][1]);
+                    const char *p = T + b_off(tile_n / NN, tile_n % NN) + over;
+                    __builtin_amdgcn_sched_barrier(0);
+                    IAGO_POLICY_MFMA16(acc2[0][n], ah0, bl[cur]);
+                    bh[nxt] = *(const half8 *)p;
+                    __builtin_amdgcn_sched_barrier(0);
+                    IAGO_POLICY_MFMA16(acc2[1][n], ah1, bl[cur]);
+                    bm[nxt] = *(const half8 *)(p + 256);
+                    __builtin_amdgcn_sched_barrier(0);
+                    IAGO_POLICY_MFMA16(acc1[0][n], ah0, bm[cur]);
+                    bl[nxt] = *(const half8 *)(p + 512);
+                    __builtin_amdgcn_sched_barrier(0);
+                    IAGO_POLICY_MFMA16(acc1[1][n], ah1, bm[cur]);
+                    if constexpr (j == 0)
+                        a_hi[(tap + 2) % 3][0] = a_load(wh, w2, 0);
+                    else if constexpr (j == 1)
+                        a_mid[(tap + 2) % 3][0] = a_load(wm, w2, 0);
+                    else if constexpr (j == 2)
+                        a_lo[(tap + 2) % 3][0] = a_load(wl, w2, 0);
+                    __builtin_amdgcn_sched_barrier(0);
+                    if constexpr (tap & 1)
+                        IAGO_POLICY_MFMA16(acc0b[0][n], ah0, bh[cur]);
+                    else
+                        IAGO_POLICY_MFMA16(acc0[0][n], ah0, bh[cur]);
+                    if constexpr (j == 0)
+                        a_hi[(tap + 2) % 3][1] = a_load(wh, w2, 1);
+                    else if constexpr (j == 1)
+                        a_mid[(tap + 2) % 3][1] = a_load(wm, w2, 1);
+                    else if constexpr (j == 2)
+                        a_lo[(tap + 2) % 3][1] = a_load(wl, w2, 1);
+                    __builtin_amdgcn_sched_barrier(0);
+                    if constexpr (tap & 1)
+                        IAGO_POLICY_MFMA16(acc0b[1][n], ah1, bh[cur]);
+                    else
+                        IAGO_POLICY_MFMA16(acc0[1][n], ah1, bh[cur]);
+                    IAGO_POLICY_MFMA16(acc2[0][n], al0, bh[cur]);
+                    IAGO_POLICY_MFMA16(acc2[1][n], al1, bh[cur]);
+                    IAGO_POLICY_MFMA16(acc1[0][n], am0, bh[cur]);
+                    IAGO_POLICY_MFMA16(acc1[1][n], am1, bh[cur]);
+                    IAGO_POLICY_MFMA16(acc2[0][n], am0, bm[cur]);
+                    IAGO_POLICY_MFMA16(acc2[1][n], am1, bm[cur]);
+                    __builtin_amdgcn_sched_barrier(0);
+                });
+#pragma unroll
+                for (int tap = 0; tap < 9; tap++)
+                    addr[0][tap] += 64u;
+            }
+#pragma unroll
+            for (int tap = 0; tap < 9; tap++)
+                addr[0][tap] -= 64u * (uint32_t)n_pairs;
+        } else {
+            auto b_addr = [&](int tile) -> const char * {
+                const int over = tile >= 36 ? 64 : 0, tt = tile % 36;
+                return T + addr[tt & 3][tt >> 2] + over;
+            };
+            {
+                const char *p0 = b_addr(0), *p1 = b_addr(1);
+                bh[0] = *(const half8 *)p0, bm[0] = *(const half8 *)(p0 + 256), bl[0] = *(const half8 *)(p0 + 512);
+                bh[1] = *(const half8 *)p1, bm[1] = *(const half8 *)(p1 + 256), bl[1] = *(const half8 *)(p1 + 512);
+            }
+            for (int cp = 0; cp < n_pairs; cp++) {
+#pragma unroll
+                for (int tap = 0; tap < 9; tap++) {
+                    int cp2 = cp, tp2 = tap + 2;
+                    if (tp2 >= 9) {
+                        tp2 -= 9;
+                        cp2 += 1;
+                    }
+                    if (cp2 >= n_pairs) {
+                        cp2 = n_pairs - 1;
+                        tp2 = 8;
+                    }
+                    const uint32_t w2 = (uint32_t)(18 * cp2 + tp2) * 4096u;
+                    half8 ah[2], am[2], al[2];
+#pragma unroll
+                    for (int m = 0; m < 2; m++) {
+                        ah[m] = __builtin_bit_cast(half8, a_hi[tap % 3][m]);
+                        am[m] = __builtin_bit_cast(half8, a_mid[tap % 3][m]);
+                        al[m] = __builtin_bit_cast(half8, a_lo[tap % 3][m]);
+                    }
+#pragma unroll
+                    for (int q = 0; q < 4; q++) {
+                        const int tile = tap * 4 + q, cur = tile % 3, nxt = (tile + 2) % 3;
+                        const char *p = b_addr(tile + 2);
+                        __builtin_amdgcn_sched_barrier(0);
+                        IAGO_POLICY_MFMA16(acc2[0][q], ah[0], bl[cur]);
+                        bh[nxt] = *(const half8 *)p;
+                        __builtin_amdgcn_sched_barrier(0);
+                        IAGO_POLICY_MFMA16(acc2[1][q], ah[1], bl[cur]);
+                        bm[nxt] = *(const half8 *)(p + 256);
+                        __builtin_amdgcn_sched_barrier(0);
+                        IAGO_POLICY_MFMA16(acc1[0][q], ah[0], bm[cur]);
+                        bl[nxt] = *(const half8 *)(p + 512);
+                        __builtin_amdgcn_sched_barrier(0);
+                        IAGO_POLICY_MFMA16(acc1[1][q], ah[1], bm[cur]);
+                        if (q == 0)
+                            a_hi[(tap + 2) % 3][0] = a_load(wh, w2, 0);
+                        else if (q == 1)
+                            a_mid[(tap + 2) % 3][0] = a_load(wm, w2, 0);
+                        else if (q == 2)
+                            a_lo[(tap + 2) % 3][0] = a_load(wl, w2, 0);
+                        __builtin_amdgcn_sched_barrier(0);
+                        if (tap & 1)
+                            IAGO_POLICY_MFMA16(acc0b[0][q], ah[0], bh[cur]);
+                        else
+                            IAGO_POLICY_MFMA16(acc0[0][q], ah[0], bh[cur]);
+                        if (q == 0)
+                            a_hi[(tap + 2) % 3][1] = a_load(wh, w2, 1);
+                        else if (q == 1)
+                            a_mid[(tap + 2) % 3][1] = a_load(wm, w2, 1);
+                        else if (q == 2)
+                            a_lo[(tap + 2) % 3][1] = a_load(wl, w2, 1);
+                        __builtin_amdgcn_sched_barrier(0);
+                        if (tap & 1)
+                            IAGO_POLICY_MFMA16(acc0b[1][q], ah[1], bh[cur]);
+                        else
+                            IAGO_POLICY_MFMA16(acc0[1][q], ah[1], bh[cur]);
+                        IAGO_POLICY_MFMA16(acc2[0][q], al[0], bh[cur]);
+                        IAGO_POLICY_MFMA16(acc2[1][q], al[1], bh[cur]);
+                        IAGO_POLICY_MFMA16(acc1[0][q], am[0], bh[cur]);
+                        IAGO_POLICY_MFMA16(acc1[1][q], am[1], bh[cur]);
+                        IAGO_POLICY_MFMA16(acc2[0][q], am[0], bm[cur]);
+                        IAGO_POLICY_MFMA16(acc2[1][q], am[1], bm[cur]);
+                        __builtin_amdgcn_sched_barrier(0);
+                    }
                 }
-                if (cp2 >= n_pairs) {
-                    cp2 = n_pairs - 1;
-                    tp2 = 8;
-                }
-                const uint32_t w2 = (uint32_t)(18 * cp2 + tp2) * 4096u;
-                half8 ah[2], am[2], al[2];
-#pragma unroll
-                for (int m = 0; m < 2; m++) {
-                    ah[m] = __builtin_bit_cast(half8, a_hi[tap % 3][m]);
-                    am[m] = __builtin_bit_cast(half8, a_mid[tap % 3][m]);
-                    al[m] = __builtin_bit_cast(half8, a_lo[tap % 3][m]);
-                }
-#pragma unroll
-                for (int q = 0; q < 4; q++) {
-                    const int tile = tap * 4 + q, cur = tile % 3, nxt = (tile + 2) % 3;
-                    const char *p = b_addr(tile + 2);
-                    __builtin_amdgcn_sched_barrier(0);
-                    IAGO_POLICY_MFMA16(acc2[0][q], ah[0], bl[cur]);
-                    bh[nxt] = *(const half8 *)p;
-                    __builtin_amdgcn_sched_barrier(0);
-                    IAGO_POLICY_MFMA16(acc2[1][q], ah[1], bl[cur]);
-                    bm[nxt] = *(const half8 *)(p + 256);
-                    __builtin_amdgcn_sched_barrier(0);
-                    IAGO_POLICY_MFMA16(acc1[0][q], ah[0], bm[cur]);
-                    bl[nxt] = *(const half8 *)(p + 512);
-                    __builtin_amdgcn_sched_barrier(0);
-                    IAGO_POLICY_MFMA16(acc1[1][q], ah[1], bm[cur]);
-                    if (q == 0)
-                        a_hi[(tap + 2) % 3][0] = a_load(wh, w2, 0);
-                    else if (q == 1)
-                        a_mid[(tap + 2) % 3][0] = a_load(wm, w2, 0);
-                    else if (q == 2)
-                        a_lo[(tap + 2) % 3][0] = a_load(wl, w2, 0);
-                    __builtin_amdgcn_sched_barrier(0);
-                    if (tap & 1)
-                        IAGO_POLICY_MFMA16(acc0b[0][q], ah[0], bh[cur]);
-                    else
-                        IAGO_POLICY_MFMA16(acc0[0][q], ah[0], bh[cur]);
-                    if (q == 0)
-                        a_hi[(tap + 2) % 3][1] = a_load(wh, w2, 1);
-                    else if (q == 1)
-                        a_mid[(tap + 2) % 3][1] = a_load(wm, w2, 1);
-                    else if (q == 2)
-                        a_lo[(tap + 2) % 3][1] = a_load(wl, w2, 1);
-                    __builtin_amdgcn_sched_barrier(0);
-                    if (tap & 1)
-                        IAGO_POLICY_MFMA16(acc0b[1][q], ah[1], bh[cur]);
-                    else
-                        IAGO_POLICY_MFMA16(acc0[1][q], ah[1], bh[cur]);
-                    IAGO_POLICY_MFMA16(acc2[0][q], al[0], bh[cur]);
-                    IAGO_POLICY_MFMA16(acc2[1][q], al[1], bh[cur]);
-                    IAGO_POLICY_MFMA16(acc1[0][q], am[0], bh[cur]);
-                    IAGO_POLICY_MFMA16(acc1[1][q], am[1], bh[cur]);
-                    IAGO_POLICY_MFMA16(acc2[0][q], am[0], bm[cur]);
-                    IAGO_POLICY_MFMA16(acc2[1][q], am[1], bm[cur]);
-                    __builtin_amdgcn_sched_barrier(0);
-                }
+#pragma unroll
+                for (int q = 0; q < 4; q++)
+#pragma unroll
+                    for (int tap = 0; tap < 9; tap++)
+                        addr[q][tap] += 64u;
             }
 #pragma unroll
             for (int q = 0; q < 4; q++)
 #pragma unroll
                 for (int tap = 0; tap < 9; tap++)
-                    addr[q][tap] += 64u;
-        }
-#pragma unroll
-        for (int q = 0; q < 4; q++)
-#pragma unroll
-            for (int tap = 0; tap < 9; tap++)
-                addr[q][tap] -= 64u * (uint32_t)n_pairs;
+                    addr[q][tap] -= 64u * (uint32_t)n_pairs;
+        }
 
         f2 bia[2][2];
 #pragma unroll
@@ -274,16 +416,26 @@
         float vmax = 0.0f;
         f2 vsum = (f2){0.0f, 0.0f};
 #pragma unroll
-        for (int q = 0; q < 4; q++) {
-            char *row = T + wrow[q] + (32 * wv + 4 * kq) * 2;
+        for (int q = 0; q < NN; q++) {
+            char *row = T + (ROWS ? wrow[0] + q * (8 * RS) : wrow[ROWS ? 0 : q]) + (32 * wv + 4 * kq) * 2;
 #pragma unroll
             for (int m = 0; m < 2; m++) {
                 h2 p0[2], p1[2], p2[2];
 #pragma unroll
                 for (int t2 = 0; t2 < 2; t2++) {
-                    const f2 m0 = (f2){acc0[m][q][2 * t2], acc0[m][q][2 * t2 + 1]} + (f2){acc0b[m][q][2 * t2], acc0b[m][q][2 * t2 + 1]};
-                    const f2 m1 = (f2){acc1[m][q][2 * t2], acc1[m][q][2 * t2 + 1]};
-                    const f2 m2 = (f2){acc2[m][q][2 * t2], acc2[m][q][2 * t2 + 1]};
+                    auto rd = [](const float a) __attribute__((always_inline)) -> float {
+                        if constexpr (ROWS) {
+                            float r;
+                            asm volatile("v_accvgpr_read_b32 %0, %1" : "=v"(r) : "a"(a));
+                            return r;
+                        } else {
+                            return a;
+                        }
+                    };
+                    const f2 m0 = (f2){rd(acc0[m][q][2 * t2]), rd(acc0[m][q][2 * t2 + 1])} +
+                                  (f2){rd(acc0b[m][q][2 * t2]), rd(acc0b[m][q][2 * t2 + 1])};
+                    const f2 m1 = (f2){rd(acc1[m][q][2 * t2]), rd(acc1[m][q][2 * t2 + 1])};
+                    const f2 m2 = (f2){rd(acc2[m][q][2 * t2]), rd(acc2[m][q][2 * t2 + 1])};
                     f2 v = (m2 * S2 + m1 * S1) + m0 + bia[m][t2];
                     vmax = fmaxf(fmaxf(vmax, v.x), v.y);
                     vsum += v;
@@ -304,14 +456,18 @@
     if (P.overflow && saturated)
         *P.overflow = 1u;
     if (P.layer_hi < 7) {
-        uint4 *dst = P.scratch + (row_id - P.row_lo) * (64 * RS / 16);
-        for (int e = tid; e < 64 * RS / 16; e += 256)
-            dst[e] = *(const uint4 *)(T + e * 16);
+#pragma unroll
+        for (int board = 0; board < TB; board++) {
+            uint4 *dst = P.scratch + (row_id + board - P.row_lo) * (64 * RS / 16);
+            for (int e = tid; e < 64 * RS / 16; e += 256)
+                dst[e] = *(const uint4 *)(T + board * BS + e * 16);
+        }
         return;
     }
 
-    if (wv == 0) {
-        const char *row = T + lane * RS;
+    if (ROWS ? wv < 2 : wv == 0) {
+        const int board = ROWS ? wv : 0;
+        const char *row = T + board * BS + lane * RS;
         float acc = 0.0f;
 #pragma unroll 4
         for (int c8 = 0; c8 < 16; c8++) {
@@ -337,9 +493,9 @@
         for (int o = 32; o > 0; o >>= 1)
             sum += __shfl_xor(sum, o);
         if constexpr (SRCH)
-            res[lane] = e / sum;
+            res[board * 64 + lane] = e / sum;
         else
-            P.probs[row_id * 64 + lane] = e / sum;
+            P.probs[(row_id + board) * 64 + lane] = e / sum;
     }
 }
 
diff --git a/iago_amd/csrc/conv_policy_kernel.hip b/iago_amd/csrc/conv_policy_kernel.hip
--- a/iago_amd/csrc/conv_policy_kernel.hip
+++ b/iago_amd/csrc/conv_policy_kernel.hip
@@ -5,13 +5,21 @@
 namespace {
 using namespace iago_policy;
 
+template <int TB>
 __global__ __launch_bounds__(256) __attribute__((amdgpu_waves_per_eu(1, 1))) void policy_resident_kernel(PolicyParams P)
 {
     int64_t n_rows = P.row_hi;
     if (P.n_dev)
         n_rows = min(n_rows, (int64_t)*P.n_dev);
-    for (int64_t row = P.row_lo + blockIdx.x; row < n_rows; row += gridDim.x) {
-        policy_item(P, row);
+    for (int64_t row = P.row_lo + TB * (int64_t)blockIdx.x; row < n_rows; row += TB * (int64_t)gridDim.x) {
+        if constexpr (TB == 2) {
+            if (row + 1 < n_rows)
+                policy_item<false, 2, true>(P, row);
+            else
+                policy_item<false, 1, true>(P, row);
+        } else {
+            policy_item(P, row);
+        }
         __syncthreads();
     }
 }
@@ -25,9 +33,16 @@
     PolicyParams P;
     if (const int rc = policy_params_of(a, P))
         return rc;
-    static std::atomic<uint64_t> configured{0};
-    if (iago_reserve_lds((const void *)policy_resident_kernel, LDS_BYTES, configured,
+    static const bool pairs = [] {
+        const char *e = getenv("IAGO_PERSISTENT_PAIR");
+        return !e || atoi(e) >= 1;
+    }();
+    static std::atomic<uint64_t> configured{0}, configured2{0};
+    if (iago_reserve_lds((const void *)policy_resident_kernel<1>, LDS_BYTES, configured,
                          "iago_policy_forward_split3: cannot reserve 52 KB of LDS"))
+        return IAGO_ERR_HIP;
+    if (pairs && iago_reserve_lds((const void *)policy_resident_kernel<2>, lds_bytes(2), configured2,
+                                  "iago_policy_forward_split3: cannot reserve 108 KB of LDS"))
         return IAGO_ERR_HIP;
     static const int64_t cap = []() {
         const char *e = getenv("IAGO_POLICY_GRID");
@@ -45,11 +60,16 @@
         P.row_lo = lo;
         P.row_hi = lo + chunk < a->n ? lo + chunk : a->n;
         const int64_t rows = P.row_hi - P.row_lo;
-        const unsigned grid = (unsigned)(rows < cap ? rows : cap);
+        const bool two = pairs && rows >= 2;
+        const int64_t items = two ? (rows + 1) / 2 : rows;
+        const unsigned grid = (unsigned)(items < cap ? items : cap);
         for (int p = 0; p < parts; p++) {
             P.layer_lo = 7 * p / parts;
             P.layer_hi = 7 * (p + 1) / parts;
-            hipLaunchKernelGGL(policy_resident_kernel, dim3(grid), dim3(256), LDS_BYTES, (hipStream_t)stream, P);
+            if (two)
+                hipLaunchKernelGGL(policy_resident_kernel<2>, dim3(grid), dim3(256), lds_bytes(2), (hipStream_t)stream, P);
+            else
+                hipLaunchKernelGGL(policy_resident_kernel<1>, dim3(grid), dim3(256), LDS_BYTES, (hipStream_t)stream, P);
         }
     }
     return iago_check_launch("iago_policy_forward_split3");
diff --git a/iago_amd/csrc/conv_trunk_body.hpp b/iago_amd/csrc/conv_trunk_body.hpp
--- a/iago_amd/csrc/conv_trunk_body.hpp
+++ b/iago_amd/csrc/conv_trunk_body.hpp
@@ -2,6 +2,7 @@
 #include "abi_common.hpp"
 #include "rollout_row_body.hpp"
 #include "search_request.hpp"
+#include "walk_tiles.hpp"
 
 #include <hip/hip_fp16.h>
 
@@ -77,37 +78,10 @@
 
 extern __shared__ __align__(16) char trunk_lds[];
 
-constexpr bool tile_off_board(int tb, int tap, int n)
-{
-    return tb >= 2 && ((tap < 3 && (n & 7) == 0) || (tap >= 6 && (n & 7) == 7));
-}
-constexpr int kept_before(int tb, int tap, int n)
-{
-    int k = 0;
-    for (int t = 0; t < 9; t++)
-        for (int m = 0; m < 4 * tb; m++) {
-            if (t == tap && m == n)
-                return k;
-            k += !tile_off_board(tb, t, m);
-        }
-    return k;
-}
-constexpr int kept_tile(int tb, int k)
-{
-    for (int t = 0; t < 9; t++)
-        for (int m = 0; m < 4 * tb; m++)
-            if (!tile_off_board(tb, t, m) && k-- == 0)
-                return t * 4 * tb + m;
-    return -1;
-}
-template <int I0, int I1, class F>
-__device__ __forceinline__ void static_for(F &&f)
-{
-    if constexpr (I0 < I1) {
-        f(std::integral_constant<int, I0>{});
-        static_for<I0 + 1, I1>(f);
-    }
-}
+using iago_walk::kept_before;
+using iago_walk::kept_tile;
+using iago_walk::static_for;
+using iago_walk::tile_off_board;
 
 template <bool FUSED, int TB, bool SRCH = false>
 __device__ __forceinline__ void trunk_item(const TrunkRParams &P, const Piece &W, const int64_t b0, const int64_t n_rows)
diff --git a/iago_amd/csrc/search_kernel.hip b/iago_amd/csrc/search_kernel.hip
--- a/iago_amd/csrc/search_kernel.hip
+++ b/iago_amd/csrc/search_kernel.hip
@@ -30,6 +30,7 @@
 constexpr int CTL_BAD_DRAW = 13;
 constexpr int CTL_PROGRESS = 5, CTL_PLAYING = 6;
 constexpr int CTL_NET_WGS = 7;
+constexpr int CTL_POLICY_PAIRS = 15;
 constexpr int CTL_IDLE = 14;
 constexpr int CTL_NEXT_GAME = 12;
 namespace rq = iago_request;
@@ -41,6 +42,9 @@
 constexpr int SEARCH_IMG_V = iago_trunk::lds_alloc(2) + iago_trunk::head_lds(2);
 constexpr int SEARCH_IMG_P = iago_policy::BS + 1024 + iago_policy::HEAD_FLOATS * 4;
 constexpr int SEARCH_IMG_TOP = SEARCH_IMG_V > SEARCH_IMG_P ? SEARCH_IMG_V : SEARCH_IMG_P;
+constexpr int SEARCH_IMG_P2 = 2 * iago_policy::BS + 1024;
+constexpr int SEARCH_HEAD_V_END = SEARCH_IMG_TOP + iago_trunk::HEAD_W_LDS;
+constexpr int SEARCH_KEPT = SEARCH_HEAD_V_END > SEARCH_IMG_P2 ? SEARCH_HEAD_V_END : SEARCH_IMG_P2;
 
 struct SearchParams {
     Tree T;
@@ -1267,11 +1271,12 @@
     epilogue<WAVE>(S, I, sh, G, st_levels, st_children, t0);
 }
 
+constexpr int POLICY_PAIR_BACKLOG = 4;
 
 struct NetLds {
     uint32_t req[2][rq::WORDS];
     uint32_t status, count;
-    float res_v[2], res_p[64];
+    float res_v[2], res_p[2][64];
 };
 struct NetWeights {
     float *w1_val, *w1_pol;
@@ -1279,17 +1284,49 @@
     float *head_p;
 };
 struct NetState {
-    uint32_t carry;
+    uint32_t carry, carry_q;
     int n_carry;
+    int head_gone;
     u64 *put_e;
     u64 put_word;
-    long long t_wait, t_walk, n_pairs;
+    long long t_wait, t_walk, n_pairs, n_pairs_p;
 };
 
+__device__ __forceinline__ void stage_value_head(const iago_trunk::TrunkRParams &VP, char *const head_v)
+{
+    int tid = threadIdx.x;
+    asm volatile("" : "+v"(tid));
+    uint4 w9[4];
+    float4 w10[8];
+#pragma unroll
+    for (int i = 0; i < 2; i++) {
+        w9[i] = VP.w9_hi[tid + 256 * i];
+        w9[2 + i] = VP.w9_lo[tid + 256 * i];
+    }
+#pragma unroll
+    for (int i = 0; i < 8; i++)
+        w10[i] = ((const float4 *)VP.w10)[tid + 256 * i];
+    const float w11 = VP.w11[tid & 127], b9 = VP.b9[0];
+#pragma unroll
+    for (int i = 0; i < 2; i++) {
+        ((uint4 *)head_v)[tid + 256 * i] = w9[i];
+        ((uint4 *)(head_v + iago_trunk::HEAD_W_W9LO))[tid + 256 * i] = w9[2 + i];
+    }
+#pragma unroll
+    for (int i = 0; i < 8; i++) {
+        const int e = tid + 256 * i;
+        ((float4 *)(head_v + iago_trunk::HEAD_W_W10))[(e & 15) * 128 + (e >> 4)] = w10[i];
+    }
+    if (tid < 128)
+        ((float *)(head_v + iago_trunk::HEAD_W_W11))[tid] = w11;
+    if (tid == 0)
+        *(float *)(head_v + iago_trunk::HEAD_W_B9) = b9;
+}
+
 __device__ __forceinline__ NetWeights stage_net_weights(const iago_trunk::TrunkRParams &VP, const iago_policy::PolicyParams &PP)
 {
     const int tid = threadIdx.x;
-    float *const w1_val = (float *)(iago_trunk::trunk_lds + SEARCH_IMG_TOP), *const w1_pol = w1_val + (64 * 18 + 64);
+    float *const w1_val = (float *)(iago_trunk::trunk_lds + SEARCH_KEPT), *const w1_pol = w1_val + (64 * 18 + 64);
     for (int e = tid; e < 64 * 18 / 4; e += 256) {
         ((float4 *)w1_val)[e] = ((const float4 *)VP.w1)[e];
         ((float4 *)w1_pol)[e] = ((const float4 *)PP.w1)[e];
@@ -1298,18 +1335,9 @@
         ((float4 *)(w1_val + 64 * 18))[tid] = ((const float4 *)VP.b1)[tid];
         ((float4 *)(w1_pol + 64 * 18))[tid] = ((const float4 *)PP.b1)[tid];
     }
-    char *const head_v = (char *)(w1_pol + (64 * 18 + 64));
-    float *const head_p = (float *)(head_v + iago_trunk::HEAD_W_LDS);
-    for (int e = tid; e < 512; e += 256) {
-        ((uint4 *)head_v)[e] = VP.w9_hi[e];
-        ((uint4 *)(head_v + iago_trunk::HEAD_W_W9LO))[e] = VP.w9_lo[e];
-    }
-    for (int e = tid; e < 128 * 16; e += 256)
-        ((float4 *)(head_v + iago_trunk::HEAD_W_W10))[(e & 15) * 128 + (e >> 4)] = ((const float4 *)VP.w10)[e];
-    if (tid < 128)
-        ((float *)(head_v + iago_trunk::HEAD_W_W11))[tid] = VP.w11[tid];
-    if (tid == 0)
-        *(float *)(head_v + iago_trunk::HEAD_W_B9) = VP.b9[0];
+    char *const head_v = iago_trunk::trunk_lds + SEARCH_IMG_TOP;
+    float *const head_p = w1_pol + (64 * 18 + 64);
+    stage_value_head(VP, head_v);
     if (tid < 128)
         head_p[tid] = PP.w9[tid];
     if (tid < 64)
@@ -1328,7 +1356,7 @@
         bool have = N.n_carry > 0;
         uint32_t t1 = N.carry;
         if (have) {
-            q = KIND_VALUE;
+            q = N.carry_q;
             N.n_carry = 0;
         } else if (ring_backlog(S, home) > 0) {
             t1 = ring_take(S, home);
@@ -1341,12 +1369,13 @@
         if (have) {
             status = ring_fetch(S, q, t1, 0u, L.req[0], t0);
             count = status == 0 ? 1 : 0;
-            if (status == 0 && q == KIND_VALUE && ring_backlog(S, KIND_VALUE) >= S.pair_backlog) {
-                const uint32_t t2 = ring_take(S, KIND_VALUE);
-                if (ring_fetch(S, KIND_VALUE, t2, 8u, L.req[1], t0) == 0) {
+            if (status == 0 && ring_backlog(S, q) >= (q == KIND_POLICY ? max(S.pair_backlog, POLICY_PAIR_BACKLOG) : S.pair_backlog)) {
+                const uint32_t t2 = ring_take(S, q);
+                if (ring_fetch(S, q, t2, 8u, L.req[1], t0) == 0) {
                     count = 2;
                 } else {
                     N.carry = t2;
+                    N.carry_q = q;
                     N.n_carry = 1;
                 }
             }
@@ -1373,6 +1402,11 @@
                                              const NetWeights &Wt, const int64_t row0, const int count)
 {
     const int tid = threadIdx.x;
+    if (N.head_gone) {
+        stage_value_head(VP, Wt.head_v);
+        N.head_gone = 0;
+        __syncthreads();
+    }
     iago_trunk::Piece W = iago_trunk::whole_walk(VP);
     W.pos = L.req[0];
     W.res = L.res_v;
@@ -1393,14 +1427,19 @@
     }
 }
 
-__device__ __forceinline__ void answer_policy(const SearchParams &S, const iago_policy::PolicyParams &PP, NetLds &L,
-                                              const NetWeights &Wt, const int64_t row0)
+__device__ __forceinline__ void answer_policy(const SearchParams &S, const iago_policy::PolicyParams &PP, NetState &N, NetLds &L,
+                                              const NetWeights &Wt, const int64_t row0, const int count)
 {
     const int tid = threadIdx.x;
-    iago_policy::policy_item<true>(PP, row0, L.req[0], L.res_p, Wt.w1_pol, Wt.head_p);
+    if (count == 2) {
+        N.head_gone = 1;
+        iago_policy::policy_item<true, 2>(PP, row0, L.req[0], L.res_p[0], Wt.w1_pol, Wt.head_p);
+    } else {
+        iago_policy::policy_item<true>(PP, row0, L.req[0], L.res_p[0], Wt.w1_pol, Wt.head_p);
+    }
     __syncthreads();
-    if (tid < 64)
-        reply_prior(S, L.req[0], tid, __float_as_uint(L.res_p[tid]));
+    if (tid < 64 * count)
+        reply_prior(S, L.req[tid >> 6], tid & 63, __float_as_uint(L.res_p[tid >> 6][tid & 63]));
 }
 
 __device__ __forceinline__ void leave(const SearchParams &S, const NetState &N)
@@ -1409,6 +1448,7 @@
         atomicAdd((unsigned long long *)&S.totals[3], (unsigned long long)N.n_pairs);
         atomicAdd((unsigned long long *)&S.totals[4], (unsigned long long)N.t_wait);
         atomicAdd((unsigned long long *)&S.totals[5], (unsigned long long)N.t_walk);
+        __hip_atomic_fetch_add(&S.ctl[CTL_POLICY_PAIRS], (uint32_t)N.n_pairs_p, RLX_AGENT);
     }
 }
 
@@ -1419,7 +1459,7 @@
     const int tid = threadIdx.x;
     const int64_t row0 = 4 * (int64_t)wg;
     const uint32_t home = ((int)((uint32_t)wg & 7u) >= 8 - S.policy_xcds) ? KIND_POLICY : KIND_VALUE;
-    NetState N = {0u, 0, nullptr, 0, 0, 0, 0};
+    NetState N = {0u, 0u, 0, 0, nullptr, 0, 0, 0, 0, 0};
     const NetWeights Wt = stage_net_weights(VP, PP);
     for (;;) {
         const long long c0 = wall_clock64();
@@ -1438,11 +1478,13 @@
         }
         const uint32_t kind = rq::kind(L.req[0]);
         const int count = (int)L.count;
-        N.n_pairs += count - 1;
-        if (kind == KIND_VALUE)
+        if (kind == KIND_VALUE) {
+            N.n_pairs += count - 1;
             answer_value(S, VP, N, L, Wt, row0, count);
-        else
-            answer_policy(S, PP, L, Wt, row0);
+        } else {
+            N.n_pairs_p += count - 1;
+            answer_policy(S, PP, N, L, Wt, row0, count);
+        }
         __syncthreads();
         N.t_walk += wall_clock64() - c1;
     }
@@ -1556,7 +1598,8 @@
     }
 }
 
-constexpr int search_lds() { return SEARCH_IMG_TOP + iago_trunk::W1_LDS + iago_policy::W1_LDS + iago_trunk::HEAD_W_LDS + 192 * 4; }
+constexpr int search_lds() { return SEARCH_KEPT + iago_trunk::W1_LDS + iago_policy::W1_LDS + 192 * 4; }
+static_assert(search_lds() <= 160 * 1024, "the net workgroups' LDS: a workgroup has 160 KB");
 
 __global__ void search_scratch_warm_kernel(uint32_t *out, int n)
 {
diff --git a/iago_amd/csrc/walk_tiles.hpp b/iago_amd/csrc/walk_tiles.hpp
--- /dev/null
+++ b/iago_amd/csrc/walk_tiles.hpp
@@ -0,0 +1,39 @@
+#pragma once
+
+#include <type_traits>
+
+namespace iago_walk {
+
+constexpr bool tile_off_board(int tb, int tap, int n)
+{
+    return tb >= 2 && ((tap < 3 && (n & 7) == 0) || (tap >= 6 && (n & 7) == 7));
+}
+constexpr int kept_before(int tb, int tap, int n)
+{
+    int k = 0;
+    for (int t = 0; t < 9; t++)
+        for (int m = 0; m < 4 * tb; m++) {
+            if (t == tap && m == n)
+                return k;
+            k += !tile_off_board(tb, t, m);
+        }
+    return k;
+}
+constexpr int kept_tile(int tb, int k)
+{
+    for (int t = 0; t < 9; t++)
+        for (int m = 0; m < 4 * tb; m++)
+            if (!tile_off_board(tb, t, m) && k-- == 0)
+                return t * 4 * tb + m;
+    return -1;
+}
+template <int I0, int I1, class F>
+__device__ __forceinline__ void static_for(F &&f)
+{
+    if constexpr (I0 < I1) {
+        f(std::integral_constant<int, I0>{});
+        static_for<I0 + 1, I1>(f);
+    }
+}
+
+}
```

After: 3045 (median of 3 runs). No clear change (+0.1%).
